# vandenheuvel/rust-lp

Measured on AMD Instinct MI355X. Metric: simplex iterations/sec, higher is better.
Workload: dtype f64; 1 GPU; dense10k: synthetic dense LP 10000x10000 f64 (+10000 slack columns), SteepestDescent, dense tableau with blocked f64-MFMA updates; m=10000, n=10000, seed=20250002, engine=tableau, update_block=64, parallelism=single GPU, solves=1

## Files before the change

include/relp_engine.h:

```cpp
#ifndef RELP_ENGINE_H
#define RELP_ENGINE_H

#include <stdint.h>

#ifdef __cplusplus
extern "C" {
#endif

typedef struct relp_engine relp_engine_t;

typedef enum {
    RELP_OK = 0,
    RELP_E_ARG = -1,
    RELP_E_HIP = -2,
    RELP_E_ZERO_PIVOT = -3,
    RELP_E_SINGULAR = -4,
    RELP_E_STATE = -5,
    RELP_E_UNSUPPORTED = -6,
    RELP_E_ALLOC = -7
} relp_status_t;

typedef enum {
    RELP_RUNNING = 0,
    RELP_OPTIMAL = 1,
// ... 37 lines not shown
    double  tol_zero;
    double  tol_tie;
    double  tol_feas;
    int32_t poll_interval;
    int32_t trace_capacity;
    int32_t shard_rank, shard_count;
    int32_t update_block;
    int32_t engine;
    int32_t ratio_rule;
    int32_t artificial_removal;
    int32_t pivot_rescue;
    int32_t auto_reinversion;
} relp_config_t;

typedef enum { RELP_RATIO_REFERENCE = 0, RELP_RATIO_LARGEST_PIVOT = 1 } relp_ratio_rule_t;
typedef enum { RELP_ARTIFICIAL_REFERENCE = 0, RELP_ARTIFICIAL_TEXTBOOK = 1 } relp_artificial_removal_t;

typedef enum {
    RELP_ENGINE_REVISED = 0,
    RELP_ENGINE_TABLEAU = 1,
    RELP_ENGINE_LU = 2,
    RELP_ENGINE_AUTO = 3
} relp_engine_kind_t;

void relp_default_config(relp_config_t *cfg);
void relp_robust_config(relp_config_t *cfg);
int32_t relp_engine_kind(const relp_engine_t *h);
relp_status_t relp_robust_stats(const relp_engine_t *h, int64_t *out4);
const char *relp_last_error(const relp_engine_t *h);
const char *relp_version(void);

relp_status_t relp_engine_create(const relp_matrix_data_t *md, const relp_config_t *cfg, relp_engine_t **out);
void          relp_engine_destroy(relp_engine_t *h);
relp_status_t relp_set_stream(relp_engine_t *h, void *hip_stream);

relp_status_t relp_select_primal_pivot_column(relp_engine_t *h, int32_t rule, int32_t *found,
                                              int32_t *column, double *relative_cost);
relp_status_t relp_relative_costs(relp_engine_t *h, double *out_n);
relp_status_t relp_generate_column(relp_engine_t *h, int32_t column, double *out_m);
relp_status_t relp_generate_element(relp_engine_t *h, int32_t row, int32_t column, double *out);
relp_status_t relp_select_primal_pivot_row(relp_engine_t *h, int32_t *found, int32_t *row);
relp_status_t relp_select_primal_pivot_row_of(relp_engine_t *h, const double *column_m, int32_t *found, int32_t *row);
relp_status_t relp_bring_into_basis(relp_engine_t *h, int32_t column, int32_t row, double relative_cost,
                                    int32_t *leaving_column);

relp_status_t relp_run(relp_engine_t *h, int64_t max_iters, int64_t *iterations_done, int32_t *outcome);
relp_status_t relp_solve_relaxation(relp_engine_t *h, int64_t max_iters, int32_t *outcome);
relp_status_t relp_from_basis(relp_engine_t *h, const int32_t *basis_columns_m);
relp_status_t relp_set_reinversion_interval(relp_engine_t *h, int64_t pivots);
int64_t       relp_reinversions(const relp_engine_t *h);
relp_status_t relp_flush(relp_engine_t *h);
relp_status_t relp_tab_flush_stats(relp_engine_t *h, int64_t *out2);
int32_t       relp_tab_load_batch(const relp_engine_t *h);
int32_t       relp_update_block(const relp_engine_t *h);
relp_status_t relp_lu_stats(const relp_engine_t *h, int64_t *out8);
relp_status_t relp_lu_lookahead_stats(const relp_engine_t *h, int64_t *out4);
relp_status_t relp_lu_kernel_layout(const relp_engine_t *h, int32_t *out4);
relp_status_t relp_lu_set_device_factorisation(relp_engine_t *h, int32_t on);
relp_status_t relp_lu_device_factorisation_stats(const relp_engine_t *h, int64_t *out6);
relp_status_t relp_lu_factor_residual(relp_engine_t *h, double *out);

relp_status_t relp_lu_phase_cycles(relp_engine_t *h, int64_t *out16);

relp_status_t relp_basis_inverse_row(relp_engine_t *h, int32_t row, double *out_m);
relp_status_t relp_should_refactor(relp_engine_t *h, int32_t *out);
relp_status_t relp_generate_column_of(relp_engine_t *h, const int32_t *row_idx, const double *values, int32_t nnz, double *out_m);
relp_status_t relp_cost_difference_of(relp_engine_t *h, const int32_t *row_idx, const double *values, int32_t nnz, double *out);
relp_status_t relp_lu_change_basis(relp_engine_t *h, int32_t pivot_row_index);
relp_status_t relp_lu_set_factors(relp_engine_t *h, const int64_t *l_col_ptr, const int32_t *l_row_idx, const double *l_values,
                                  const int64_t *u_col_ptr, const int32_t *u_row_idx, const double *u_values);
relp_status_t relp_lu_updates(relp_engine_t *h, int32_t *count);
relp_status_t relp_lu_get_update(relp_engine_t *h, int32_t k, int32_t *pivot, int32_t *idx, double *values, int32_t cap, int32_t *nnz);
relp_status_t relp_lu_get_upper(relp_engine_t *h, int64_t *col_ptr_m1, int32_t *row_idx, double *values, int64_t cap, int64_t *nnz);

int32_t relp_nr_rows(const relp_engine_t *h);
int32_t relp_nr_columns(const relp_engine_t *h);
int32_t relp_phase(const relp_engine_t *h);
int32_t relp_nr_artificial(const relp_engine_t *h);
relp_status_t relp_get_objective(relp_engine_t *h, double *out);
relp_status_t relp_get_b(relp_engine_t *h, double *out_m);
relp_status_t relp_get_minus_pi(relp_engine_t *h, double *out_m);
relp_status_t relp_get_basis_indices(relp_engine_t *h, int32_t *out_m);
relp_status_t relp_get_basis_inverse(relp_engine_t *h, double *out_mm);
relp_status_t relp_current_bfs(relp_engine_t *h, int32_t *cols, double *vals, int32_t cap, int32_t *count);
relp_status_t relp_get_iterations(relp_engine_t *h, int64_t *out);
relp_status_t relp_get_degenerate_pivots(relp_engine_t *h, int64_t *out);
relp_status_t relp_get_trace(relp_engine_t *h, int32_t *phase, int32_t *entering, int32_t *row,
                             int32_t *leaving, int64_t cap, int64_t *count);
relp_status_t relp_check_basis(relp_engine_t *h, double *max_identity_error, double *max_basic_cost,
                               double *min_b);

typedef enum {
    RELP_K_PRICE = 0, RELP_K_SELECT_COLUMN = 1, RELP_K_BUILD_COLUMN = 2, RELP_K_FTRAN = 3,
    RELP_K_RATIO = 4, RELP_K_UPDATE_VECTORS = 5, RELP_K_UPDATE_INVERSE = 6,
    RELP_K_APPLY_W = 7,
    RELP_K_UPDATE_W = 8,
    RELP_K_FLUSH = 9,
    RELP_K_FT_RUN = 10,
    RELP_K_COUNT = 11
} relp_kernel_id_t;
relp_status_t relp_profile_enable(relp_engine_t *h, int32_t enable, int64_t max_launches, int32_t sample_every);
relp_status_t relp_profile_read(relp_engine_t *h, int32_t kernel_id, int64_t *launches, double *total_ms);

relp_status_t relp_synth_fill_dense(double *device_a, int64_t ld, int32_t m, int32_t n, uint64_t seed,
                                    int64_t first_column, void *hip_stream);
relp_status_t relp_device_alloc(void **out, int64_t bytes);
// ... 33 lines not shown
```

rust-lp_amd/csrc/relp_abi.cpp:

```cpp
#include <cstring>
#include <new>

#include "relp_engine.hpp"

using relp::Engine;

struct relp_engine { Engine impl; };

#define H(h) ((h)->impl)

extern "C" {

void relp_default_config(relp_config_t* cfg) {
    std::memset(cfg, 0, sizeof(*cfg));
    cfg->device = -1;
    cfg->phase_one_rule = RELP_RULE_FIRST_PROFITABLE_WITH_MEMORY;
    cfg->phase_two_rule = RELP_RULE_STEEPEST_DESCENT;
    cfg->tol_cost = 1e-7; cfg->tol_pivot = 1e-5; cfg->tol_zero = 1e-11; cfg->tol_tie = 1e-9; cfg->tol_feas = 1e-7;
    cfg->poll_interval = 64;
    cfg->trace_capacity = 0;
    cfg->shard_rank = 0; cfg->shard_count = 1;
    cfg->update_block = -1;
    cfg->engine = RELP_ENGINE_REVISED;
}
// ... 5 lines not shown
    cfg->pivot_rescue = 1;
    cfg->auto_reinversion = 1;
    cfg->engine = RELP_ENGINE_AUTO;
}
int32_t relp_engine_kind(const relp_engine_t* h) { return h ? H(h).engine_kind() : -1; }
relp_status_t relp_robust_stats(const relp_engine_t* h, int64_t* out4) { return (h && out4) ? H(h).robust_stats(out4) : RELP_E_ARG; }

const char* relp_last_error(const relp_engine_t* h) { return h ? H(h).last_error() : "null handle"; }
const char* relp_version(void) { return "relp-mi355x 0.2 (gfx950; engines: explicit inverse, dense tableau, sparse LU + Forrest-Tomlin)"; }

relp_status_t relp_engine_create(const relp_matrix_data_t* md, const relp_config_t* cfg, relp_engine_t** out) {
    if (!md || !cfg || !out) return RELP_E_ARG;
    relp_engine_t* h = new (std::nothrow) relp_engine_t();
    if (!h) return RELP_E_ALLOC;
    relp_status_t st = H(h).create(*md, *cfg);
    *out = h;
    return st;
}

void relp_engine_destroy(relp_engine_t* h) { delete h; }
relp_status_t relp_set_stream(relp_engine_t* h, void* s) { return h ? H(h).set_stream((hipStream_t)s) : RELP_E_ARG; }

relp_status_t relp_select_primal_pivot_column(relp_engine_t* h, int32_t rule, int32_t* found, int32_t* column, double* cost) {
    return h ? H(h).select_primal_pivot_column(rule, found, column, cost) : RELP_E_ARG;
}
relp_status_t relp_relative_costs(relp_engine_t* h, double* out) { return (h && out) ? H(h).relative_costs(out) : RELP_E_ARG; }
relp_status_t relp_generate_column(relp_engine_t* h, int32_t column, double* out) { return h ? H(h).generate_column(column, out) : RELP_E_ARG; }
relp_status_t relp_generate_element(relp_engine_t* h, int32_t row, int32_t column, double* out) {
    return h ? H(h).generate_element(row, column, out) : RELP_E_ARG;
}
relp_status_t relp_select_primal_pivot_row(relp_engine_t* h, int32_t* found, int32_t* row) {
    return h ? H(h).select_primal_pivot_row(found, row) : RELP_E_ARG;
}
relp_status_t relp_select_primal_pivot_row_of(relp_engine_t* h, const double* column, int32_t* found, int32_t* row) {
    return (h && column) ? H(h).select_primal_pivot_row_of(column, found, row) : RELP_E_ARG;
}
relp_status_t relp_bring_into_basis(relp_engine_t* h, int32_t column, int32_t row, double cost, int32_t* leaving) {
    return h ? H(h).bring_into_basis(column, row, cost, leaving) : RELP_E_ARG;
}

relp_status_t relp_run(relp_engine_t* h, int64_t max_iters, int64_t* done, int32_t* outcome) {
    return h ? H(h).run(max_iters, done, outcome) : RELP_E_ARG;
}
relp_status_t relp_solve_relaxation(relp_engine_t* h, int64_t max_iters, int32_t* outcome) {
    return h ? H(h).solve_relaxation(max_iters, outcome) : RELP_E_ARG;
}
relp_status_t relp_from_basis(relp_engine_t* h, const int32_t* basis) { return (h && basis) ? H(h).from_basis(basis) : RELP_E_ARG; }

relp_status_t relp_flush(relp_engine_t* h) { return h ? H(h).flush() : RELP_E_ARG; }
relp_status_t relp_set_reinversion_interval(relp_engine_t* h, int64_t pivots) { return h ? H(h).set_reinversion_interval(pivots) : RELP_E_ARG; }
int64_t relp_reinversions(const relp_engine_t* h) { return h ? H(h).reinversions() : -1; }
int32_t relp_update_block(const relp_engine_t* h) { return h ? H(h).update_block() : -1; }
int32_t relp_tab_load_batch(const relp_engine_t* h) { return h ? H(h).tab_load_batch_size() : -1; }
relp_status_t relp_lu_stats(const relp_engine_t* h, int64_t* out8) { return (h && out8) ? H(h).lu_stats(out8) : RELP_E_ARG; }
relp_status_t relp_lu_lookahead_stats(const relp_engine_t* h, int64_t* out4) { return (h && out4) ? H(h).lu_lookahead_stats(out4) : RELP_E_ARG; }
relp_status_t relp_lu_kernel_layout(const relp_engine_t* h, int32_t* out4) { return (h && out4) ? H(h).lu_kernel_layout(out4) : RELP_E_ARG; }
relp_status_t relp_lu_set_device_factorisation(relp_engine_t* h, int32_t on) { return h ? H(h).lu_set_device_factorisation(on != 0) : RELP_E_ARG; }
relp_status_t relp_lu_factor_residual(relp_engine_t* h, double* out) { return (h && out) ? H(h).lu_factor_residual(out) : RELP_E_ARG; }
relp_status_t relp_lu_device_factorisation_stats(const relp_engine_t* h, int64_t* out6) { return (h && out6) ? H(h).luf_stats(out6) : RELP_E_ARG; }
relp_status_t relp_shard_inject_failure(relp_engine_t* h, int64_t after_pivots) { if (!h) return RELP_E_ARG; H(h).shard_inject_failure(after_pivots); return RELP_OK; }
relp_status_t relp_lu_phase_cycles(relp_engine_t* h, int64_t* out16) { return (h && out16) ? H(h).lu_phase_cycles(out16) : RELP_E_ARG; }
relp_status_t relp_basis_inverse_row(relp_engine_t* h, int32_t row, double* out_m) { return (h && out_m) ? H(h).basis_inverse_row(row, out_m) : RELP_E_ARG; }
relp_status_t relp_should_refactor(relp_engine_t* h, int32_t* out) { return (h && out) ? H(h).should_refactor(out) : RELP_E_ARG; }
relp_status_t relp_generate_column_of(relp_engine_t* h, const int32_t* idx, const double* val, int32_t nnz, double* out_m) {
    return h ? H(h).generate_column_of(idx, val, nnz, out_m) : RELP_E_ARG;
}
relp_status_t relp_cost_difference_of(relp_engine_t* h, const int32_t* idx, const double* val, int32_t nnz, double* out) {
    return h ? H(h).cost_difference_of(idx, val, nnz, out) : RELP_E_ARG;
}
relp_status_t relp_lu_change_basis(relp_engine_t* h, int32_t row) { return h ? H(h).lu_change_basis(row) : RELP_E_ARG; }
relp_status_t relp_lu_set_factors(relp_engine_t* h, const int64_t* l_ptr, const int32_t* l_idx, const double* l_val,
                                  const int64_t* u_ptr, const int32_t* u_idx, const double* u_val) {
    return h ? H(h).lu_set_factors(l_ptr, l_idx, l_val, u_ptr, u_idx, u_val) : RELP_E_ARG;
}
relp_status_t relp_lu_updates(relp_engine_t* h, int32_t* count) { return (h && count) ? H(h).lu_updates(count) : RELP_E_ARG; }
relp_status_t relp_lu_get_update(relp_engine_t* h, int32_t k, int32_t* pivot, int32_t* idx, double* val, int32_t cap, int32_t* nnz) {
    return h ? H(h).lu_get_update(k, pivot, idx, val, cap, nnz) : RELP_E_ARG;
}
relp_status_t relp_lu_get_upper(relp_engine_t* h, int64_t* col_ptr, int32_t* row_idx, double* values, int64_t cap, int64_t* nnz) {
    return h ? H(h).lu_get_upper(col_ptr, row_idx, values, cap, nnz) : RELP_E_ARG;
}
relp_status_t relp_shard_flush_begin(relp_engine_t* h, double** snap, int64_t* len) {
    return h ? H(h).shard_flush_begin(snap, len) : RELP_E_ARG;
}
relp_status_t relp_shard_flush_end(relp_engine_t* h) { return h ? H(h).shard_flush_end() : RELP_E_ARG; }
relp_status_t relp_shard_set_collectives(relp_engine_t* h, relp_allgather_fn ag, relp_allreduce_sum_fn ar, void* ctx) {
    return h ? H(h).shard_set_collectives(ag, ar, ctx) : RELP_E_ARG;
}
relp_status_t relp_shard_run(relp_engine_t* h, int64_t max_iters, int64_t* done, int32_t* outcome) {
    return h ? H(h).shard_run(max_iters, done, outcome) : RELP_E_ARG;
}
relp_status_t relp_rccl_attach(relp_engine_t* h, const uint8_t* id) { return (h && id) ? H(h).rccl_attach(id) : RELP_E_ARG; }

int32_t relp_nr_rows(const relp_engine_t* h) { return h ? H(h).nr_rows() : -1; }
int32_t relp_nr_columns(const relp_engine_t* h) { return h ? H(h).nr_columns() : -1; }
int32_t relp_phase(const relp_engine_t* h) { return h ? H(h).phase() : -1; }
int32_t relp_nr_artificial(const relp_engine_t* h) { return h ? H(h).nr_artificial() : -1; }
relp_status_t relp_get_objective(relp_engine_t* h, double* out) { return (h && out) ? H(h).get_objective(out) : RELP_E_ARG; }
relp_status_t relp_get_b(relp_engine_t* h, double* out) { return (h && out) ? H(h).get_vector(0, out) : RELP_E_ARG; }
relp_status_t relp_get_minus_pi(relp_engine_t* h, double* out) { return (h && out) ? H(h).get_vector(1, out) : RELP_E_ARG; }
relp_status_t relp_get_basis_indices(relp_engine_t* h, int32_t* out) { return (h && out) ? H(h).get_basis_indices(out) : RELP_E_ARG; }
relp_status_t relp_get_basis_inverse(relp_engine_t* h, double* out) { return (h && out) ? H(h).get_basis_inverse(out) : RELP_E_ARG; }
relp_status_t relp_current_bfs(relp_engine_t* h, int32_t* cols, double* vals, int32_t cap, int32_t* count) {
    return h ? H(h).current_bfs(cols, vals, cap, count) : RELP_E_ARG;
}
relp_status_t relp_get_iterations(relp_engine_t* h, int64_t* out) { return (h && out) ? H(h).get_iterations(out) : RELP_E_ARG; }
// ... 62 lines not shown
```

rust-lp_amd/csrc/relp_device_common.h:

```cpp
#pragma once
#include <algorithm>
#include "relp_kernels.h"

#include <math.h>

namespace relp {

static constexpr int kThreads = 256;
static constexpr int kVecPerBlock = 8;
static constexpr int kSingleBlock = 1024;

__device__ __forceinline__ double wave_sum(double v) {
#pragma unroll
    for (int off = 32; off > 0; off >>= 1) v += __shfl_down(v, off, 64);
    return v;
}

__device__ __forceinline__ void block_multi_dot(const double* __restrict__ M, int64_t ld, int len,
                                                int v0, int v_hi, const double* __restrict__ x,
                                                double* s_partial ,
                                                double& result) {
    const int t = threadIdx.x;
    double acc[kVecPerBlock];
    const double* base[kVecPerBlock];
// ... 44 lines not shown
    __shared__ double s_k[BS / 64];
    __shared__ int s_j[BS / 64];
#pragma unroll
    for (int off = 32; off > 0; off >>= 1) {
        const double ok = __shfl_down(key, off, 64);
        const int oj = __shfl_down(kj, off, 64);
        if (ok < key || (ok == key && oj < kj)) { key = ok; kj = oj; }
    }
    const int lane = threadIdx.x & 63, wave = threadIdx.x >> 6;
    if (lane == 0) { s_k[wave] = key; s_j[wave] = kj; }
    __syncthreads();
    key = s_k[0]; kj = s_j[0];
#pragma unroll
    for (int w = 1; w < BS / 64; ++w)
        if (s_k[w] < key || (s_k[w] == key && s_j[w] < kj)) { key = s_k[w]; kj = s_j[w]; }
}

__device__ __forceinline__ void block_partial_min(double key, int kj, SelectPartials sp, int slot) {
    block_min_key<kThreads>(key, kj);
    if (threadIdx.x == 0) { sp.k1[slot] = key; sp.j[slot] = kj; }
}

__device__ __forceinline__ void price_virtual_body(const ColumnTable& ct, const double* __restrict__ minus_pi,
                                                   double* __restrict__ d, int cost_mode, const SelectPartials& sp,
                                                   const PivotRecord* rec, int block) {
    const int t = block * kThreads + threadIdx.x;
    int j = -1;
    double val = 0.0;
    if (t < ct.nr_artificial) {
        j = t;
        val = (cost_mode == 1 ? 1.0 : 0.0) + minus_pi[ct.column_to_row[t]];
    } else {
        const int v = t - ct.nr_artificial;
        if (v < ct.nr_virtual) {
            const int r0 = ct.vrow0[v];
            double s = r0 >= 0 ? (double)ct.vsign[v] * minus_pi[r0] : 0.0;
            const int r1 = ct.vrow1[v];
            if (r1 >= 0) s += minus_pi[r1];
            j = ct.nr_artificial + ct.nr_normal + v;
            val = s;
        }
    }
    if (j >= 0) d[j] = val;
    if (!sp.k1) return;
    double key = INFINITY;
    int kj = 0x7fffffff;
    if (j >= 0 && !sp.in_basis[j] && val < -sp.tol_cost) { key = select_key(sp.rule, sp.n, rec, j, val); kj = j; }
    block_partial_min(key, kj, sp, sp.offset + block);
}

template <int BS>
__device__ __forceinline__ void tab_select_entering(const TableauView& tv, const SelectPartials& sp, int count, double& k1,
                                                    int& bj) {
    constexpr int kListMax = 32, kGroups = BS / kThreads;
    __shared__ int s_list[kListMax];
    __shared__ int s_cnt;
    __shared__ int s_low[BS / 64];
    for (int t = threadIdx.x + BS; t < count; t += BS) {
        const double key = sp.k1[t];
        const int j = sp.j[t];
        if (key < k1 || (key == k1 && j < bj)) { k1 = key; bj = j; }
    }
    if (threadIdx.x == 0) s_cnt = 0;
    block_min_key<BS>(k1, bj);
    if (!(bj != 0x7fffffff && sp.rule == 2 && sp.tol_tie > 0.0)) return;
    const double bound = k1 + sp.tol_tie * fmax(1.0, fabs(k1));
    for (int t = threadIdx.x; t < count; t += BS) {
        if (!(sp.k1[t] <= bound)) continue;
        const int pos = atomicAdd(&s_cnt, 1);
        if (pos < kListMax) s_list[pos] = t;
    }
    __syncthreads();
    const int listed = s_cnt;
    const int grp = threadIdx.x / kThreads, u = threadIdx.x % kThreads;
    int lowest = 0x7fffffff;
    auto scan_slot = [&](int t) {
        const int c = tv.c_lo + t * kThreads + u;
        const int j = c - tv.col_off;
        if (c < tv.c_hi && j >= 0 && j < tv.n) {
            const double v = tv.d[c];
            if (!sp.in_basis[j] && v < -sp.tol_cost && v <= bound && j < lowest) lowest = j;
        }
    };
    if (listed <= kListMax) {
        for (int i = grp; i < listed; i += kGroups) scan_slot(s_list[i]);
    } else {
        for (int t = grp; t < count; t += kGroups)
            if (sp.k1[t] <= bound) scan_slot(t);
    }
#pragma unroll
    for (int off = 32; off > 0; off >>= 1) lowest = min(lowest, __shfl_down(lowest, off, 64));
    if ((threadIdx.x & 63) == 0) s_low[threadIdx.x >> 6] = lowest;
    __syncthreads();
    bj = s_low[0];
#pragma unroll
    for (int w = 1; w < BS / 64; ++w) bj = min(bj, s_low[w]);
}

__device__ __forceinline__ int candidate_winner(const double* key, const double* idx, int64_t stride, int count, int rule,
                                                double tol_tie) {
    int win = -1; double k1 = INFINITY; double kj = 0.0;
    for (int g = 0; g < count; ++g) {
        const double a = key[g * stride], j = idx[g * stride];
        if (a < k1 || (a == k1 && win >= 0 && j < kj)) { k1 = a; kj = j; win = g; }
    }
    if (win >= 0 && rule == 2 && tol_tie > 0.0) {
        const double bound = k1 + tol_tie * fmax(1.0, fabs(k1));
        for (int g = 0; g < count; ++g)
            if (key[g * stride] <= bound && idx[g * stride] < kj) { kj = idx[g * stride]; win = g; }
    }
    return win;
}

static constexpr int kMaxRanks = 64;
__device__ __forceinline__ int candidate_winner_staged(const double* __restrict__ msgs, int count, int64_t msg_len, int rule,
                                                       double tol_tie, int* q, double* d_q) {
    __shared__ double s_key[kMaxRanks], s_idx[kMaxRanks], s_dq[kMaxRanks];
    __shared__ int s_win;
    for (int g = threadIdx.x; g < count && g < kMaxRanks; g += blockDim.x) {
        s_key[g] = msgs[g * msg_len + 0]; s_idx[g] = msgs[g * msg_len + 1]; s_dq[g] = msgs[g * msg_len + 2];
    }
    __syncthreads();
    if (threadIdx.x == 0) s_win = candidate_winner(s_key, s_idx, 1, count, rule, tol_tie);
    __syncthreads();
    const int win = s_win;
    if (win >= 0) { *q = (int)s_idx[win]; *d_q = s_dq[win]; }
    return win;
}

__device__ __forceinline__ void record_candidate(PivotRecord* rec, int rule, int win, int q, double d_q) {
    if (win < 0) {
        rec->outcome = DEV_NO_CANDIDATE;
        if (rule == 1) rec->last_selected = -1;
    } else {
        rec->q = q;
        rec->d_q = d_q;
        if (rule == 1) rec->last_selected = q;
    }
}

__device__ __forceinline__ double pivot_b(double a, double b_i, double br, bool is_r) {
    return is_r ? br : (a != 0.0 ? fma(-a, br, b_i) : b_i);
}

__device__ __forceinline__ void pivot_bookkeeping(int phase, long long iterations, double minus_objective, double d_q, double br,
                                                  int q, int r, int leaving, uint8_t* in_basis, int32_t* trace, int64_t trace_cap,
                                                  PivotRecord* rec) {
    rec->minus_objective = fma(-d_q, br, minus_objective);
    if (leaving < kWrappedArtificialBase) in_basis[leaving] = 0;
    in_basis[q] = 1;
    if (trace && iterations < trace_cap) {
        trace[0 * trace_cap + iterations] = phase;
        trace[1 * trace_cap + iterations] = q;
        trace[2 * trace_cap + iterations] = r;
        trace[3 * trace_cap + iterations] = leaving;
    }
    if (br == 0.0) rec->degenerate += 1;
    rec->iterations = iterations + 1;
}

static constexpr int kMaxEta = 128;

typedef unsigned long long tie_key_t;
static constexpr tie_key_t kNoTieKey = ~0ull;
__device__ __forceinline__ tie_key_t tie_key(double a, int leave, int ratio_rule) {
    const unsigned size = ratio_rule ? 0x7fffffffu - __float_as_uint((float)a) : 0u;
    return ((tie_key_t)size << 32) | (unsigned)leave;
}
__device__ __forceinline__ int tie_key_leaving(tie_key_t k) { return (int)(unsigned)(k & 0xffffffffull); }

template <int BS>
__device__ __forceinline__ void tie_reduce(tie_key_t& key, int& row, tie_key_t* s_k, int* s_r, bool wide) {
    const int lane = threadIdx.x & 63, wave = threadIdx.x >> 6;
    if (wide) {
#pragma unroll
        for (int off = 32; off > 0; off >>= 1) {
            const tie_key_t ok = __shfl_down(key, off, 64);
            const int orow = __shfl_down(row, off, 64);
            if (ok < key) { key = ok; row = orow; }
        }
    } else {
        int lv = (int)(unsigned)key;
        if (key == kNoTieKey) lv = 0x7fffffff;
#pragma unroll
        for (int off = 32; off > 0; off >>= 1) {
            const int ol = __shfl_down(lv, off, 64);
            const int orow = __shfl_down(row, off, 64);
            if (ol < lv) { lv = ol; row = orow; }
        }
        key = (unsigned)lv;
    }
    if (lane == 0) { s_k[wave] = key; s_r[wave] = row; }
    __syncthreads();
    key = s_k[0]; row = s_r[0];
#pragma unroll
    for (int w = 1; w < BS / 64; ++w)
        if (s_k[w] < key) { key = s_k[w]; row = s_r[w]; }
}

template <int BS>
__device__ __forceinline__ void ratio_commit_row(int r, int leaving, const double* alpha, const double* b, const DeferredUpdate& du,
                                                 int p, PivotRecord* rec, int guard_m = 0, double guard_rel = 0.0) {
    if (guard_m > 0) {
        __shared__ double s_gm[BS / 64];
        double mx = 0.0;
        for (int i = threadIdx.x; i < guard_m; i += BS) mx = fmax(mx, fabs(alpha[i]));
#pragma unroll
        for (int off = 32; off > 0; off >>= 1) mx = fmax(mx, __shfl_down(mx, off, 64));
        __syncthreads();
        if ((threadIdx.x & 63) == 0) s_gm[threadIdx.x >> 6] = mx;
        __syncthreads();
        double amax = s_gm[0];
#pragma unroll
        for (int w = 1; w < BS / 64; ++w) amax = fmax(amax, s_gm[w]);
// ... 189 lines not shown
```

rust-lp_amd/csrc/relp_engine.cpp:

```cpp
#include "relp_engine_internal.hpp"

#include <algorithm>
#include <chrono>
#include <cmath>
#include <cstdio>
#include <cstdlib>
#include <cstring>
#include <limits>

namespace relp {

bool Engine::hip_ok(hipError_t e, const char* what) {
    if (e == hipSuccess) return true;
    err_ = std::string(what) + ": " + hipGetErrorString(e);
    return false;
}

Engine::~Engine() { rccl_release(); luf_release(); }

ColumnTable Engine::table() const {
    ColumnTable ct;
    ct.nr_artificial = lay_.nr_artificial;
    ct.nr_normal = lay_.nr_normal;
    ct.nr_virtual = lay_.nr_virtual;
    ct.nr_constraints = lay_.mc;
    ct.column_to_row = d_column_to_row_;
    ct.bound_row = d_bound_row_;
    ct.vrow0 = d_vrow0_;
    ct.vrow1 = d_vrow1_;
    ct.vsign = d_vsign_;
    ct.cost = d_cost_;
    return ct;
}

Tolerances Engine::tolerances() const { return Tolerances{cfg_.tol_cost, cfg_.tol_pivot, cfg_.tol_zero, cfg_.tol_tie, cfg_.ratio_rule, (pivot_guard_on_ && guard_rel_ > 0.0) ? 1 : 0, guard_rel_}; }

TableauView Engine::tview() const {
    TableauView tv;
    tv.T0 = dT0_ - (int64_t)lay_.sc_lo * ld_t_; tv.ld_t = ld_t_;
    tv.R0 = dR0_ - (int64_t)lay_.sc_lo; tv.ld_r = ld_r_;
    tv.d = d_d_; tv.m = lay_.m; tv.n_store = n_store_;
    tv.col_off = phase_ == 1 ? 0 : tab_na_;
    tv.n = nr_columns();
    tv.c_lo = lay_.sc_lo; tv.c_hi = lay_.sc_hi;
    return tv;
}

FlushList Engine::flush_list() const {
    FlushList fl;
    fl.cols = d_fcols_; fl.count = d_fcount_; fl.mask = d_fmask_; fl.R0c = d_R0c_; fl.ld = ld_r_; fl.stats = d_fstats_;
    return fl;
}

SelectPartials Engine::tab_partials(int rule) const {
    SelectPartials sp;
    sp.k1 = d_part_k1_; sp.j = d_part_j_; sp.in_basis = d_in_basis_; sp.tol_cost = cfg_.tol_cost; sp.rule = rule;
    sp.n = nr_columns(); sp.offset = 0; sp.nb_struct = 0; sp.tol_tie = cfg_.tol_tie; sp.p_lo = 0; sp.cols_per_slot = 8;
    return sp;
}

DeferredUpdate Engine::deferred() const {
    DeferredUpdate du;
    du.W = d_W_; du.ld = ld_b_; du.kmax = block_; du.S = d_S_; du.pos_of_row = d_pos_of_row_; du.wr = d_wr_; du.R = d_R_;
    du.batch = load_batch_; du.w_split = w_split_;
    return du;
}

relp_status_t Engine::fetch(void* dst, const void* src, size_t bytes) {
    HIP_TRY(hipMemcpyAsync(dst, src, bytes, hipMemcpyDeviceToHost, stream_));
    HIP_TRY(hipStreamSynchronize(stream_));
    return RELP_OK;
}

relp_status_t Engine::download_rec() { return fetch(h_rec_, d_rec_, sizeof(PivotRecord)); }

relp_status_t Engine::upload_rec() {
    HIP_TRY(hipMemcpyAsync(d_rec_, h_rec_, sizeof(PivotRecord), hipMemcpyHostToDevice, stream_));
    HIP_TRY(hipStreamSynchronize(stream_));
    return RELP_OK;
}

relp_status_t Engine::set_stream(hipStream_t s) {
    if (stream_) HIP_TRY(hipStreamSynchronize(stream_));
    if (owns_stream_ && stream_) HIP_TRY(hipStreamDestroy(stream_));
    stream_ = s;
    owns_stream_ = false;
    return RELP_OK;
}

Switches Switches::read() {
    Switches s;
    auto given = [](const char* name) { return std::getenv(name) != nullptr; };
    auto num = [](const char* name, int unset) { const char* e = std::getenv(name); return e ? std::atoi(e) : unset; };
    s.debug = given("RELP_DEBUG");
    s.pivot_guard_set = given("RELP_PIVOT_GUARD");
    if (s.pivot_guard_set) s.pivot_guard = std::atof(std::getenv("RELP_PIVOT_GUARD"));
    s.tab_flush_all = num("RELP_TAB_FLUSH_ALL", 0) != 0;
    s.tab_load_batch = num("RELP_TAB_LOAD_BATCH", 0);
    s.tab_w_split = num("RELP_TAB_W_SPLIT", 0);
    s.fused_update = num("RELP_FUSED_UPDATE", 1) != 0;
    s.lu_lookahead_set = given("RELP_LU_LOOKAHEAD");
    s.lu_lookahead = num("RELP_LU_LOOKAHEAD", 8);
    s.fuse_lanes = num("RELP_FUSE_LANES", 256);
    s.lu_device_factor = num("RELP_LU_DEVICE_FACTOR", 0);
    s.lu_pipeline_short = num("RELP_LU_PIPELINE_SHORT", 0) != 0;
    s.ft_big = num("RELP_FT_BIG", -1);
    s.ft_hyper_set = given("RELP_FT_HYPER");
    s.ft_hyper = num("RELP_FT_HYPER", 0x9);
    s.ft_grid_price = given("RELP_FT_GRID_PRICE") ? (num("RELP_FT_GRID_PRICE", 0) != 0 ? 1 : 0) : -1;
    if (given("RELP_LUF_BUMP_CAP")) s.luf_bump_cap = std::max(16, num("RELP_LUF_BUMP_CAP", 0));
    s.luf_dense = std::max(0, std::min(64, num("RELP_LUF_DENSE", 64)));
    s.dump_basis_set = given("RELP_DUMP_BASIS");
    if (s.dump_basis_set) s.dump_basis = std::getenv("RELP_DUMP_BASIS");
    return s;
}

relp_status_t Engine::create(const relp_matrix_data_t& md, const relp_config_t& cfg) {
    (void)hipGetLastError();
    cfg_ = cfg;
    sw_ = Switches::read();
    if (sw_.pivot_guard_set && cfg_.pivot_rescue && cfg_.shard_count <= 1) guard_rel_ = sw_.pivot_guard;
    if (cfg_.shard_count < 1) cfg_.shard_count = 1;
    if (cfg_.poll_interval < 1) cfg_.poll_interval = 64;
    if (const relp_status_t lst = lay_.build(md, cfg_, &err_)) return lst;
    if (cfg_.device >= 0) HIP_TRY(hipSetDevice(cfg_.device));
    phase_ = 1;
    n_alloc_ = lay_.nr_columns();

    HIP_TRY(hipStreamCreateWithFlags(&stream_, hipStreamNonBlocking));
    owns_stream_ = true;
    const int32_t n_local = lay_.col_hi - lay_.col_lo;
    lu_ = lay_.engine == RELP_ENGINE_LU;
    tableau_ = lay_.engine == RELP_ENGINE_TABLEAU;
    if (lu_) {
        if (cfg_.shard_count > 1) return fail(RELP_E_UNSUPPORTED, "the LU engine is not sharded");
        relp_status_t lst = lu_load_matrix(md);
        if (lst) return lst;
    } else if (md.format == RELP_FORMAT_DENSE) {
        if (lay_.nr_normal > 0 && lay_.mc > 0 && !md.dense) return fail(RELP_E_ARG, "dense matrix missing");
        const int64_t src_ld = md.dense_ld > 0 ? md.dense_ld : lay_.mc;
        if (src_ld < lay_.mc) return fail(RELP_E_ARG, "dense_ld < nr_constraints");
        if (md.matrix_memory == RELP_MEM_DEVICE && (src_ld % 2) == 0) {
            dA_.adopt(const_cast<double*>(md.dense)); ld_a_ = src_ld;
        } else {
            ld_a_ = round_up(std::max<int64_t>(lay_.mc, 1), 2);
            HIP_TRY(dA_.alloc(ld_a_ * std::max(n_local, 1)));
            if (n_local > 0 && lay_.mc > 0)
                HIP_TRY(hipMemcpy2D(dA_, ld_a_ * sizeof(double), md.dense, src_ld * sizeof(double), lay_.mc * sizeof(double),
                                    n_local, md.matrix_memory == RELP_MEM_DEVICE ? hipMemcpyDeviceToDevice : hipMemcpyHostToDevice));
        }
    } else if (md.format == RELP_FORMAT_CSC) {
        if (md.matrix_memory != RELP_MEM_HOST) return fail(RELP_E_UNSUPPORTED, "CSC input must be in host memory");
        if (!md.col_ptr) return fail(RELP_E_ARG, "col_ptr missing");
        ld_a_ = round_up(std::max<int64_t>(lay_.mc, 1), 2);
        const int64_t e0 = n_local > 0 ? md.col_ptr[lay_.col_lo] : 0, e1 = n_local > 0 ? md.col_ptr[lay_.col_hi] : 0;
        for (int64_t p = e0; p < e1; ++p)
            if (md.row_idx[p] < 0 || md.row_idx[p] >= lay_.mc) return fail(RELP_E_ARG, "row index out of range");
        const int64_t cells = ld_a_ * std::max(n_local, 1);
        HIP_TRY(dA_.alloc(cells));
        HIP_TRY(hipMemset(dA_, 0, (size_t)cells * sizeof(double)));
        if (e1 > e0) {
            DeviceBuf<int64_t> t_ptr; DeviceBuf<int32_t> t_idx; DeviceBuf<double> t_val;
            if (t_ptr.alloc_raw(sizeof(int64_t) * (size_t)(n_local + 1)) != hipSuccess ||
                t_idx.alloc_raw(sizeof(int32_t) * (size_t)(e1 - e0)) != hipSuccess ||
                t_val.alloc_raw(sizeof(double) * (size_t)(e1 - e0)) != hipSuccess)
                return fail(RELP_E_ALLOC, "staging the CSC arrays");
            hipError_t err = hipMemcpy(t_ptr, md.col_ptr + lay_.col_lo, sizeof(int64_t) * (size_t)(n_local + 1), hipMemcpyHostToDevice);
            if (err == hipSuccess) err = hipMemcpy(t_idx, md.row_idx + e0, sizeof(int32_t) * (size_t)(e1 - e0), hipMemcpyHostToDevice);
            if (err == hipSuccess) err = hipMemcpy(t_val, md.values + e0, sizeof(double) * (size_t)(e1 - e0), hipMemcpyHostToDevice);
            if (err == hipSuccess) {
                launch_csc_to_dense(t_ptr, t_idx, t_val, n_local, dA_, ld_a_, nullptr);
                err = hipDeviceSynchronize();
            }
            if (err != hipSuccess) return fail(RELP_E_HIP, "dense copy of the CSC input");
        }
    } else {
        return fail(RELP_E_ARG, "unknown matrix format");
    }

    ld_b_ = round_up(lay_.m, 16);
    const int64_t rows_local = std::max(lay_.row_hi - lay_.row_lo, 1);
    HIP_TRY(dBinv_.alloc((tableau_ || lu_) ? 16 : rows_local * ld_b_));
    HIP_TRY(d_minus_pi_.alloc(ld_b_));
    HIP_TRY(d_b_.alloc(ld_b_));
    HIP_TRY(d_alpha_.alloc(ld_b_));
    HIP_TRY(d_aq_.alloc(ld_b_));
    HIP_TRY(d_rho_.alloc(ld_b_));
    HIP_TRY(d_w_.alloc(ld_b_));
    HIP_TRY(d_d_.alloc(n_alloc_));
    HIP_TRY(d_cost_.alloc(lay_.nr_normal));
    HIP_TRY(d_basis_.alloc(lay_.m));
    HIP_TRY(d_column_to_row_.alloc(lay_.nr_artificial));
    HIP_TRY(d_bound_row_.alloc(lay_.nr_normal));
    HIP_TRY(d_vrow0_.alloc(lay_.nr_virtual));
    HIP_TRY(d_vrow1_.alloc(lay_.nr_virtual));
    HIP_TRY(d_vsign_.alloc(lay_.nr_virtual));
    HIP_TRY(d_in_basis_.alloc(n_alloc_));
    HIP_TRY(d_rec_.alloc(1));
    {
        const int64_t slots = price_structural_blocks(lay_.col_lo, lay_.col_hi) + (lay_.nr_artificial + lay_.nr_virtual + 255) / 256 + 8 +
                              tab_scan_blocks(n_alloc_) + price_csc_blocks(0, lay_.nr_normal);
        HIP_TRY(d_part_k1_.alloc(slots));
        HIP_TRY(d_part_j_.alloc(slots));
    }
    block_ = cfg_.update_block < 0 ? (lay_.m >= 4096 ? 64 : 0) : std::min(cfg_.update_block, 128);
    if (lu_) {
        block_ = cfg_.update_block < 0 ? 128 : std::max(1, std::min(cfg_.update_block, 128));
        HIP_TRY(d_lu_scratch_.alloc(ld_b_));
        HIP_TRY(h_basis_.alloc(sizeof(int32_t) * (size_t)std::max(lay_.m, 1)));
        luf_enabled_ = sw_.lu_device_factor != 0;
        luf_download_ = sw_.lu_device_factor == 2;
        relp_status_t fst = ft_plan_and_alloc();
        if (fst) return fst;
    }
    if (tableau_) {
        if (block_ == 0) block_ = 64;
        if (cfg_.update_block < 0 && lay_.m >= 4096 && n_alloc_ >= 40000) block_ = 96;
        n_store_ = n_alloc_;
        tab_na_ = lay_.nr_artificial;
        const int64_t n_owned = std::max(lay_.sc_hi - lay_.sc_lo, 1);
        ld_t_ = round_up(lay_.m, 2);
        ld_r_ = round_up(n_owned, 2);
        HIP_TRY(dT0_.alloc(ld_t_ * n_owned));
        HIP_TRY(dR0_.alloc(ld_r_ * (block_ + 1)));
        {
            flush_all_ = sw_.tab_flush_all;
            HIP_TRY(d_fstats_.alloc(2));
            if (!flush_all_) {
                HIP_TRY(d_fcols_.alloc(n_owned));
                HIP_TRY(d_fcount_.alloc(1));
                HIP_TRY(d_fmask_.alloc((n_owned + 63) / 64));
                HIP_TRY(d_R0c_.alloc(ld_r_ * block_));
            }
        }
        {
            load_batch_ = tab_load_batch(sw_.tab_load_batch);
            w_split_ = sw_.tab_w_split >= 1 ? std::min(sw_.tab_w_split, 16) : kTabSplitDefault;
        }
        {
            fused_update_ = sw_.fused_update;
            if (cfg_.pivot_rescue && cfg_.shard_count == 1) fused_update_ = false;
            if (fused_update_) {
                HIP_TRY(d_b_alt_.alloc(ld_b_));
                HIP_TRY(d_basis_alt_.alloc(lay_.m));
                HIP_TRY(d_shadow_.alloc(std::max(block_, 1) + 1));
                HIP_TRY(d_shadow_meta_.alloc_raw(2 * sizeof(int32_t)));
                const int32_t none[2] = {-1, 0};
                HIP_TRY(hipMemcpy(d_shadow_meta_, none, sizeof none, hipMemcpyHostToDevice));
            }
        }
        HIP_TRY(d_cost_store_.alloc(n_store_));
        HIP_TRY(d_idcol_.alloc(lay_.m));
    }
    if (block_ > 0) HIP_TRY(d_v_.alloc(ld_b_));
    if (block_ > 0 && !ft_) {
        HIP_TRY(d_W_.alloc(ld_b_ * block_));
        if (!tableau_) HIP_TRY(d_R_.alloc(ld_b_ * block_));
        HIP_TRY(d_wr_.alloc(block_));
        HIP_TRY(d_S_.alloc(block_));
        HIP_TRY(d_pos_of_row_.alloc(lay_.m));
        HIP_TRY(hipMemset(d_pos_of_row_, 0xFF, sizeof(int32_t) * lay_.m));
    }
    HIP_TRY(d_rmin_.alloc(lay_.m / 8 + 2));
    HIP_TRY(h_rec_.alloc(sizeof(PivotRecord)));
    trace_cap_ = std::max(cfg_.trace_capacity, 0);
    if (trace_cap_ > 0) HIP_TRY(d_trace_.alloc(4 * trace_cap_));

    auto up = [&](void* dst, const void* src, size_t bytes) -> hipError_t {
        return bytes ? hipMemcpy(dst, src, bytes, hipMemcpyHostToDevice) : hipSuccess;
    };
    HIP_TRY(up(d_cost_, lay_.cost.data(), sizeof(double) * lay_.nr_normal));
    HIP_TRY(up(d_bound_row_, lay_.bound_row.data(), sizeof(int32_t) * lay_.nr_normal));
    HIP_TRY(up(d_vrow0_, lay_.vrow0.data(), sizeof(int32_t) * lay_.nr_virtual));
    HIP_TRY(up(d_vrow1_, lay_.vrow1.data(), sizeof(int32_t) * lay_.nr_virtual));
    HIP_TRY(up(d_vsign_, lay_.vsign.data(), sizeof(int32_t) * lay_.nr_virtual));
    HIP_TRY(up(d_column_to_row_, lay_.column_to_row.data(), sizeof(int32_t) * lay_.nr_artificial));
    HIP_TRY(up(d_basis_, lay_.basis.data(), sizeof(int32_t) * lay_.m));
    HIP_TRY(up(d_b_, lay_.rhs.data(), sizeof(double) * lay_.m));
    HIP_TRY(up(d_minus_pi_, lay_.minus_pi.data(), sizeof(double) * lay_.m));
    std::vector<uint8_t> flags(n_alloc_, 0);
    for (int32_t r = 0; r < lay_.m; ++r) flags[lay_.basis[r]] = 1;
    HIP_TRY(up(d_in_basis_, flags.data(), flags.size()));
    if (lay_.row_hi > lay_.row_lo && !tableau_ && !lu_) launch_set_identity(dBinv_, ld_b_, lay_.row_lo, lay_.row_hi, stream_);
    if (tableau_) {
        idcol_h_ = lay_.basis;
        HIP_TRY(up(d_idcol_, idcol_h_.data(), sizeof(int32_t) * lay_.m));
        launch_tab_build(tview(), A_base(), ld_a_, table(), stream_);
        cost_store_h_.assign(n_store_, 0.0);
        for (int32_t k = 0; k < lay_.nr_artificial; ++k) cost_store_h_[k] = 1.0;
        std::vector<double> w(ld_b_, 0.0);
// ... 33 lines not shown
        prof_ev_.resize((size_t)max_launches * 2);
        for (auto& e : prof_ev_) HIP_TRY(hipEventCreate(&e));
        prof_kid_.reserve((size_t)max_launches);
    }
    return RELP_OK;
}

void Engine::prof_begin(int kid, hipStream_t on) {
    prof_open_ = false;
    if (!prof_on_ || (prof_kid_.size() + 1) * 2 > prof_ev_.size()) return;
    if (kid != RELP_K_FLUSH && (prof_tick_ % prof_stride_) != 0) return;
    (void)hipEventRecord(prof_ev_[2 * prof_kid_.size()], on ? on : stream_);
    prof_kid_.push_back(kid);
    prof_open_ = true;
}

void Engine::prof_end(hipStream_t on) {
    if (!prof_open_) return;
    (void)hipEventRecord(prof_ev_[2 * (prof_kid_.size() - 1) + 1], on ? on : stream_);
    prof_open_ = false;
}

relp_status_t Engine::profile_read(int kernel_id, int64_t* launches, double* total_ms) {
    HIP_TRY(hipStreamSynchronize(stream_));
    int64_t n = 0; double ms = 0.0;
    for (size_t k = 0; k < prof_kid_.size(); ++k) {
        if (prof_kid_[k] != kernel_id) continue;
        float t = 0.f;
        if (hipEventElapsedTime(&t, prof_ev_[2 * k], prof_ev_[2 * k + 1]) == hipSuccess) { ms += t; ++n; }
    }
    if (launches) *launches = n;
    if (total_ms) *total_ms = ms;
    return RELP_OK;
}

void Engine::enqueue_price(int cost_mode, const double* vec, const PivotRecord* rec, int32_t p_lo, int32_t p_hi) {
    const ColumnTable ct = table();
    if (lu_) {
        launch_price_csc(csc(), ct, vec, d_d_, 0, lay_.nr_normal, cost_mode, SelectPartials{}, rec, stream_);
        launch_price_virtual(ct, vec, d_d_, cost_mode, rec, stream_);
        return;
    }
    launch_price_structural(A_base(), ld_a_, ct, vec, d_d_, p_lo, p_hi, cost_mode, rec, stream_);
    if (p_lo > 0 || p_hi < lay_.nr_normal) launch_price_mask_unowned(ct, d_d_, p_lo, p_hi, rec, stream_);
    launch_price_virtual(ct, vec, d_d_, cost_mode, rec, stream_);
}

void Engine::enqueue_iteration_tableau(int rule) {
    const TableauView tv = tview();
    const DeferredUpdate du = deferred();
    const SelectPartials sp = tab_partials(rule);
    if (fused_update_ && in_loop_) {
        prof_begin(RELP_K_FTRAN);
        launch_tab_select_column_rmin(tv, du, sp, tab_scan_blocks(lay_.sc_hi - lay_.sc_lo), d_alpha_, d_b_, tolerances(), d_rmin_,
                                      d_rec_, stream_, d_shadow_, d_shadow_meta_);
        prof_end();
        prof_begin(RELP_K_PRICE);
        launch_tab_ratio_update_all(tv, du, sp, lay_.m, d_alpha_, d_b_, d_b_alt_, d_basis_, d_basis_alt_, d_in_basis_, d_trace_,
                                    trace_cap_, tolerances(), d_rmin_, d_shadow_, d_shadow_meta_, d_rec_, stream_);
        prof_end();
        d_b_.swap(d_b_alt_);
        d_basis_.swap(d_basis_alt_);
        shadow_pending_ = true;
        if (++since_flush_ >= block_) enqueue_flush();
        return;
    }
    tab_settle();
    prof_begin(RELP_K_FTRAN);
    launch_tab_select_column_rmin(tv, du, sp, tab_scan_blocks(lay_.sc_hi - lay_.sc_lo), d_alpha_, d_b_, tolerances(), d_rmin_,
                                  d_rec_, stream_);
    prof_end();
    prof_begin(RELP_K_RATIO);
    launch_ratio_blocks(d_alpha_, d_b_, d_basis_, lay_.m, tolerances(), du, d_rmin_, d_rec_, stream_);
    prof_end();
    prof_begin(RELP_K_PRICE);
    launch_tab_update_all(tv, du, sp, lay_.m, d_alpha_, d_b_, d_basis_, d_in_basis_, d_trace_, trace_cap_, d_rec_, stream_);
    prof_end();
    if (++since_flush_ >= block_) enqueue_flush();
}

void Engine::enqueue_iteration(int rule) {
    struct Tick { int64_t& t; ~Tick() { ++t; } } tick{prof_tick_};
    if (tableau_) { enqueue_iteration_tableau(rule); return; }
    if (lu_) { enqueue_iteration_lu(rule); return; }
    const ColumnTable ct = table();
    const double* A = A_base();
    double* Binv = Binv_base();
    const int nb_struct = price_structural_blocks(lay_.col_lo, lay_.col_hi);
    SelectPartials sp = tab_partials(rule);
    sp.nb_struct = nb_struct; sp.p_lo = lay_.col_lo;
    const int nb_virt = price_virtual_blocks(ct);
    prof_begin(RELP_K_PRICE);
    if (lay_.col_lo > 0 || lay_.col_hi < lay_.nr_normal) {
        launch_price_structural_sel(A, ld_a_, ct, d_minus_pi_, d_d_, lay_.col_lo, lay_.col_hi, phase_, sp, d_rec_, stream_);
        launch_price_mask_unowned(ct, d_d_, lay_.col_lo, lay_.col_hi, d_rec_, stream_);
        SelectPartials spv = sp;
        spv.offset = nb_struct;
        launch_price_virtual_sel(ct, d_minus_pi_, d_d_, phase_, spv, d_rec_, stream_);
    } else {
        launch_price_all_sel(A, ld_a_, ct, d_minus_pi_, d_d_, lay_.col_lo, lay_.col_hi, phase_, sp, d_rec_, stream_);
    }
    prof_end();
    prof_begin(RELP_K_SELECT_COLUMN);
    launch_select_partials(sp, nb_struct + nb_virt, d_d_, A, ld_a_, ct, lay_.m, d_aq_, d_rec_, stream_);
    prof_end();
    if (block_ == 0) {
        prof_begin(RELP_K_FTRAN);
        launch_ftran_rmin(Binv, ld_b_, lay_.m, d_aq_, d_alpha_, d_b_, tolerances(), d_rmin_, d_rec_, stream_);
        prof_end();
        prof_begin(RELP_K_RATIO);
        launch_ratio_rows(d_alpha_, d_b_, d_basis_, lay_.m, tolerances(), DeferredUpdate{}, d_rmin_, ftran_rows_per_block(), d_rec_,
                          stream_);
        prof_end();
        prof_begin(RELP_K_UPDATE_VECTORS);
        launch_compute_rho(Binv, ld_b_, lay_.m, lay_.row_lo, lay_.row_hi, d_rho_, d_rec_, stream_);
        prof_end();
        prof_begin(RELP_K_UPDATE_INVERSE);
        launch_update_inverse_vectors(Binv, ld_b_, lay_.m, d_alpha_, d_rho_, d_b_, d_minus_pi_, d_basis_, d_in_basis_, d_trace_,
                                      trace_cap_, d_rec_, stream_);
        prof_end();
        return;
    }
// ... 41 lines not shown
        prof_begin(RELP_K_FLUSH);
        launch_tab_flush(tview(), dut, d_rec_, flush_list(), stream_);
        launch_flush_reset(dut, d_rec_, stream_);
        prof_end();
        since_flush_ = 0;
        if (++flushes_since_reprice_ >= kRepriceEveryFlushes) {
            tableau_reprice();
        }
        return;
    }
    const DeferredUpdate du = deferred();
    double* Binv = Binv_base();
    prof_begin(RELP_K_FLUSH);
    launch_flush_snapshot(du, Binv, ld_b_, lay_.row_lo, lay_.row_hi, d_rec_, stream_);
    launch_flush_apply(du, Binv, ld_b_, lay_.m, lay_.row_lo, lay_.row_hi, d_rec_, stream_);
    launch_flush_reset(du, d_rec_, stream_);
    prof_end();
    since_flush_ = 0;
}

void Engine::tableau_reprice() {
    const TableauView tv = tview();
    flushes_since_reprice_ = 0;
    launch_tab_basis_costs(tv, d_basis_, d_cost_store_, d_w_, stream_);
    launch_tab_price_init(tv, d_w_, d_cost_store_, stream_);
    launch_tab_scan(tv, tab_partials(current_rule()), d_rec_, stream_);
}

relp_status_t Engine::flush() {
    tab_settle();
    if (cfg_.shard_count > 1 && block_ > 0 && !tableau_) {
        if (!coll_allreduce_) return fail(RELP_E_STATE, "sharded flush needs relp_shard_flush_begin/end (or the collective hooks)");
        if (since_flush_ == 0) return RELP_OK;
        double* snap = nullptr; int64_t len = 0;
        relp_status_t st = shard_flush_begin(&snap, &len);
        if (st) return st;
        if (len > 0) {
            if (coll_allreduce_(coll_ctx_, snap, len, stream_)) return fail(RELP_E_HIP, "all-reduce of the flush snapshot failed");
            if ((st = shard_flush_end())) return st;
        }
        since_flush_ = 0;
        return RELP_OK;
    }
    enqueue_flush();
    return RELP_OK;
}

relp_status_t Engine::select_primal_pivot_column(int rule, int32_t* found, int32_t* column, double* cost) {
    relp_status_t st = edit_rec();
    if (st) return st;
    if (tableau_) {
        const SelectPartials sp = tab_partials(rule);
        launch_tab_scan(tview(), sp, d_rec_, stream_);
        launch_tab_select(tview(), sp, tab_scan_blocks(lay_.sc_hi - lay_.sc_lo), d_rec_, stream_);
    } else {
        enqueue_price(phase_, d_minus_pi_, d_rec_, lay_.col_lo, lay_.col_hi);
        launch_select_column(d_d_, d_in_basis_, nr_columns(), rule, cfg_.tol_cost, cfg_.tol_tie, d_rec_, stream_);
    }
    if ((st = download_rec())) return st;
    const bool ok = h_rec_->outcome == DEV_RUNNING;
    if (found) *found = ok ? 1 : 0;
    if (ok) { if (column) *column = h_rec_->q; if (cost) *cost = h_rec_->d_q; }
    h_rec_->outcome = DEV_RUNNING;
    return upload_rec();
}

relp_status_t Engine::relative_costs(double* out_n) {
    if (!tableau_) enqueue_price(phase_, d_minus_pi_, nullptr, lay_.col_lo, lay_.col_hi);
    const double* src = tableau_ ? d_d_ + (phase_ == 1 ? 0 : tab_na_) : d_d_;
    return fetch(out_n, src, sizeof(double) * nr_columns());
}

relp_status_t Engine::generate_column(int32_t column, double* out_m) {
    if (column < 0 || column >= nr_columns()) return fail(RELP_E_ARG, "column out of range");
    const relp_status_t st = edit_rec([&](PivotRecord& r) { r.q = column; });
    if (st) return st;
    if (tableau_) {
        launch_tab_column(tview(), deferred(), d_alpha_, d_rec_, stream_);
    } else if (lu_ && ft_) {
        launch_ft_ftran(dlu_, fts_, ft_problem(0), column, nullptr, d_alpha_, stream_);
    } else if (lu_) {
        launch_build_column_csc(csc(), table(), lay_.m, d_aq_, d_rec_, stream_);
        launch_lu_ftran(dlu_, d_aq_, d_v_, d_lu_scratch_, d_rec_, stream_);
        launch_apply_w(deferred(), lay_.m, d_v_, d_alpha_, d_rec_, stream_);
    } else {
        enqueue_flush();
        launch_build_column(A_base(), ld_a_, table(), lay_.m, d_aq_, d_rec_, stream_);
        launch_ftran(Binv_base(), ld_b_, lay_.m, lay_.row_lo, lay_.row_hi, d_aq_, d_alpha_, 0, d_rec_, stream_);
    }
    if (out_m) HIP_TRY(hipMemcpyAsync(out_m, d_alpha_, sizeof(double) * lay_.m, hipMemcpyDeviceToHost, stream_));
    HIP_TRY(hipStreamSynchronize(stream_));
    return RELP_OK;
}

relp_status_t Engine::generate_element(int32_t row, int32_t column, double* out) {
    if (row < 0 || row >= lay_.m) return fail(RELP_E_ARG, "row out of range");
    std::vector<double> col(lay_.m);
    relp_status_t st = generate_column(column, col.data());
    if (st) return st;
    if (out) *out = col[row];
    return RELP_OK;
}

relp_status_t Engine::read_pivot_row(int32_t* found, int32_t* row) {
    const relp_status_t st = download_rec();
    if (st) return st;
    const bool ok = h_rec_->outcome == DEV_RUNNING;
// ... 833 lines not shown
```

rust-lp_amd/csrc/relp_engine.hpp:

```cpp
#pragma once
#include <hip/hip_runtime.h>

#include <cstdint>
#include <chrono>
#include <condition_variable>
#include <functional>
#include <mutex>
#include <string>
#include <thread>
#include <vector>

#include "../../include/relp_engine.h"
#include "relp_buffers.hpp"
#include "relp_kernels.h"
#include "relp_layout.hpp"
#include "relp_lu.hpp"

namespace relp {

struct HostPool {
    struct Slot { std::thread th; std::mutex mu; std::condition_variable cv; std::function<void()> job; bool busy = false, stop = false; };
    Slot slot[2];
    void run(int i, std::function<void()> f) {
        Slot& s = slot[i];
        if (!s.th.joinable())
            s.th = std::thread([&s] {
                std::unique_lock<std::mutex> lk(s.mu);
                for (;;) {
                    s.cv.wait(lk, [&s] { return s.busy || s.stop; });
                    if (s.stop) return;
                    lk.unlock(); s.job(); lk.lock();
                    s.busy = false;
                    s.cv.notify_all();
                }
            });
        { std::lock_guard<std::mutex> lk(s.mu); s.job = std::move(f); s.busy = true; }
        s.cv.notify_all();
    }
    void wait() {
        for (Slot& s : slot) { std::unique_lock<std::mutex> lk(s.mu); s.cv.wait(lk, [&s] { return !s.busy; }); }
    }
    ~HostPool() {
        for (Slot& s : slot) {
            if (!s.th.joinable()) continue;
            { std::lock_guard<std::mutex> lk(s.mu); s.stop = true; }
            s.cv.notify_all();
            s.th.join();
        }
    }
};

struct Switches {
    bool debug = false;
    bool pivot_guard_set = false; double pivot_guard = 0.0;
    bool tab_flush_all = false;
    int tab_load_batch = 0, tab_w_split = 0;
    bool fused_update = true;
    bool lu_lookahead_set = false; int lu_lookahead = 8;
    int fuse_lanes = 256;
    int lu_device_factor = 0;
    bool lu_pipeline_short = false;
    int ft_big = -1;
    bool ft_hyper_set = false; int ft_hyper = 0x9;
    int ft_grid_price = -1;
    int luf_bump_cap = INT32_MAX;
    int luf_dense = 64;
    bool dump_basis_set = false; std::string dump_basis;
    static Switches read();
};

struct EngineQueue {
    hipStream_t stream_ = nullptr; bool owns_stream_ = false;
    std::vector<hipEvent_t> prof_ev_;
    ~EngineQueue() {
        for (auto e : prof_ev_) (void)hipEventDestroy(e);
        if (owns_stream_ && stream_) (void)hipStreamDestroy(stream_);
    }
};

class Engine : private EngineQueue {
  public:
    Engine() = default;
    ~Engine();

    relp_status_t create(const relp_matrix_data_t& md, const relp_config_t& cfg);
    relp_status_t set_stream(hipStream_t s);

    relp_status_t select_primal_pivot_column(int rule, int32_t* found, int32_t* column, double* cost);
    relp_status_t relative_costs(double* out_n);
    relp_status_t generate_column(int32_t column, double* out_m);
    relp_status_t generate_element(int32_t row, int32_t column, double* out);
    relp_status_t select_primal_pivot_row(int32_t* found, int32_t* row);
    relp_status_t select_primal_pivot_row_of(const double* column, int32_t* found, int32_t* row);
    relp_status_t bring_into_basis(int32_t column, int32_t row, double cost, int32_t* leaving);

    relp_status_t run(int64_t max_iters, int64_t* done, int32_t* outcome);
    int32_t engine_kind() const { return lay_.engine; }
    relp_status_t robust_stats(int64_t* out4) const;
    relp_status_t solve_relaxation(int64_t max_iters, int32_t* outcome);
    relp_status_t from_basis(const int32_t* basis_columns);
    relp_status_t set_reinversion_interval(int64_t pivots);
    int64_t reinversions() const { return reinversions_; }
    relp_status_t flush();
    int32_t update_block() const { return block_; }
    relp_status_t lu_stats(int64_t* out8) const;
    relp_status_t lu_lookahead_stats(int64_t* out4) const;
    relp_status_t lu_kernel_layout(int32_t* out4) const;
    relp_status_t luf_stats(int64_t* out6) const;
    relp_status_t lu_set_device_factorisation(bool on);
    relp_status_t lu_factor_residual(double* out);
    relp_status_t lu_basis_columns(std::vector<std::vector<std::pair<int32_t, double>>>& cols);
    relp_status_t lu_basis_flat(std::vector<int64_t>& ptr, std::vector<int32_t>& idx, std::vector<double>& val);
    relp_status_t lu_phase_cycles(int64_t* out16);
    relp_status_t lu_download_basis();
    relp_status_t lu_factor_downloaded_basis();
    relp_status_t lu_refactor_lookahead(int rule, int64_t budget, bool have_basis);
    relp_status_t ft_read_report(bool* have_basis);
    void lu_refactor_clock(std::chrono::steady_clock::time_point tb, std::chrono::steady_clock::time_point t0,
                           std::chrono::steady_clock::time_point t1, std::chrono::steady_clock::time_point t2);
    relp_status_t basis_inverse_row(int32_t row, double* out_m);
    relp_status_t should_refactor(int32_t* out);
    relp_status_t generate_column_of(const int32_t* idx, const double* val, int32_t nnz, double* out_m);
    relp_status_t cost_difference_of(const int32_t* idx, const double* val, int32_t nnz, double* out);
    relp_status_t lu_change_basis(int32_t row);
    relp_status_t lu_updates(int32_t* count);
    relp_status_t lu_get_update(int32_t k, int32_t* pivot, int32_t* idx, double* val, int32_t cap, int32_t* nnz);
    relp_status_t lu_get_upper(int64_t* col_ptr, int32_t* row_idx, double* values, int64_t cap, int64_t* nnz);
    relp_status_t lu_set_factors(const int64_t* l_ptr, const int32_t* l_idx, const double* l_val, const int64_t* u_ptr,
                                 const int32_t* u_idx, const double* u_val);
    relp_status_t shard_flush_begin(double** dev_snapshot, int64_t* len);
    relp_status_t shard_flush_end();

    int32_t nr_rows() const { return lay_.m; }
    int32_t nr_columns() const { return lay_.nr_columns(); }
    int32_t phase() const { return phase_; }
    int32_t nr_artificial() const { return lay_.nr_artificial; }
    relp_status_t get_objective(double* out);
    relp_status_t get_vector(int which, double* out);
    relp_status_t get_basis_indices(int32_t* out);
    relp_status_t get_basis_inverse(double* out);
    relp_status_t current_bfs(int32_t* cols, double* vals, int32_t cap, int32_t* count);
    relp_status_t get_iterations(int64_t* out);
    relp_status_t get_degenerate_pivots(int64_t* out);
    relp_status_t tab_flush_stats(int64_t* out2);
    int32_t tab_load_batch_size() const { return tableau_ ? load_batch_ : 0; }
    relp_status_t get_trace(int32_t* phase, int32_t* entering, int32_t* row, int32_t* leaving, int64_t cap,
                            int64_t* count);
    relp_status_t check_basis(double* max_identity_error, double* max_basic_cost, double* min_b);

    relp_status_t profile_enable(bool enable, int64_t max_launches, int32_t sample_every);
    relp_status_t profile_read(int kernel_id, int64_t* launches, double* total_ms);

    void shard_ranges(int32_t* col_lo, int32_t* col_hi, int32_t* row_lo, int32_t* row_hi, int32_t* stride) const;
    int64_t candidate_len() const { return lay_.candidate_len; }
    int64_t rho_len() const { return ld_b_; }
    relp_status_t shard_price(double* dev_candidate);
    relp_status_t shard_select_column(const double* dev_candidates, int32_t count);
    relp_status_t shard_ftran(double* dev_alpha_slice);
    relp_status_t shard_ratio(const double* dev_alpha_slices, int32_t count, double* dev_rho);
    relp_status_t shard_update(const double* dev_rho);
    relp_status_t shard_pivot();
    relp_status_t shard_set_collectives(relp_allgather_fn ag, relp_allreduce_sum_fn ar, void* ctx);
    relp_status_t shard_run(int64_t max_iters, int64_t* done, int32_t* outcome);
    void shard_inject_failure(int64_t after_pivots) { inject_failure_after_ = after_pivots; }
    relp_status_t rccl_attach(const uint8_t* id);
    relp_status_t poll(int32_t* outcome, int64_t* iterations);

    const char* last_error() const { return err_.c_str(); }

  private:
    Layout lay_;
    relp_config_t cfg_{};
    int32_t phase_ = 1;

    Switches sw_;
    DeviceBuf<double> dA_; int64_t ld_a_ = 0;
    DeviceBuf<double> dBinv_; int64_t ld_b_ = 0;
    DeviceBuf<double> d_minus_pi_, d_b_, d_alpha_, d_aq_, d_rho_, d_d_, d_w_, d_cost_;
    DeviceBuf<int32_t> d_basis_, d_column_to_row_, d_bound_row_, d_vrow0_, d_vrow1_, d_vsign_, d_trace_;
    DeviceBuf<uint8_t> d_in_basis_;
    DeviceBuf<PivotRecord> d_rec_;
    PinnedBuf<PivotRecord> h_rec_;
    int64_t trace_cap_ = 0;
    int32_t block_ = 0;
    int64_t since_flush_ = 0;
    DeviceBuf<double> d_v_;
    DeviceBuf<double> d_W_, d_wr_, d_R_;
    DeviceBuf<int32_t> d_S_, d_pos_of_row_;
    DeviceBuf<double> d_part_k1_;
    DeviceBuf<int32_t> d_part_j_;
    bool tableau_ = false;
    DeviceBuf<double> dT0_; int64_t ld_t_ = 0;
    DeviceBuf<double> dR0_; int64_t ld_r_ = 0;
    bool flush_all_ = false;
    DeviceBuf<int32_t> d_fcols_, d_fcount_;
    DeviceBuf<unsigned long long> d_fmask_, d_fstats_;
    DeviceBuf<double> d_R0c_;
    FlushList flush_list() const;
    int32_t load_batch_ = 0, w_split_ = 0;
    DeviceBuf<double> d_cost_store_;
    DeviceBuf<int32_t> d_idcol_;
    bool fused_update_ = false, shadow_pending_ = false;
    DeviceBuf<double> d_b_alt_, d_shadow_;
    DeviceBuf<int32_t> d_basis_alt_, d_shadow_meta_;
    DeviceBuf<double> d_rmin_;
    int32_t n_store_ = 0;
    int32_t tab_na_ = 0;
    bool tab_partials_valid_ = false;
    static constexpr int kRepriceEveryFlushes = 8;
    int32_t flushes_since_reprice_ = 0;
    std::vector<int32_t> idcol_h_;
    std::vector<double> cost_store_h_;
    bool in_loop_ = false;
    void tab_settle();
    struct LoopScope {
        Engine& e;
        explicit LoopScope(Engine& en) : e(en) { e.in_loop_ = true; }
        ~LoopScope() { e.in_loop_ = false; e.tab_settle(); }
    };
    struct SettledScope {
        Engine& e; bool was;
        explicit SettledScope(Engine& en) : e(en), was(en.in_loop_) { e.in_loop_ = false; e.tab_settle(); }
        ~SettledScope() { e.in_loop_ = was; }
    };
    TableauView tview() const;
    double* d_aq_big() { return dR0_ + (int64_t)block_ * ld_r_; }
    SelectPartials tab_partials(int rule) const;
    SelectPartials lu_partials(int rule) const;
    void enqueue_iteration_tableau(int rule);
    void tableau_reprice();
    bool lu_ = false;
    std::vector<int64_t> hc_ptr_; std::vector<int32_t> hc_idx_; std::vector<double> hc_val_;
    DeviceBuf<int64_t> d_cptr_; DeviceBuf<int32_t> d_cidx_; DeviceBuf<double> d_cval_;
    LUFactors hlu_;
    DeviceBuf<char> d_lu_buf_; int64_t lu_cap_ = 0;
    std::vector<std::vector<std::pair<int32_t, double>>> basis_cols_;
    std::vector<int64_t> basis_ptr_; std::vector<int32_t> basis_idx_; std::vector<double> basis_val_;
    HostPool host_pool_;
    PinnedBuf<char> h_lu_buf_; size_t h_lu_cap_ = 0;
    DeviceBuf<char> d_lu_buf_alt_; int64_t lu_cap_alt_ = 0;
    PinnedBuf<int32_t> h_basis_;
    PinnedBuf<FtMirror> h_mirror_;
    DeviceBuf<double> d_lu_scratch_;
    relp_status_t ensure_lu_scratch();
    DeviceLU dlu_{};
    relp_status_t lu_status_ = RELP_OK;
    int64_t lu_refactors_ = 0;
    int64_t lu_lookahead_installs_ = 0, lu_replayed_changes_ = 0;
    int32_t lu_pipeline_cap_ = 0;
    double refactor_us_[3] = {0.0, 0.0, 0.0};
    int64_t reinvert_interval_ = 0, since_reinvert_ = 0, reinversions_ = 0;
    DeviceCSC csc() const { return DeviceCSC{d_cptr_, d_cidx_, d_cval_}; }
// ... 122 lines not shown
```

rust-lp_amd/csrc/relp_engine_shard.cpp:

```cpp
#include "relp_engine_internal.hpp"

namespace relp {

void Engine::shard_ranges(int32_t* col_lo, int32_t* col_hi, int32_t* row_lo, int32_t* row_hi, int32_t* stride) const {
    if (col_lo) *col_lo = lay_.col_lo;
    if (col_hi) *col_hi = lay_.col_hi;
    if (row_lo) *row_lo = lay_.row_lo;
    if (row_hi) *row_hi = lay_.row_hi;
    if (stride) *stride = lay_.row_stride;
}

relp_status_t Engine::shard_pivot() {
    if (lu_) return fail(RELP_E_UNSUPPORTED, "the LU engine is not sharded");
    if (!tableau_) return fail(RELP_E_STATE, "relp_shard_pivot is the tableau engine's step");
    const int rule = current_rule();
    const TableauView tv = tview();
    const DeferredUpdate du = deferred();
    const SelectPartials sp = tab_partials(rule);
    prof_begin(RELP_K_PRICE);
    launch_tab_update_all(tv, du, sp, lay_.m, d_alpha_, d_b_, d_basis_, d_in_basis_, d_trace_, trace_cap_, d_rec_, stream_);
    prof_end();
    tab_partials_valid_ = true;
    if (++since_flush_ >= block_) enqueue_flush();
    ++prof_tick_;
    return RELP_OK;
}

relp_status_t Engine::shard_price(double* dev_candidate) {
    if (lu_) return fail(RELP_E_UNSUPPORTED, "the LU engine is not sharded");
    const int rule = current_rule();
    if (tableau_) {
        const TableauView tv = tview();
        const SelectPartials sp = tab_partials(rule);
        if (!tab_partials_valid_) { launch_tab_scan(tv, sp, d_rec_, stream_); tab_partials_valid_ = true; }
        prof_begin(RELP_K_FTRAN);
        launch_tab_select_column_msg(tv, deferred(), sp, tab_scan_blocks(lay_.sc_hi - lay_.sc_lo), dev_candidate, d_b_, tolerances(), d_rec_,
                                     stream_);
        prof_end();
        return RELP_OK;
    }
    prof_begin(RELP_K_PRICE);
    enqueue_price(phase_, d_minus_pi_, d_rec_, lay_.col_lo, lay_.col_hi);
    prof_end();
    prof_begin(RELP_K_SELECT_COLUMN);
    launch_select_column(d_d_, d_in_basis_, nr_columns(), rule, cfg_.tol_cost, cfg_.tol_tie, d_rec_, stream_);
    prof_end();
    prof_begin(RELP_K_BUILD_COLUMN);
    launch_build_column(A_base(), ld_a_, table(), lay_.m, d_aq_, d_rec_, stream_);
    launch_pack_candidate(d_aq_, lay_.m, dev_candidate, d_rec_, stream_);
    prof_end();
    return RELP_OK;
}

relp_status_t Engine::shard_select_column(const double* dev_candidates, int32_t count) {
    if (lu_) return fail(RELP_E_UNSUPPORTED, "the LU engine is not sharded");
    const int rule = current_rule();
    if (tableau_) {
        if (count > 64) return fail(RELP_E_UNSUPPORTED, "at most 64 shards");
        prof_begin(RELP_K_RATIO);
        launch_tab_select_candidate_ratio(dev_candidates, count, lay_.candidate_len, lay_.m, d_alpha_, d_b_, d_basis_, rule, tolerances(),
                                          deferred(), -1, d_rec_, stream_);
        prof_end();
        return RELP_OK;
    }
    launch_select_candidate(dev_candidates, count, lay_.candidate_len, lay_.m, d_aq_, rule, cfg_.tol_tie, d_rec_, stream_);
    return RELP_OK;
}

relp_status_t Engine::shard_ftran(double* dev_alpha_slice) {
    if (lu_) return fail(RELP_E_UNSUPPORTED, "the LU engine is not sharded");
    double* Binv = Binv_base();
    prof_begin(RELP_K_FTRAN);
    launch_ftran(Binv, ld_b_, lay_.m, lay_.row_lo, lay_.row_hi, d_aq_, dev_alpha_slice, lay_.row_lo, d_rec_, stream_);
    launch_pad_slice(dev_alpha_slice, lay_.row_hi - lay_.row_lo, lay_.row_stride, stream_);
    prof_end();
    return RELP_OK;
}

relp_status_t Engine::shard_ratio(const double* dev_alpha_slices, int32_t count, double* dev_rho) {
    if (lu_) return fail(RELP_E_UNSUPPORTED, "the LU engine is not sharded");
    double* Binv = Binv_base();
    if (block_ == 0) {
        prof_begin(RELP_K_RATIO);
        launch_gather_alpha(dev_alpha_slices, count, lay_.row_stride, lay_.m, d_alpha_, d_rec_, stream_);
        launch_ratio(d_alpha_, d_b_, d_basis_, lay_.m, tolerances(), d_rec_, stream_);
        launch_compute_rho(Binv, ld_b_, lay_.m, lay_.row_lo, lay_.row_hi, dev_rho, d_rec_, stream_);
        prof_end();
        return RELP_OK;
    }
// ... 26 lines not shown
    return RELP_OK;
}

relp_status_t Engine::shard_flush_end() {
    if (lu_) return fail(RELP_E_UNSUPPORTED, "the LU engine is not sharded");
    if (block_ == 0) return RELP_OK;
    const DeferredUpdate du = deferred();
    double* Binv = Binv_base();
    prof_begin(RELP_K_FLUSH);
    launch_flush_apply(du, Binv, ld_b_, lay_.m, lay_.row_lo, lay_.row_hi, d_rec_, stream_);
    launch_flush_reset(du, d_rec_, stream_);
    prof_end();
    since_flush_ = 0;
    return RELP_OK;
}

relp_status_t Engine::shard_update(const double* dev_rho) {
    if (lu_) return fail(RELP_E_UNSUPPORTED, "the LU engine is not sharded");
    double* Binv = Binv_base();
    prof_begin(RELP_K_UPDATE_VECTORS);
    launch_update_vectors(lay_.m, d_alpha_, dev_rho, d_b_, d_minus_pi_, d_basis_, d_in_basis_, d_trace_, trace_cap_, d_rec_,
                          stream_);
    prof_end();
    if (block_ == 0) {
        prof_begin(RELP_K_UPDATE_INVERSE);
        launch_update_inverse(Binv, ld_b_, lay_.m, lay_.row_lo, lay_.row_hi, d_alpha_, dev_rho, d_rec_, stream_);
        prof_end();
    } else {
        ++since_flush_;
    }
    return RELP_OK;
}

relp_status_t Engine::remove_artificial_basis_variables_sharded(std::vector<int32_t>& rows_to_remove) {
    std::vector<int32_t> basis, arts;
    relp_status_t st = basic_artificials(&basis, &arts);
    if (st) return st;
    if (arts.empty()) return RELP_OK;
    if (!coll_allgather_)
        return fail(RELP_E_STATE, "artificial variables are still basic after phase 1: the sharded engine pivots them out "
                                  "through the collective hooks (relp_shard_set_collectives / relp_rccl_attach)");
    const int32_t g = std::max(cfg_.shard_count, 1);
    const bool textbook = cfg_.artificial_removal == RELP_ARTIFICIAL_TEXTBOOK;
    for (int32_t a : arts) {
        int32_t pivot_row = lay_.column_to_row[a];
        if (textbook) pivot_row = (int32_t)(std::find(basis.begin(), basis.end(), a) - basis.begin());
        if ((st = edit_rec())) return st;
        const TableauView tv = tview();
        const DeferredUpdate du = deferred();
        const SelectPartials sp = tab_partials(RELP_RULE_FIRST_PROFITABLE);
        Tolerances zt = tolerances();
        if (textbook) zt.cost = INFINITY;
        launch_tab_zero_level_scan(tv, du, sp, pivot_row, lay_.nr_artificial, zt, d_rec_, stream_);
        launch_tab_select_column_msg(tv, du, sp, tab_scan_blocks(lay_.sc_hi - lay_.sc_lo), d_msg_cand_, d_b_, tolerances(), d_rec_, stream_);
        if (coll_allgather_(coll_ctx_, d_msg_cand_, d_msg_cands_, lay_.candidate_len * (int64_t)sizeof(double), stream_))
            return fail(RELP_E_HIP, "all-gather of the zero-level candidates failed");
        launch_tab_select_candidate_ratio(d_msg_cands_, g, lay_.candidate_len, lay_.m, d_alpha_, d_b_, d_basis_, RELP_RULE_FIRST_PROFITABLE,
                                          tolerances(), du, pivot_row, d_rec_, stream_);
        if ((st = download_rec())) return st;
        if (h_rec_->outcome == DEV_NO_CANDIDATE) { keep_artificial_row(a, rows_to_remove); continue; }
        if (h_rec_->alpha_r == 0.0) return fail(RELP_E_ZERO_PIVOT, "Pivot value can't be zero.");
        launch_tab_update_all(tv, du, sp, lay_.m, d_alpha_, d_b_, d_basis_, d_in_basis_, d_trace_, trace_cap_, d_rec_, stream_);
        tab_partials_valid_ = false;
        basis[pivot_row] = h_rec_->q;
        if (++since_flush_ >= block_) enqueue_flush();
    }
    return RELP_OK;
}

relp_status_t Engine::shard_set_collectives(relp_allgather_fn ag, relp_allreduce_sum_fn ar, void* ctx) {
    if (lu_) return fail(RELP_E_UNSUPPORTED, "the LU engine is not sharded");
    if (!ag || (!tableau_ && !ar)) return fail(RELP_E_ARG, "collective hooks missing");
    coll_allgather_ = ag; coll_allreduce_ = ar; coll_ctx_ = ctx;
    const int64_t g = std::max(cfg_.shard_count, 1);
    if (!d_msg_cand_) {
        HIP_TRY(d_msg_status_.alloc(2));
        HIP_TRY(d_msg_statuses_.alloc(2 * g));
        HIP_TRY(d_msg_cand_.alloc(lay_.candidate_len));
        HIP_TRY(d_msg_cands_.alloc(lay_.candidate_len * g));
        if (!tableau_) {
            HIP_TRY(d_msg_slice_.alloc(lay_.row_stride));
            HIP_TRY(d_msg_slices_.alloc((int64_t)lay_.row_stride * g));
            HIP_TRY(d_msg_rho_.alloc(rho_len()));
        }
    }
    return RELP_OK;
}

relp_status_t Engine::shard_iteration() {
    relp_status_t st;
    const int32_t g = std::max(cfg_.shard_count, 1);
    coll_step_ = 0;
    shadow_flush_ = since_flush_;
    if (inject_failure_after_ == 0) { inject_failure_after_ = -1; return fail(RELP_E_STATE, "injected failure (relp_shard_inject_failure)"); }
    if (inject_failure_after_ > 0) --inject_failure_after_;
    auto broken = [&](const char* what) { coll_broken_ = true; return fail(RELP_E_HIP, what); };
    if (tableau_ && fused_update_ && in_loop_) {
        if (g > 64) return fail(RELP_E_UNSUPPORTED, "at most 64 shards");
        const int rule = current_rule();
        const TableauView tv = tview();
        const DeferredUpdate du = deferred();
        const SelectPartials sp = tab_partials(rule);
        if (!tab_partials_valid_) { launch_tab_scan(tv, sp, d_rec_, stream_); tab_partials_valid_ = true; }
        prof_begin(RELP_K_FTRAN);
        launch_tab_select_column_msg(tv, du, sp, tab_scan_blocks(lay_.sc_hi - lay_.sc_lo), d_msg_cand_, d_b_, tolerances(), d_rec_, stream_,
                                     d_shadow_, d_shadow_meta_);
        prof_end();
        if (coll_allgather_(coll_ctx_, d_msg_cand_, d_msg_cands_, lay_.candidate_len * (int64_t)sizeof(double), stream_))
            return broken("all-gather of the PRICE candidates failed");
        ++coll_step_;
        prof_begin(RELP_K_PRICE);
        launch_tab_ratio_update_all(tv, du, sp, lay_.m, nullptr, d_b_, d_b_alt_, d_basis_, d_basis_alt_, d_in_basis_, d_trace_,
                                    trace_cap_, tolerances(), nullptr, d_shadow_, d_shadow_meta_, d_rec_, stream_, d_msg_cands_, g,
                                    lay_.candidate_len, rule);
        prof_end();
        d_b_.swap(d_b_alt_);
        d_basis_.swap(d_basis_alt_);
        shadow_pending_ = true;
        if (++since_flush_ >= block_) enqueue_flush();
        ++prof_tick_;
        return RELP_OK;
    }
    if ((st = shard_price(d_msg_cand_))) return st;
    if (coll_allgather_(coll_ctx_, d_msg_cand_, d_msg_cands_, lay_.candidate_len * (int64_t)sizeof(double), stream_))
        return broken("all-gather of the PRICE candidates failed");
    ++coll_step_;
    if ((st = shard_select_column(d_msg_cands_, g))) return st;
    if (tableau_) return shard_pivot();
    if ((st = shard_ftran(d_msg_slice_))) return st;
    if (coll_allgather_(coll_ctx_, d_msg_slice_, d_msg_slices_, lay_.row_stride * (int64_t)sizeof(double), stream_))
        return broken("all-gather of the FTRAN slices failed");
    ++coll_step_;
    if ((st = shard_ratio(d_msg_slices_, g, d_msg_rho_))) return st;
    if (coll_allreduce_(coll_ctx_, d_msg_rho_, rho_len(), stream_)) return broken("all-reduce of the pivot row failed");
    ++coll_step_;
    if ((st = shard_update(d_msg_rho_))) return st;
    if (block_ > 0 && since_flush_ >= block_) {
        double* snap = nullptr; int64_t len = 0;
        if ((st = shard_flush_begin(&snap, &len))) return st;
        if (len > 0) {
            if (coll_allreduce_(coll_ctx_, snap, len, stream_)) return broken("all-reduce of the flush snapshot failed");
            ++coll_step_;
            if ((st = shard_flush_end())) return st;
        }
        since_flush_ = 0;
    }
    return RELP_OK;
}

relp_status_t Engine::shard_iteration_comm_only(int from_step) {
    auto broken = [&](const char* what) { coll_broken_ = true; return fail(RELP_E_HIP, what); };
    if (from_step <= 0 && coll_allgather_(coll_ctx_, d_msg_cand_, d_msg_cands_, lay_.candidate_len * (int64_t)sizeof(double), stream_)) return broken("all-gather failed");
    if (tableau_) return RELP_OK;
    if (from_step <= 1 && coll_allgather_(coll_ctx_, d_msg_slice_, d_msg_slices_, lay_.row_stride * (int64_t)sizeof(double), stream_)) return broken("all-gather failed");
    if (from_step <= 2 && coll_allreduce_(coll_ctx_, d_msg_rho_, rho_len(), stream_)) return broken("all-reduce failed");
    ++shadow_flush_;
    if (block_ > 0 && shadow_flush_ >= block_) {
        if (from_step <= 3 && coll_allreduce_(coll_ctx_, d_R_, ld_b_ * block_, stream_)) return broken("all-reduce failed");
// ... 71 lines not shown
```

rust-lp_amd/csrc/relp_kernels.h:

```cpp
#pragma once
#include <hip/hip_runtime.h>
#include <stdint.h>

#include "relp_layout.hpp"

namespace relp {

enum DeviceOutcome : int32_t { DEV_RUNNING = 0, DEV_NO_CANDIDATE = 1, DEV_NO_ROW = 2 };

struct PivotRecord {
    int32_t outcome;
    int32_t q;
    double  d_q;
    int32_t r;
    int32_t leaving;
    double  alpha_r;
    double  b_r;
    double  minus_objective;
    long long iterations;
    int32_t last_selected;
    int32_t phase;
    int32_t owner_has_row;
    int32_t pad_;
    double  key1;
    int32_t n_eta;
    int32_t eta_target;
    int32_t n_eta_old;
    int32_t degenerate;
    int32_t p_now;
    int32_t pad2_;
};

struct DeferredUpdate {
    double*  W;
    int64_t  ld;
    int32_t  kmax;
    int32_t* S;
    int32_t* pos_of_row;
    double*  wr;
    double*  R;
    int32_t  batch;
    int32_t  w_split;
};

struct ColumnTable {
    int32_t nr_artificial;
    int32_t nr_normal;
    int32_t nr_virtual;
    int32_t nr_constraints;
    const int32_t* column_to_row;
    const int32_t* bound_row;
    const int32_t* vrow0;
    const int32_t* vrow1;
    const int32_t* vsign;
    const double*  cost;
};

struct Tolerances { double cost, pivot, zero, tie; int32_t ratio_rule, pivot_guard; double guard_rel; };

struct SelectPartials {
    double*        k1;
    int32_t*       j;
    const uint8_t* in_basis;
    double         tol_cost;
    int32_t        rule;
    int32_t        n;
    int32_t        offset;
    int32_t        nb_struct;
    double         tol_tie;
    int32_t        p_lo;
    int32_t        cols_per_slot;
};

struct LuRow { int32_t k, e0, e1, pad_; double diag; };
struct DeviceSchedule {
    const LuRow* rows;
    const int32_t* idx; const double* val;
    const int32_t* level_ptr;
    int32_t n_levels; int32_t nnz;
    const int32_t* seg; int32_t n_seg; int32_t pad_;
};
struct DeviceLU {
    int32_t m; int32_t pad_;
    const int32_t* rowperm;
    const int32_t* colperm;
    DeviceSchedule Lf, Uf, Ub, Lb;
};
static constexpr int kEllLg = 13;
static constexpr int kEllLgWide = 24;
static constexpr int kEllPadHeaders = 4;
struct EllPass { int32_t lane0, lanes, info, level; };
struct EllSchedule {
    const EllPass*  passes;
    const int32_t*  lvl_pass;
    double*         rdiag;
    double*         sval;
    const double*   oval;
    const int32_t*  rovf;
    const uint16_t* sidx;
    const uint16_t* oidx;
    const int32_t*  via_ptr;
    const int32_t*  via_pos;
    int32_t n_passes, n_levels, m, n_lanes, n_ovf;
    int32_t bytes;
    int32_t rhs_base;
    int32_t n_triv;
    const int32_t* triv;
    const int32_t* reach;
    const int32_t* rhs_src;
    int32_t n_rhs, pad_;
    const int32_t* rhs_pos;
    const uint32_t* triv_bits;
};

struct DeviceCSC { const int64_t* col_ptr; const int32_t* row_idx; const double* values; };

static constexpr int kFtThreads = 512;
static constexpr int kFtWaves = kFtThreads / 64;
static constexpr int kFtMaxSlots = 64;
static constexpr int kFtMaxRows = 1 << 20;
static constexpr int kFtLdsBudget = 156 * 1024;
static constexpr int kFtBitmapBytes = 40 * 1024;
static inline __host__ __device__ int ft_bitmap_shift(int m, int rhs_cap) {
    int s = 0;
// ... 106 lines not shown
void launch_compute_rho(const double* Binv, int64_t ld_b, int32_t m, int32_t row_lo, int32_t row_hi,
                        double* rho, PivotRecord* rec, hipStream_t s);
void launch_update_vectors(int32_t m, const double* alpha, const double* rho, double* b, double* minus_pi,
                           int32_t* basis_indices, uint8_t* in_basis, int32_t* trace, int64_t trace_cap,
                           PivotRecord* rec, hipStream_t s);
void launch_update_inverse(double* Binv, int64_t ld_b, int32_t m, int32_t row_lo, int32_t row_hi,
                           const double* alpha, const double* rho, const PivotRecord* rec, hipStream_t s);
void launch_update_inverse_vectors(double* Binv, int64_t ld_b, int32_t m, const double* alpha, const double* rho, double* b,
                                   double* minus_pi, int32_t* basis_indices, uint8_t* in_basis, int32_t* trace,
                                   int64_t trace_cap, PivotRecord* rec, hipStream_t s);

void launch_weighted_column_sums(const double* Binv, int64_t ld_b, int32_t m, const double* w,
                                 double* minus_pi, hipStream_t s);
void launch_set_identity(double* Binv_local, int64_t ld_b, int32_t row_lo, int32_t row_hi, hipStream_t s);
void launch_fill_dense(double* A, int64_t ld, int32_t m, int32_t n, uint64_t seed, int64_t first_column,
                       hipStream_t s);
void launch_csc_to_dense(const int64_t* col_ptr, const int32_t* row_idx, const double* values, int32_t n_cols, double* A,
                         int64_t ld, hipStream_t s);

void launch_apply_w(const DeferredUpdate& du, int32_t m, const double* v, double* alpha, const PivotRecord* rec,
                    hipStream_t s);
int32_t ftran_rows_per_block();
void launch_ftran_rmin(const double* Binv, int64_t ld_b, int32_t m, const double* aq, double* out, const double* b,
                       Tolerances tol, double* rmin, const PivotRecord* rec, hipStream_t s);
void launch_apply_w_rmin(const DeferredUpdate& du, int32_t m, const double* v, double* alpha, const double* b, Tolerances tol,
                         double* rmin, const PivotRecord* rec, hipStream_t s);
void launch_ratio_rows(const double* alpha, const double* b, const int32_t* basis_indices, int32_t m, Tolerances tol,
                       const DeferredUpdate& du, const double* rmin, int32_t rows_per_block, PivotRecord* rec, hipStream_t s);
void launch_eta_prepare(const DeferredUpdate& du, PivotRecord* rec, hipStream_t s);
void launch_update_w(const DeferredUpdate& du, int32_t m, const double* alpha, const PivotRecord* rec, hipStream_t s);
void launch_rho_deferred(const DeferredUpdate& du, const double* Binv, int64_t ld_b, int32_t m, int32_t row_lo,
                         int32_t row_hi, double* rho, PivotRecord* rec, hipStream_t s);
void launch_flush_snapshot(const DeferredUpdate& du, const double* Binv, int64_t ld_b, int32_t row_lo, int32_t row_hi,
                           const PivotRecord* rec, hipStream_t s);
void launch_flush_apply(const DeferredUpdate& du, double* Binv, int64_t ld_b, int32_t m, int32_t row_lo,
                        int32_t row_hi, const PivotRecord* rec, hipStream_t s);
void launch_flush_reset(const DeferredUpdate& du, PivotRecord* rec, hipStream_t s);

struct TableauView {
    double*  T0;      int64_t ld_t;
    double*  R0;      int64_t ld_r;
    double*  d;
    int32_t  m;
    int32_t  n_store;
    int32_t  col_off;
    int32_t  n;
    int32_t  c_lo, c_hi;
};
void launch_tab_build(const TableauView& tv, const double* A, int64_t ld_a, const ColumnTable& ct, hipStream_t s);
void launch_tab_price_init(const TableauView& tv, const double* w, const double* cost_store, hipStream_t s);
void launch_tab_basis_costs(const TableauView& tv, const int32_t* basis_indices, const double* cost_store, double* w,
                            hipStream_t s);
void launch_tab_scan(const TableauView& tv, SelectPartials sp, const PivotRecord* rec, hipStream_t s);
int32_t tab_scan_blocks(int32_t n_owned_columns);
bool launch_lu_ftran_cols(const DeviceLU& lu, const TableauView& tv, const double* A, int64_t ld_a, const ColumnTable& ct,
                          int32_t c_first, int32_t c_count, hipStream_t s);
void launch_tab_select(const TableauView& tv, SelectPartials sp, int32_t count, PivotRecord* rec, hipStream_t s);
void launch_tab_column(const TableauView& tv, const DeferredUpdate& du, double* alpha, const PivotRecord* rec,
                       hipStream_t s);
void launch_tab_row_update(const TableauView& tv, const DeferredUpdate& du, SelectPartials sp, PivotRecord* rec,
                           hipStream_t s);
void launch_tab_update_vectors(int32_t m, const double* alpha, double* b, int32_t* basis_indices, uint8_t* in_basis,
                               int32_t* trace, int64_t trace_cap, PivotRecord* rec, hipStream_t s);
void launch_tab_select_column_rmin(const TableauView& tv, const DeferredUpdate& du, SelectPartials sp, int32_t count,
                                   double* alpha, const double* b, Tolerances tol, double* rmin, PivotRecord* rec,
                                   hipStream_t s, const double* shadow = nullptr, int32_t* shadow_meta = nullptr);
void launch_ratio_blocks(const double* alpha, const double* b, const int32_t* basis_indices, int32_t m, Tolerances tol,
                         const DeferredUpdate& du, const double* rmin, PivotRecord* rec, hipStream_t s);
void launch_tab_select_column_msg(const TableauView& tv, const DeferredUpdate& du, SelectPartials sp, int32_t count,
                                  double* msg, const double* b, Tolerances tol, PivotRecord* rec, hipStream_t s,
                                  const double* shadow = nullptr, int32_t* shadow_meta = nullptr);
void launch_tab_select_candidate_ratio(const double* msgs, int32_t count, int64_t msg_len, int32_t m, double* alpha,
                                       const double* b, const int32_t* basis_indices, int32_t rule, Tolerances tol,
                                       const DeferredUpdate& du, int32_t forced_row, PivotRecord* rec, hipStream_t s);
void launch_tab_zero_level_scan(const TableauView& tv, const DeferredUpdate& du, SelectPartials sp, int32_t row,
                                int32_t nr_artificial, Tolerances tol, const PivotRecord* rec, hipStream_t s);
void launch_tab_update_all(const TableauView& tv, const DeferredUpdate& du, SelectPartials sp, int32_t m,
                           const double* alpha, double* b, int32_t* basis_indices, uint8_t* in_basis, int32_t* trace,
                           int64_t trace_cap, PivotRecord* rec, hipStream_t s);
struct FlushList {
    int32_t*            cols;
    int32_t*            count;
    unsigned long long* mask;
    double*             R0c;
    int64_t             ld;
    unsigned long long* stats;
};
static constexpr int32_t kTabLoadBatchDefault = 8;
static constexpr int32_t kTabSplitDefault = 2;
static constexpr int32_t kTabSplitCUs = 256;
int32_t tab_load_batch(int32_t wanted);
void launch_tab_flush(const TableauView& tv, const DeferredUpdate& du, const PivotRecord* rec, const FlushList& fl,
                      hipStream_t s);
void launch_tab_ratio_update_all(const TableauView& tv, const DeferredUpdate& du, SelectPartials sp, int32_t m,
                                 const double* alpha, const double* b_in, double* b_out, const int32_t* basis_in,
                                 int32_t* basis_out, uint8_t* in_basis, int32_t* trace, int64_t trace_cap, Tolerances tol,
                                 const double* rmin, double* shadow, int32_t* shadow_meta, PivotRecord* rec, hipStream_t s,
                                 const double* msgs = nullptr, int32_t count = 0, int64_t msg_len = 0, int32_t rule = 0);
void launch_tab_apply_shadow(const DeferredUpdate& du, double* shadow, int32_t* shadow_meta, hipStream_t s);
void launch_tab_gather_columns(const TableauView& tv, const int32_t* cols, double* out, hipStream_t s);
void launch_tab_row(const TableauView& tv, const DeferredUpdate& du, int32_t row, double* out, const PivotRecord* rec,
                    hipStream_t s);

void launch_price_csc(const DeviceCSC& csc, const ColumnTable& ct, const double* vec, double* d, int32_t p_lo,
                      int32_t p_hi, int32_t cost_mode, SelectPartials sp, const PivotRecord* rec, hipStream_t s);
void launch_price_csc_all(const DeviceCSC& csc, const ColumnTable& ct, const double* vec, double* d, int32_t nr_normal,
                          int32_t cost_mode, SelectPartials sp, int32_t nb_virtual, const PivotRecord* rec, hipStream_t s);
int32_t price_csc_blocks(int32_t p_lo, int32_t p_hi);
void launch_select_partials_csc(SelectPartials sp, int32_t count, const double* d, const DeviceCSC& csc,
                                const ColumnTable& ct, int32_t m, double* aq, PivotRecord* rec, hipStream_t s);
void launch_build_column_csc(const DeviceCSC& csc, const ColumnTable& ct, int32_t m, double* aq, const PivotRecord* rec,
                             hipStream_t s);
void launch_lu_ftran(const DeviceLU& lu, const double* aq, double* v, double* scratch, const PivotRecord* rec,
                     hipStream_t s);
void launch_lu_btran(const DeviceLU& lu, const DeferredUpdate& du, const double* rhs, int32_t row, double* rho,
                     double* scratch, const PivotRecord* rec, hipStream_t s);
void launch_lu_btran_rows(const DeviceLU& lu, const DeferredUpdate& none, double* out, int64_t ld, double* scratch,
                          hipStream_t s);

size_t ft_lds_base_bytes(int32_t m, int32_t tcap, int32_t eta_cap, int32_t tier, int32_t rhs_cap);
int64_t ft_schedule_stage_bytes(int32_t m, int64_t nnz, int32_t n_levels, int32_t n_seg);
void launch_ft_run(const DeviceLU& lu, const FtState& st, const FtProblem& pb, int64_t max_pivots, hipStream_t s);
void launch_ft_ftran(const DeviceLU& lu, const FtState& st, const FtProblem& pb, int32_t column, const double* rhs, double* alpha,
                     hipStream_t s);
void launch_ft_btran(const DeviceLU& lu, const FtState& st, const FtProblem& pb, int32_t row, const double* rhs, double* rho,
                     hipStream_t s);
void launch_ft_update(const DeviceLU& lu, const FtState& st, const FtProblem& pb, hipStream_t s);
void launch_ft_replay(const DeviceLU& lu, const FtState& st, const FtProblem& pb, int32_t count, hipStream_t s);

void launch_pack_candidate(const double* aq, int32_t m, double* msg, PivotRecord* rec, hipStream_t s);
void launch_select_candidate(const double* msgs, int32_t count, int64_t msg_len, int32_t m, double* aq,
                             int32_t rule, double tol_tie, PivotRecord* rec, hipStream_t s);
void launch_gather_alpha(const double* slices, int32_t count, int32_t stride, int32_t m, double* alpha,
                         const PivotRecord* rec, hipStream_t s);
void launch_pad_slice(double* slice, int32_t valid, int32_t stride, hipStream_t s);

}
```

rust-lp_amd/csrc/relp_kernels_tableau.hip:

```cpp
#include "relp_device_common.h"
#include <type_traits>

namespace relp {

typedef double double4_t __attribute__((ext_vector_type(4)));

template <int B, class Use>
__device__ __forceinline__ void for_pending(const double* base, int64_t stride, int64_t x, int n, Use&& use) {
    int j0 = 0;
    for (; j0 + B <= n; j0 += B) {
        double v[B];
#pragma unroll
        for (int t = 0; t < B; ++t) v[t] = base[(int64_t)(j0 + t) * stride + x];
#pragma unroll
        for (int t = 0; t < B; ++t) use(j0 + t, v[t]);
    }
    if (B > 1 && j0 < n) {
        double v[B];
#pragma unroll
        for (int t = 0; t < B; ++t) v[t] = j0 + t < n ? base[(int64_t)(j0 + t) * stride + x] : 0.0;
#pragma unroll
        for (int t = 0; t < B; ++t)
            if (j0 + t < n) use(j0 + t, v[t]);
    }
}

template <int B>
__device__ __forceinline__ void tab_update_w_row(const DeferredUpdate& du, int i, double u, const double* s_wr, int j0, int j1) {
    if (u == 0.0 || j1 <= j0) return;
    double* col = du.W + (int64_t)j0 * du.ld;
    for_pending<B>(col, du.ld, i, j1 - j0, [&](int j, double old) {
        const double w = s_wr[j0 + j];
        if (w != 0.0) col[(int64_t)j * du.ld + i] = fma(u, w, old);
    });
}

__global__ void k_tab_build(TableauView tv, const double* __restrict__ A, int64_t ld_a, ColumnTable ct) {
    const int64_t total = (int64_t)tv.m * (tv.c_hi - tv.c_lo);
    for (int64_t idx = (int64_t)blockIdx.x * blockDim.x + threadIdx.x; idx < total; idx += (int64_t)gridDim.x * blockDim.x) {
        const int c = tv.c_lo + (int)(idx / tv.m), i = (int)(idx % tv.m);
        double v = 0.0;
        if (c < ct.nr_artificial) {
            v = (i == ct.column_to_row[c]) ? 1.0 : 0.0;
        } else {
            const int p = c - ct.nr_artificial;
            if (p < ct.nr_normal) {
                if (i < ct.nr_constraints) v = A[(int64_t)p * ld_a + i];
                else v = (i == ct.bound_row[p]) ? 1.0 : 0.0;
            } else {
                const int vv = p - ct.nr_normal;
                if (i == ct.vrow0[vv]) v = (double)ct.vsign[vv];
                else if (i == ct.vrow1[vv]) v = 1.0;
            }
        }
        tv.T0[(int64_t)c * tv.ld_t + i] = v;
    }
}

__global__ __launch_bounds__(kThreads) void k_tab_price_init(TableauView tv, const double* __restrict__ w,
                                                             const double* __restrict__ cost_store) {
    __shared__ double s_partial[4 * kVecPerBlock];
    const int v0 = tv.c_lo + blockIdx.x * kVecPerBlock;
    double dot = 0.0;
    block_multi_dot(tv.T0, tv.ld_t, tv.m, v0, tv.c_hi, w, s_partial, dot);
    const int c = v0 + threadIdx.x;
    if (threadIdx.x < kVecPerBlock && c < tv.c_hi) tv.d[c] = cost_store[c] - dot;
}

__global__ void k_tab_basis_costs(const int32_t* __restrict__ basis_indices, const double* __restrict__ cost_store,
                                  int col_off, int n_store, int m, double* __restrict__ w) {
    const int i = blockIdx.x * blockDim.x + threadIdx.x;
    if (i >= m) return;
    const int j = basis_indices[i];
    const int c = j + col_off;
    w[i] = (j < kWrappedArtificialBase && c >= 0 && c < n_store) ? cost_store[c] : 0.0;
}

__global__ __launch_bounds__(kThreads) void k_tab_scan(TableauView tv, SelectPartials sp, const PivotRecord* rec) {
    if (rec->outcome != DEV_RUNNING) return;
    const int c = tv.c_lo + blockIdx.x * kThreads + threadIdx.x;
    const int j = c - tv.col_off;
    double key = INFINITY;
    int kj = 0x7fffffff;
    if (c < tv.c_hi && j >= 0 && j < tv.n) {
        const double v = tv.d[c];
        if (!sp.in_basis[j] && v < -sp.tol_cost) { key = select_key(sp.rule, sp.n, rec, j, v); kj = j; }
    }
    block_partial_min(key, kj, sp, blockIdx.x);
}

__global__ __launch_bounds__(kSingleBlock) void k_tab_select(TableauView tv, SelectPartials sp, int count,
                                                             PivotRecord* rec) {
    if (rec->outcome != DEV_RUNNING) return;
    double k1 = INFINITY;
    int bj = 0x7fffffff;
    if ((int)threadIdx.x < count) { k1 = sp.k1[threadIdx.x]; bj = sp.j[threadIdx.x]; }
    tab_select_entering<kSingleBlock>(tv, sp, count, k1, bj);
    if (threadIdx.x == 0) {
        if (bj == 0x7fffffff) {
            rec->outcome = DEV_NO_CANDIDATE;
            if (sp.rule == 1) rec->last_selected = -1;
        } else {
            rec->q = bj;
            rec->d_q = tv.d[bj + tv.col_off];
            rec->key1 = k1;
            if (sp.rule == 1) rec->last_selected = bj;
        }
    }
}

template <int B>
__global__ __launch_bounds__(kThreads) void k_tab_column(TableauView tv, DeferredUpdate du, double* __restrict__ alpha,
                                                         const PivotRecord* rec) {
    if (rec->outcome != DEV_RUNNING) return;
    __shared__ double s_vs[kMaxEta];
    const int p = rec->n_eta;
    const int cq = rec->q + tv.col_off;
    if ((int)threadIdx.x < p) s_vs[threadIdx.x] = tv.R0[(int64_t)threadIdx.x * tv.ld_r + cq];
    __syncthreads();
    const int i = blockIdx.x * kThreads + threadIdx.x;
    if (i >= tv.m) return;
    double a = tv.T0[(int64_t)cq * tv.ld_t + i];
    for_pending<B>(du.W, du.ld, i, p, [&](int j, double w) { a = fma(w, s_vs[j], a); });
    alpha[i] = a;
}

template <int B>
__device__ __forceinline__ void tab_row_update_core(const TableauView& tv, const DeferredUpdate& du, const SelectPartials& sp,
                                                    const PivotRecord& R, int block, const double* s_wr, int p_old, int jt, int r,
                                                    int q, int leaving, double d_q, double alpha_r) {
    const PivotRecord* rec = &R;
    const int c = tv.c_lo + block * kThreads + threadIdx.x;
    const double d_old = c < tv.c_hi ? tv.d[c] : 0.0;
    __syncthreads();
    double key = INFINITY;
    int kj = 0x7fffffff;
    if (c < tv.c_hi) {
        double base;
        if (jt < p_old) base = tv.R0[(int64_t)jt * tv.ld_r + c];
        else {
            base = tv.T0[(int64_t)c * tv.ld_t + r];
            tv.R0[(int64_t)jt * tv.ld_r + c] = base;
        }
        double row = base;
        for_pending<B>(tv.R0, tv.ld_r, c, p_old, [&](int j, double r0) { row = fma(s_wr[j], r0, row); });
        const double theta = d_q / alpha_r;
        const int j = c - tv.col_off;
        double dn = fma(-theta, row, d_old);
        if (j == q) dn = 0.0;
        tv.d[c] = dn;
        if (j >= 0 && j < tv.n) {
            const bool basic = (j == q) || (sp.in_basis[j] && j != leaving);
            if (!basic && dn < -sp.tol_cost) { key = select_key(sp.rule, sp.n, rec, j, dn); kj = j; }
        }
    }
    block_partial_min(key, kj, sp, block);
}

template <int B>
__device__ __forceinline__ void tab_row_update_body(const TableauView& tv, const DeferredUpdate& du,
                                                    const SelectPartials& sp, const PivotRecord& R, int block) {
    __shared__ double s_wr[kMaxEta];
    if ((int)threadIdx.x < du.kmax) s_wr[threadIdx.x] = du.wr[threadIdx.x];
    tab_row_update_core<B>(tv, du, sp, R, block, s_wr, R.n_eta_old, R.eta_target, R.r, R.q, R.leaving, R.d_q, R.alpha_r);
}

template <int B>
__global__ __launch_bounds__(kThreads) void k_tab_row_update(TableauView tv, DeferredUpdate du, SelectPartials sp,
                                                             PivotRecord* rec) {
    const PivotRecord R = *rec;
    if (R.outcome != DEV_RUNNING) return;
    tab_row_update_body<B>(tv, du, sp, R, blockIdx.x);
}

template <int B>
__device__ __forceinline__ void tab_update_w_vectors_body(const DeferredUpdate& du, int m, const double* __restrict__ alpha,
                                                          double* __restrict__ b, int32_t* __restrict__ basis_indices,
                                                          uint8_t* __restrict__ in_basis, int32_t* __restrict__ trace,
                                                          int64_t trace_cap, const PivotRecord& R, PivotRecord* rec,
                                                          int block) {
    __shared__ double s_wr2[kMaxEta];
    const int p_old = R.n_eta_old, jt = R.eta_target, r = R.r;
    if ((int)threadIdx.x < du.kmax) s_wr2[threadIdx.x] = du.wr[threadIdx.x];
    const int i = block * kThreads + threadIdx.x;
    const double a_i = i < m ? alpha[i] : 0.0;
    const double b_i = i < m ? b[i] : 0.0;
    __syncthreads();
    const double ar = R.alpha_r;
    const double br = R.b_r / ar;
    if (i < m) {
        const double a = a_i;
        const double u = (i == r) ? (1.0 / ar - 1.0) : (-a / ar);
        tab_update_w_row<B>(du, i, u, s_wr2, 0, p_old);
        double* tgt = du.W + (int64_t)jt * du.ld + i;
        if (jt < p_old) *tgt += u; else *tgt = u;
        b[i] = pivot_b(a, b_i, br, i == r);
    }
    if (i == 0) {
        basis_indices[r] = R.q;
        pivot_bookkeeping(R.phase, R.iterations, R.minus_objective, R.d_q, br, R.q, r, R.leaving, in_basis, trace, trace_cap, rec);
    }
}

template <int B>
__global__ __launch_bounds__(kThreads) void k_tab_update_all(TableauView tv, DeferredUpdate du, SelectPartials sp,
                                                             int nb_row, int m, const double* __restrict__ alpha,
                                                             double* __restrict__ b, int32_t* __restrict__ basis_indices,
                                                             uint8_t* __restrict__ in_basis, int32_t* __restrict__ trace,
                                                             int64_t trace_cap, PivotRecord* rec) {
    const PivotRecord R = *rec;
    if (R.outcome != DEV_RUNNING) return;
    if ((int)blockIdx.x < nb_row) tab_row_update_body<B>(tv, du, sp, R, blockIdx.x);
    else tab_update_w_vectors_body<B>(du, m, alpha, b, basis_indices, in_basis, trace, trace_cap, R, rec, blockIdx.x - nb_row);
}

template <int B>
__global__ __launch_bounds__(kThreads) void k_tab_ratio_update_all(TableauView tv, DeferredUpdate du, SelectPartials sp, int nb_row,
                                                                   int m, const double* alpha,
                                                                   const double* __restrict__ b_in, double* __restrict__ b_out,
                                                                   const int32_t* __restrict__ basis_in,
                                                                   int32_t* __restrict__ basis_out, uint8_t* in_basis,
                                                                   int32_t* __restrict__ trace, int64_t trace_cap, Tolerances tol,
                                                                   const double* rmin, int nblk,
                                                                   double* __restrict__ shadow, int32_t* __restrict__ shadow_meta,
                                                                   PivotRecord* rec, const double* __restrict__ msgs, int count,
                                                                   int64_t msg_len, int rule, int split) {
    const double first = (!msgs && (int)threadIdx.x < nblk) ? rmin[threadIdx.x] : INFINITY;
    PivotRecord R = *rec;
    const bool w_half = (int)blockIdx.x >= nb_row;
    const int part = w_half ? ((int)blockIdx.x - nb_row) / nblk : 0;
    const int wblock = (int)blockIdx.x - nb_row - part * nblk;
    const int i = wblock * kThreads + threadIdx.x;
    const bool lead = w_half && part == 0;
    const bool mine = lead && i < m;
    if (R.outcome != DEV_RUNNING) {
        if (mine) { b_out[i] = b_in[i]; basis_out[i] = basis_in[i]; }
        return;
    }
    if (msgs) {
        int q_win = 0;
        double d_win = 0.0;
        const int win = candidate_winner_staged(msgs, count, msg_len, rule, tol.tie, &q_win, &d_win);
        if (win < 0) {
            if (mine) { b_out[i] = b_in[i]; basis_out[i] = basis_in[i]; }
            if (lead && wblock == 0 && threadIdx.x == 0) record_candidate(rec, rule, -1, 0, 0.0);
            return;
        }
        R.q = q_win;
        R.d_q = d_win;
        if (rule == 1) R.last_selected = R.q;
        alpha = msgs + win * msg_len + 3;
        rmin = alpha + m;
    }
    int r, leaving;
    ratio_blocks_pick<kThreads>(alpha, b_in, basis_in, m, tol, rmin, nblk, &r, &leaving, first, !msgs);
    if (r < 0) {
        if (mine) { b_out[i] = b_in[i]; basis_out[i] = basis_in[i]; }
        if (lead && wblock == 0 && threadIdx.x == 0) rec->outcome = DEV_NO_ROW;
        return;
    }
    __shared__ double s_wr[kMaxEta];
    __shared__ double s_ab[2];
    __shared__ int s_jt;
    const int p_old = R.p_now;
    if ((int)threadIdx.x < p_old) s_wr[threadIdx.x] = du.W[(int64_t)threadIdx.x * du.ld + r];
    if (threadIdx.x == 0) {
        s_ab[0] = alpha[r]; s_ab[1] = b_in[r];
        const int slot = du.pos_of_row[r];
        s_jt = slot < 0 ? p_old : slot;
    }
    __syncthreads();
    const double alpha_r = s_ab[0], b_r = s_ab[1];
    const int jt = s_jt, q = R.q;
    if (!w_half) {
        tab_row_update_core<B>(tv, du, sp, R, blockIdx.x, s_wr, p_old, jt, r, q, leaving, R.d_q, alpha_r);
        return;
    }
    const double br = b_r / alpha_r;
    const int share = (p_old + split - 1) / split;
    const int j_lo = min(part * share, p_old), j_hi = min(j_lo + share, p_old);
    if (!lead) {
        if (i < m && i != r) {
            const double u = -alpha[i] / alpha_r;
            tab_update_w_row<B>(du, i, u, s_wr, j_lo, j_hi);
            if (jt >= j_lo && jt < j_hi) du.W[(int64_t)jt * du.ld + i] += u;
        }
        return;
    }
    if (i < m) {
        const double a = alpha[i], b_i = b_in[i];
        const double u = (i == r) ? (1.0 / alpha_r - 1.0) : (-a / alpha_r);
        if (i != r) {
            tab_update_w_row<B>(du, i, u, s_wr, j_lo, j_hi);
            double* tgt = du.W + (int64_t)jt * du.ld + i;
            if (jt >= p_old) *tgt = u;
            else if (jt < j_hi) *tgt += u;
        } else {
            for (int j = 0; j < p_old; ++j) {
                const double w = s_wr[j];
                shadow[j] = (u != 0.0 && w != 0.0) ? fma(u, w, w) : w;
            }
            if (jt < p_old) shadow[jt] += u; else shadow[jt] = u;
            shadow_meta[0] = r;
            shadow_meta[1] = jt < p_old ? p_old : p_old + 1;
        }
        b_out[i] = pivot_b(a, b_i, br, i == r);
        basis_out[i] = (i == r) ? q : basis_in[i];
    }
    if (i == 0) {
        if (msgs) record_candidate(rec, rule, 0, q, R.d_q);
        rec->r = r; rec->leaving = leaving; rec->alpha_r = alpha_r; rec->b_r = b_r;
        rec->n_eta_old = p_old; rec->eta_target = jt;
        if (jt >= p_old) { du.S[p_old] = r; du.pos_of_row[r] = p_old; rec->n_eta = p_old + 1; }
        pivot_bookkeeping(R.phase, R.iterations, R.minus_objective, R.d_q, br, q, r, leaving, in_basis, trace, trace_cap, rec);
    }
}

__global__ void k_tab_apply_shadow(DeferredUpdate du, double* __restrict__ shadow, int32_t* __restrict__ shadow_meta) {
    const int row = shadow_meta[0], len = shadow_meta[1];
    if (row < 0) return;
    for (int j = threadIdx.x; j < len; j += blockDim.x) du.W[(int64_t)j * du.ld + row] = shadow[j];
    __syncthreads();
    if (threadIdx.x == 0) shadow_meta[0] = -1;
}

template <int B>
__global__ __launch_bounds__(kThreads) void k_tab_select_column(TableauView tv, DeferredUpdate du, SelectPartials sp,
                                                                int count, double* alpha, double* msg,
                                                                const double* b, Tolerances tol,
                                                                double* rmin, PivotRecord* rec,
                                                                const double* shadow, int32_t* shadow_meta) {
    const int outcome = rec->outcome, p = rec->n_eta;
    if (shadow_meta) {
        const int srow = shadow_meta[0], slen = shadow_meta[1];
        if (srow >= 0 && srow / kThreads == (int)blockIdx.x) {
            if ((int)threadIdx.x < slen) du.W[(int64_t)threadIdx.x * du.ld + srow] = shadow[threadIdx.x];
            __syncthreads();
            if (threadIdx.x == 0) shadow_meta[0] = -1;
        }
        if (blockIdx.x == 0 && threadIdx.x == 0) rec->p_now = p;
    }
    double k1 = INFINITY;
    int bj = 0x7fffffff;
    if ((int)threadIdx.x < count) { k1 = sp.k1[threadIdx.x]; bj = sp.j[threadIdx.x]; }
    const int i = blockIdx.x * kThreads + threadIdx.x;
    const double b_i = (rmin && i < tv.m) ? b[i] : 0.0;
    if (outcome != DEV_RUNNING) return;
    __shared__ double s_vs[kMaxEta];
    __shared__ double s_min[kThreads / 64];
    tab_select_entering<kThreads>(tv, sp, count, k1, bj);
    if (bj == 0x7fffffff) {
        if (msg) {
            if (i < tv.m) alpha[i] = 0.0;
            if (i == 0) { msg[0] = INFINITY; msg[1] = 0.0; msg[2] = 0.0; }
        } else if (blockIdx.x == 0 && threadIdx.x == 0) {
            rec->outcome = DEV_NO_CANDIDATE;
            if (sp.rule == 1) rec->last_selected = -1;
        }
        return;
    }
    const int cq = bj + tv.col_off;
    if (blockIdx.x == 0 && threadIdx.x == 0) {
        if (msg) { msg[0] = k1; msg[1] = (double)bj; msg[2] = tv.d[cq]; }
        else {
            rec->q = bj;
            rec->d_q = tv.d[cq];
            rec->key1 = k1;
            if (sp.rule == 1) rec->last_selected = bj;
        }
    }
    if ((int)threadIdx.x < p) s_vs[threadIdx.x] = tv.R0[(int64_t)threadIdx.x * tv.ld_r + cq];
    const double t0 = i < tv.m ? tv.T0[(int64_t)cq * tv.ld_t + i] : 0.0;
    __syncthreads();
    double ratio = INFINITY;
    if (i < tv.m) {
        double a = t0;
        for_pending<B>(du.W, du.ld, i, p, [&](int j, double w) { a = fma(w, s_vs[j], a); });
        alpha[i] = a;
        const double bz = b_i <= tol.zero ? 0.0 : b_i;
        if (a > tol.pivot) ratio = bz / a;
    }
    if (!rmin) return;
#pragma unroll
    for (int off = 32; off > 0; off >>= 1) ratio = fmin(ratio, __shfl_down(ratio, off, 64));
    if ((threadIdx.x & 63) == 0) s_min[threadIdx.x >> 6] = ratio;
    __syncthreads();
    if (threadIdx.x == 0) rmin[blockIdx.x] = fmin(fmin(s_min[0], s_min[1]), fmin(s_min[2], s_min[3]));
}

__global__ __launch_bounds__(kSingleBlock) void k_ratio_blocks(const double* __restrict__ alpha, const double* __restrict__ b,
                                                               const int32_t* __restrict__ basis_indices, int m,
                                                               Tolerances tol, DeferredUpdate du,
                                                               const double* __restrict__ rmin, int nblk, PivotRecord* rec) {
    const int outcome = rec->outcome, p = rec->n_eta;
    const double first = (int)threadIdx.x < nblk ? rmin[threadIdx.x] : INFINITY;
    if (outcome != DEV_RUNNING) return;
    ratio_blocks_body<kSingleBlock>(alpha, b, basis_indices, m, tol, du, rmin, nblk, p, rec, first, true);
}

__global__ __launch_bounds__(kSingleBlock) void k_tab_select_candidate_ratio(const double* __restrict__ msgs, int count,
                                                                             int64_t msg_len, int m, double* __restrict__ alpha,
                                                                             const double* __restrict__ b,
                                                                             const int32_t* __restrict__ basis_indices,
                                                                             int rule, Tolerances tol, DeferredUpdate du,
                                                                             int forced_row, PivotRecord* rec) {
    const int outcome = rec->outcome, p = rec->n_eta;
    if (outcome != DEV_RUNNING) return;
    int q = 0;
    double d_q = 0.0;
    const int win = candidate_winner_staged(msgs, count, msg_len, rule, tol.tie, &q, &d_q);
    if (threadIdx.x == 0) record_candidate(rec, rule, win, q, d_q);
    if (win < 0) return;
    const double* __restrict__ col = msgs + win * msg_len + 3;
    const int nblk = (m + kThreads - 1) / kThreads;
    if (forced_row >= 0) {
        for (int i = threadIdx.x; i < m; i += kSingleBlock) alpha[i] = col[i];
        ratio_commit_row<kSingleBlock>(forced_row, basis_indices[forced_row], col, b, du, p, rec);
        return;
    }
    const double first = (int)threadIdx.x < nblk ? col[m + threadIdx.x] : INFINITY;
    constexpr int kCopy = 16;
    double cp[kCopy];
#pragma unroll
    for (int u = 0; u < kCopy; ++u) {
        const int i = threadIdx.x + u * kSingleBlock;
        cp[u] = i < m ? col[i] : 0.0;
    }
    ratio_blocks_body<kSingleBlock>(col, b, basis_indices, m, tol, du, col + m, nblk, p, rec, first, true);
#pragma unroll
    for (int u = 0; u < kCopy; ++u) {
        const int i = threadIdx.x + u * kSingleBlock;
        if (i < m) alpha[i] = cp[u];
    }
    for (int i = threadIdx.x + kCopy * kSingleBlock; i < m; i += kSingleBlock) alpha[i] = col[i];
}

__global__ void k_tab_update_vectors(int m, const double* __restrict__ alpha, double* __restrict__ b,
                                     int32_t* __restrict__ basis_indices, uint8_t* __restrict__ in_basis,
                                     int32_t* __restrict__ trace, int64_t trace_cap, PivotRecord* rec) {
    if (rec->outcome != DEV_RUNNING) return;
    const int i = blockIdx.x * blockDim.x + threadIdx.x;
    const int r = rec->r;
    const double br = rec->b_r / rec->alpha_r;
    if (i < m) b[i] = pivot_b(alpha[i], b[i], br, i == r);
    if (i == 0) {
        basis_indices[r] = rec->q;
        pivot_bookkeeping(rec->phase, rec->iterations, rec->minus_objective, rec->d_q, br, rec->q, r, rec->leaving, in_basis, trace,
                          trace_cap, rec);
    }
}
// ... 201 lines not shown
    before = s_before[0] + s_before[1] + s_before[2] + s_before[3];
    const unsigned long long mask = fl.mask[blockIdx.x];
    if ((mask >> lane) & 1ull) {
        const int c = tv.c_lo + blockIdx.x * 64 + lane;
        const int x = before + __popcll(mask & ((1ull << lane) - 1ull));
        if (wave == 0) fl.cols[x] = c;
        for (int j0 = wave; j0 < p; j0 += 4 * 8) {
            double v[8];
#pragma unroll
            for (int u = 0; u < 8; ++u) v[u] = j0 + 4 * u < p ? tv.R0[(int64_t)(j0 + 4 * u) * tv.ld_r + c] : 0.0;
#pragma unroll
            for (int u = 0; u < 8; ++u)
                if (j0 + 4 * u < p) fl.R0c[(int64_t)(j0 + 4 * u) * fl.ld + x] = v[u];
        }
    }
    if ((int)blockIdx.x == nb - 1 && threadIdx.x == 0) {
        const int count = before + __popcll(mask);
        *fl.count = count;
        fl.stats[0] += 1;
        fl.stats[1] += count;
    }
}

__global__ void k_tab_gather_columns(TableauView tv, const int32_t* __restrict__ cols, double* __restrict__ out) {
    const int64_t total = (int64_t)tv.m * tv.m;
    for (int64_t idx = (int64_t)blockIdx.x * blockDim.x + threadIdx.x; idx < total; idx += (int64_t)gridDim.x * blockDim.x) {
        const int k = (int)(idx / tv.m), i = (int)(idx % tv.m);
        out[(int64_t)i * tv.m + k] = tv.T0[(int64_t)cols[k] * tv.ld_t + i];
    }
}

template <int B>
__global__ __launch_bounds__(kThreads) void k_tab_row(TableauView tv, DeferredUpdate du, int row, double* __restrict__ out,
                                                      const PivotRecord* rec) {
    __shared__ double s_w[kMaxEta];
    const int p = rec->n_eta;
    if ((int)threadIdx.x < p) s_w[threadIdx.x] = du.W[(int64_t)threadIdx.x * du.ld + row];
    __syncthreads();
    const int c = tv.c_lo + blockIdx.x * kThreads + threadIdx.x;
    if (c >= tv.c_hi) return;
    double v = tv.T0[(int64_t)c * tv.ld_t + row];
    for_pending<B>(tv.R0, tv.ld_r, c, p, [&](int j, double r0) { v = fma(s_w[j], r0, v); });
    out[c - tv.c_lo] = v;
}

template <int B>
__global__ __launch_bounds__(kThreads) void k_tab_zero_level_scan(TableauView tv, DeferredUpdate du, SelectPartials sp, int row,
                                                                  int nr_artificial, Tolerances tol, const PivotRecord* rec) {
    const int outcome = rec->outcome, p = rec->n_eta;
    if (outcome != DEV_RUNNING) return;
    __shared__ double s_w[kMaxEta];
    if ((int)threadIdx.x < p) s_w[threadIdx.x] = du.W[(int64_t)threadIdx.x * du.ld + row];
    __syncthreads();
    const int c = tv.c_lo + blockIdx.x * kThreads + threadIdx.x;
    const int j = c - tv.col_off;
    double key = INFINITY;
    int kj = 0x7fffffff;
    if (c < tv.c_hi && j >= nr_artificial && j < tv.n && !sp.in_basis[j] && fabs(tv.d[c]) <= tol.cost) {
        double v = tv.T0[(int64_t)c * tv.ld_t + row];
        for_pending<B>(tv.R0, tv.ld_r, c, p, [&](int k, double r0) { v = fma(s_w[k], r0, v); });
        if (fabs(v) > tol.pivot) { key = (double)j; kj = j; }
    }
    block_partial_min(key, kj, sp, blockIdx.x);
}

int32_t tab_scan_blocks(int32_t n_owned_columns) { return cdiv(n_owned_columns, kThreads); }

int32_t tab_load_batch(int32_t wanted) {
    return (wanted == 1 || wanted == 8 || wanted == 16 || wanted == 32) ? wanted : kTabLoadBatchDefault;
}

template <class Launch>
static void with_load_batch(int32_t batch, Launch&& launch) {
    switch (tab_load_batch(batch)) {
    case 1:  launch(std::integral_constant<int, 1>{}); break;
    case 16: launch(std::integral_constant<int, 16>{}); break;
    case 32: launch(std::integral_constant<int, 32>{}); break;
    default: launch(std::integral_constant<int, 8>{}); break;
    }
    static_assert(kTabLoadBatchDefault == 8, "the default of tab_load_batch is the switch's default case");
}

void launch_tab_build(const TableauView& tv, const double* A, int64_t ld_a, const ColumnTable& ct, hipStream_t s) {
    const int64_t total = (int64_t)tv.m * (tv.c_hi - tv.c_lo);
    if (total <= 0) return;
    hipLaunchKernelGGL(k_tab_build, dim3(element_blocks(total)), dim3(256), 0, s, tv, A, ld_a, ct);
}

void launch_tab_price_init(const TableauView& tv, const double* w, const double* cost_store, hipStream_t s) {
    if (tv.c_hi <= tv.c_lo) return;
    hipLaunchKernelGGL(k_tab_price_init, dim3(cdiv(tv.c_hi - tv.c_lo, kVecPerBlock)), dim3(kThreads), 0, s, tv, w,
                       cost_store);
}

void launch_tab_basis_costs(const TableauView& tv, const int32_t* basis_indices, const double* cost_store, double* w,
                            hipStream_t s) {
    hipLaunchKernelGGL(k_tab_basis_costs, dim3(cdiv(tv.m, 256)), dim3(256), 0, s, basis_indices, cost_store, tv.col_off,
                       tv.n_store, tv.m, w);
}

void launch_tab_scan(const TableauView& tv, SelectPartials sp, const PivotRecord* rec, hipStream_t s) {
    if (tv.c_hi <= tv.c_lo) return;
    hipLaunchKernelGGL(k_tab_scan, dim3(tab_scan_blocks(tv.c_hi - tv.c_lo)), dim3(kThreads), 0, s, tv, sp, rec);
}

void launch_tab_select(const TableauView& tv, SelectPartials sp, int32_t count, PivotRecord* rec, hipStream_t s) {
    hipLaunchKernelGGL(k_tab_select, dim3(1), dim3(kSingleBlock), 0, s, tv, sp, count, rec);
}

void launch_tab_column(const TableauView& tv, const DeferredUpdate& du, double* alpha, const PivotRecord* rec,
                       hipStream_t s) {
    with_load_batch(du.batch, [&](auto B) {
        hipLaunchKernelGGL((k_tab_column<decltype(B)::value>), dim3(cdiv(tv.m, kThreads)), dim3(kThreads), 0, s, tv, du, alpha, rec);
    });
}

void launch_tab_row_update(const TableauView& tv, const DeferredUpdate& du, SelectPartials sp, PivotRecord* rec,
                           hipStream_t s) {
    if (tv.c_hi <= tv.c_lo) return;
    with_load_batch(du.batch, [&](auto B) {
        hipLaunchKernelGGL((k_tab_row_update<decltype(B)::value>), dim3(tab_scan_blocks(tv.c_hi - tv.c_lo)), dim3(kThreads), 0, s, tv, du, sp,
                           rec);
    });
}

void launch_tab_update_vectors(int32_t m, const double* alpha, double* b, int32_t* basis_indices, uint8_t* in_basis,
                               int32_t* trace, int64_t trace_cap, PivotRecord* rec, hipStream_t s) {
    hipLaunchKernelGGL(k_tab_update_vectors, dim3(cdiv(m, 256)), dim3(256), 0, s, m, alpha, b, basis_indices, in_basis,
                       trace, trace_cap, rec);
}

void launch_tab_select_column_rmin(const TableauView& tv, const DeferredUpdate& du, SelectPartials sp, int32_t count,
                                   double* alpha, const double* b, Tolerances tol, double* rmin, PivotRecord* rec,
                                   hipStream_t s, const double* shadow, int32_t* shadow_meta) {
    with_load_batch(du.batch, [&](auto B) {
        hipLaunchKernelGGL((k_tab_select_column<decltype(B)::value>), dim3(cdiv(tv.m, kThreads)), dim3(kThreads), 0, s, tv, du, sp, count, alpha,
                           (double*)nullptr, b, tol, rmin, rec, shadow, shadow_meta);
    });
}

void launch_tab_ratio_update_all(const TableauView& tv, const DeferredUpdate& du, SelectPartials sp, int32_t m,
                                 const double* alpha, const double* b_in, double* b_out, const int32_t* basis_in,
                                 int32_t* basis_out, uint8_t* in_basis, int32_t* trace, int64_t trace_cap, Tolerances tol,
                                 const double* rmin, double* shadow, int32_t* shadow_meta, PivotRecord* rec, hipStream_t s,
                                 const double* msgs, int32_t count, int64_t msg_len, int32_t rule) {
    const int nb_row = tv.c_hi > tv.c_lo ? tab_scan_blocks(tv.c_hi - tv.c_lo) : 0;
    const int nb_w = cdiv(m, kThreads);
    int split = tab_load_batch(du.batch) == 1 ? 1 : std::max(1, std::min({(int)du.w_split, (int)du.kmax, (kTabSplitCUs - nb_row) / nb_w}));
    with_load_batch(du.batch, [&](auto B) {
        hipLaunchKernelGGL((k_tab_ratio_update_all<decltype(B)::value>), dim3(nb_row + split * nb_w), dim3(kThreads), 0, s, tv, du, sp, nb_row, m,
                           alpha, b_in, b_out, basis_in, basis_out, in_basis, trace, trace_cap, tol, rmin, nb_w, shadow,
                           shadow_meta, rec, msgs, (int)count, msg_len, (int)rule, split);
    });
}

void launch_tab_apply_shadow(const DeferredUpdate& du, double* shadow, int32_t* shadow_meta, hipStream_t s) {
    hipLaunchKernelGGL(k_tab_apply_shadow, dim3(1), dim3(128), 0, s, du, shadow, shadow_meta);
}

void launch_ratio_blocks(const double* alpha, const double* b, const int32_t* basis_indices, int32_t m, Tolerances tol,
                         const DeferredUpdate& du, const double* rmin, PivotRecord* rec, hipStream_t s) {
    hipLaunchKernelGGL(k_ratio_blocks, dim3(1), dim3(kSingleBlock), 0, s, alpha, b, basis_indices, m, tol, du, rmin,
                       cdiv(m, kThreads), rec);
}

void launch_tab_select_column_msg(const TableauView& tv, const DeferredUpdate& du, SelectPartials sp, int32_t count,
                                  double* msg, const double* b, Tolerances tol, PivotRecord* rec, hipStream_t s,
                                  const double* shadow, int32_t* shadow_meta) {
    with_load_batch(du.batch, [&](auto B) {
        hipLaunchKernelGGL((k_tab_select_column<decltype(B)::value>), dim3(cdiv(tv.m, kThreads)), dim3(kThreads), 0, s, tv, du, sp, count, msg + 3,
                           msg, b, tol, msg + 3 + tv.m, rec, shadow, shadow_meta);
    });
}

void launch_tab_select_candidate_ratio(const double* msgs, int32_t count, int64_t msg_len, int32_t m, double* alpha,
                                       const double* b, const int32_t* basis_indices, int32_t rule, Tolerances tol,
                                       const DeferredUpdate& du, int32_t forced_row, PivotRecord* rec, hipStream_t s) {
    hipLaunchKernelGGL(k_tab_select_candidate_ratio, dim3(1), dim3(kSingleBlock), 0, s, msgs, count, msg_len, m, alpha, b,
                       basis_indices, rule, tol, du, forced_row, rec);
}

void launch_tab_zero_level_scan(const TableauView& tv, const DeferredUpdate& du, SelectPartials sp, int32_t row,
                                int32_t nr_artificial, Tolerances tol, const PivotRecord* rec, hipStream_t s) {
    if (tv.c_hi <= tv.c_lo) return;
    with_load_batch(du.batch, [&](auto B) {
        hipLaunchKernelGGL((k_tab_zero_level_scan<decltype(B)::value>), dim3(tab_scan_blocks(tv.c_hi - tv.c_lo)), dim3(kThreads), 0, s, tv, du, sp,
                           row, nr_artificial, tol, rec);
    });
}

void launch_tab_update_all(const TableauView& tv, const DeferredUpdate& du, SelectPartials sp, int32_t m,
                           const double* alpha, double* b, int32_t* basis_indices, uint8_t* in_basis, int32_t* trace,
                           int64_t trace_cap, PivotRecord* rec, hipStream_t s) {
    const int nb_row = tv.c_hi > tv.c_lo ? tab_scan_blocks(tv.c_hi - tv.c_lo) : 0;
    const int nb_w = cdiv(m, kThreads);
    with_load_batch(du.batch, [&](auto B) {
        hipLaunchKernelGGL((k_tab_update_all<decltype(B)::value>), dim3(nb_row + nb_w), dim3(kThreads), 0, s, tv, du, sp, nb_row, m, alpha, b,
                           basis_indices, in_basis, trace, trace_cap, rec);
    });
}

void launch_tab_flush(const TableauView& tv, const DeferredUpdate& du, const PivotRecord* rec, const FlushList& fl,
                      hipStream_t s) {
    if (tv.c_hi <= tv.c_lo) return;
    const int ncols = tv.c_hi - tv.c_lo;
    const int32_t* p_dev = &rec->n_eta;
    if ((int64_t)ncols * tv.m >= (1 << 16)) {
        constexpr int WC = 2, WR = 4, KC = 16;
        dim3 grid(cdiv(tv.m, WR * 32), cdiv(ncols, WC * 64));
        if (fl.cols) {
            const int nb = cdiv(ncols, 64);
            hipLaunchKernelGGL(k_tab_flush_mark, dim3(nb), dim3(kThreads), 0, s, tv, fl, p_dev);
            hipLaunchKernelGGL(k_tab_flush_compact, dim3(nb), dim3(kThreads), 0, s, tv, fl, p_dev, nb);
            hipLaunchKernelGGL((k_tab_flush_lds<WC, WR, KC, true>), grid, dim3(WC * WR * 64), 0, s, tv, du, p_dev, fl);
        } else {
            hipLaunchKernelGGL((k_tab_flush_lds<WC, WR, KC, false>), grid, dim3(WC * WR * 64), 0, s, tv, du, p_dev, fl);
        }
        return;
    }
    constexpr int MT = 4, NT = 2;
    dim3 grid(cdiv(ncols, 2 * 16 * MT), cdiv(tv.m, 2 * 16 * NT));
    hipLaunchKernelGGL((k_tab_flush<MT, NT>), grid, dim3(kThreads), 0, s, tv, du, p_dev, fl.stats);
}

void launch_tab_gather_columns(const TableauView& tv, const int32_t* cols, double* out, hipStream_t s) {
    const int64_t total = (int64_t)tv.m * tv.m;
    hipLaunchKernelGGL(k_tab_gather_columns, dim3(element_blocks(total)), dim3(256), 0, s, tv, cols, out);
}

void launch_tab_row(const TableauView& tv, const DeferredUpdate& du, int32_t row, double* out, const PivotRecord* rec,
                    hipStream_t s) {
    if (tv.c_hi <= tv.c_lo) return;
    with_load_batch(du.batch, [&](auto B) {
        hipLaunchKernelGGL((k_tab_row<decltype(B)::value>), dim3(tab_scan_blocks(tv.c_hi - tv.c_lo)), dim3(kThreads), 0, s, tv, du, row, out, rec);
    });
}


}
```

rust-lp_amd/engine.py:

```python
from __future__ import annotations

import ctypes as C
import os
from typing import List, Optional, Tuple

import numpy as np

from .matrix_data import MatrixData

_HERE = os.path.dirname(os.path.abspath(__file__))
LIB_PATH = os.path.join(_HERE, "librelp_engine.so")

FIRST_PROFITABLE, FIRST_PROFITABLE_WITH_MEMORY, STEEPEST_DESCENT = 0, 1, 2
RUNNING, OPTIMAL, UNBOUNDED, INFEASIBLE, PHASE_ONE_DONE, NO_ROW_PHASE_ONE = range(6)
OUTCOME_NAMES = {RUNNING: "running", OPTIMAL: "optimal", UNBOUNDED: "unbounded", INFEASIBLE: "infeasible",
                 PHASE_ONE_DONE: "phase_one_done", NO_ROW_PHASE_ONE: "no_row_phase_one"}
(K_PRICE, K_SELECT_COLUMN, K_BUILD_COLUMN, K_FTRAN, K_RATIO, K_UPDATE_VECTORS, K_UPDATE_INVERSE, K_APPLY_W,
 K_UPDATE_W, K_FLUSH, K_FT_RUN) = range(11)
KERNEL_NAMES = ["price", "select_column", "build_column", "ftran", "ratio", "update_vectors", "update_inverse",
                "apply_w", "update_w", "flush", "ft_run"]
ENGINE_REVISED, ENGINE_TABLEAU, ENGINE_LU, ENGINE_AUTO = 0, 1, 2, 3
RATIO_REFERENCE, RATIO_LARGEST_PIVOT = 0, 1
ARTIFICIAL_REFERENCE, ARTIFICIAL_TEXTBOOK = 0, 1
E_ARG, E_HIP, E_ZERO_PIVOT, E_SINGULAR, E_STATE, E_UNSUPPORTED, E_ALLOC = -1, -2, -3, -4, -5, -6, -7
FORMAT_CSC, FORMAT_DENSE = 0, 1
MEM_HOST, MEM_DEVICE = 0, 1


class RelpError(RuntimeError):
    pass


class _MatrixData(C.Structure):
    _fields_ = [("nr_normal", C.c_int32), ("nr_eq", C.c_int32), ("nr_range", C.c_int32), ("nr_le", C.c_int32),
                ("nr_ge", C.c_int32), ("format", C.c_int32), ("matrix_memory", C.c_int32),
                ("col_ptr", C.c_void_p), ("row_idx", C.c_void_p), ("values", C.c_void_p),
                ("dense", C.c_void_p), ("dense_ld", C.c_int64),
                ("b", C.c_void_p), ("ranges", C.c_void_p), ("cost", C.c_void_p), ("upper_bound", C.c_void_p)]


class Config(C.Structure):
    _fields_ = [("device", C.c_int32), ("phase_one_rule", C.c_int32), ("phase_two_rule", C.c_int32),
                ("tol_cost", C.c_double), ("tol_pivot", C.c_double), ("tol_zero", C.c_double),
                ("tol_tie", C.c_double), ("tol_feas", C.c_double),
                ("poll_interval", C.c_int32), ("trace_capacity", C.c_int32),
                ("shard_rank", C.c_int32), ("shard_count", C.c_int32),
                ("update_block", C.c_int32), ("engine", C.c_int32),
                ("ratio_rule", C.c_int32), ("artificial_removal", C.c_int32),
                ("pivot_rescue", C.c_int32), ("auto_reinversion", C.c_int32)]


_SIGNATURES = {
    "relp_default_config": (None, [C.POINTER(Config)]),
    "relp_robust_config": (None, [C.POINTER(Config)]),
    "relp_engine_kind": (C.c_int32, [C.c_void_p]),
    "relp_robust_stats": (C.c_int, [C.c_void_p, C.POINTER(C.c_int64)]),
    "relp_last_error": (C.c_char_p, [C.c_void_p]),
    "relp_version": (C.c_char_p, []),
    "relp_engine_create": (C.c_int, [C.POINTER(_MatrixData), C.POINTER(Config), C.POINTER(C.c_void_p)]),
    "relp_engine_destroy": (None, [C.c_void_p]),
    "relp_set_stream": (C.c_int, [C.c_void_p, C.c_void_p]),
    "relp_select_primal_pivot_column": (C.c_int, [C.c_void_p, C.c_int32, C.POINTER(C.c_int32), C.POINTER(C.c_int32),
                                                  C.POINTER(C.c_double)]),
    "relp_relative_costs": (C.c_int, [C.c_void_p, C.c_void_p]),
    "relp_generate_column": (C.c_int, [C.c_void_p, C.c_int32, C.c_void_p]),
    "relp_generate_element": (C.c_int, [C.c_void_p, C.c_int32, C.c_int32, C.POINTER(C.c_double)]),
    "relp_select_primal_pivot_row": (C.c_int, [C.c_void_p, C.POINTER(C.c_int32), C.POINTER(C.c_int32)]),
    "relp_select_primal_pivot_row_of": (C.c_int, [C.c_void_p, C.POINTER(C.c_double), C.POINTER(C.c_int32), C.POINTER(C.c_int32)]),
    "relp_bring_into_basis": (C.c_int, [C.c_void_p, C.c_int32, C.c_int32, C.c_double, C.POINTER(C.c_int32)]),
    "relp_run": (C.c_int, [C.c_void_p, C.c_int64, C.POINTER(C.c_int64), C.POINTER(C.c_int32)]),
    "relp_solve_relaxation": (C.c_int, [C.c_void_p, C.c_int64, C.POINTER(C.c_int32)]),
    "relp_from_basis": (C.c_int, [C.c_void_p, C.c_void_p]),
    "relp_flush": (C.c_int, [C.c_void_p]),
    "relp_update_block": (C.c_int32, [C.c_void_p]),
    "relp_tab_load_batch": (C.c_int32, [C.c_void_p]),
    "relp_tab_flush_stats": (C.c_int, [C.c_void_p, C.POINTER(C.c_int64)]),
    "relp_lu_stats": (C.c_int, [C.c_void_p, C.POINTER(C.c_int64)]),
    "relp_lu_lookahead_stats": (C.c_int, [C.c_void_p, C.POINTER(C.c_int64)]),
    "relp_lu_kernel_layout": (C.c_int, [C.c_void_p, C.POINTER(C.c_int32)]),
    "relp_lu_set_device_factorisation": (C.c_int, [C.c_void_p, C.c_int32]),
    "relp_lu_device_factorisation_stats": (C.c_int, [C.c_void_p, C.POINTER(C.c_int64)]),
    "relp_lu_factor_residual": (C.c_int, [C.c_void_p, C.POINTER(C.c_double)]),
    "relp_lu_phase_cycles": (C.c_int, [C.c_void_p, C.POINTER(C.c_int64)]),
    "relp_basis_inverse_row": (C.c_int, [C.c_void_p, C.c_int32, C.c_void_p]),
    "relp_should_refactor": (C.c_int, [C.c_void_p, C.POINTER(C.c_int32)]),
    "relp_generate_column_of": (C.c_int, [C.c_void_p, C.c_void_p, C.c_void_p, C.c_int32, C.c_void_p]),
    "relp_cost_difference_of": (C.c_int, [C.c_void_p, C.c_void_p, C.c_void_p, C.c_int32, C.POINTER(C.c_double)]),
    "relp_lu_change_basis": (C.c_int, [C.c_void_p, C.c_int32]),
    "relp_lu_set_factors": (C.c_int, [C.c_void_p] + [C.c_void_p] * 6),
    "relp_lu_updates": (C.c_int, [C.c_void_p, C.POINTER(C.c_int32)]),
    "relp_lu_get_update": (C.c_int, [C.c_void_p, C.c_int32, C.POINTER(C.c_int32), C.c_void_p, C.c_void_p, C.c_int32, C.POINTER(C.c_int32)]),
    "relp_lu_get_upper": (C.c_int, [C.c_void_p, C.c_void_p, C.c_void_p, C.c_void_p, C.c_int64, C.POINTER(C.c_int64)]),
    "relp_shard_flush_begin": (C.c_int, [C.c_void_p, C.POINTER(C.c_void_p), C.POINTER(C.c_int64)]),
    "relp_shard_flush_end": (C.c_int, [C.c_void_p]),
    "relp_nr_rows": (C.c_int32, [C.c_void_p]),
    "relp_nr_columns": (C.c_int32, [C.c_void_p]),
    "relp_phase": (C.c_int32, [C.c_void_p]),
    "relp_nr_artificial": (C.c_int32, [C.c_void_p]),
    "relp_get_objective": (C.c_int, [C.c_void_p, C.POINTER(C.c_double)]),
    "relp_get_b": (C.c_int, [C.c_void_p, C.c_void_p]),
    "relp_get_minus_pi": (C.c_int, [C.c_void_p, C.c_void_p]),
    "relp_get_basis_indices": (C.c_int, [C.c_void_p, C.c_void_p]),
    "relp_get_basis_inverse": (C.c_int, [C.c_void_p, C.c_void_p]),
    "relp_current_bfs": (C.c_int, [C.c_void_p, C.c_void_p, C.c_void_p, C.c_int32, C.POINTER(C.c_int32)]),
    "relp_get_iterations": (C.c_int, [C.c_void_p, C.POINTER(C.c_int64)]),
    "relp_get_degenerate_pivots": (C.c_int, [C.c_void_p, C.POINTER(C.c_int64)]),
    "relp_get_trace": (C.c_int, [C.c_void_p, C.c_void_p, C.c_void_p, C.c_void_p, C.c_void_p, C.c_int64,
                                 C.POINTER(C.c_int64)]),
    "relp_check_basis": (C.c_int, [C.c_void_p, C.POINTER(C.c_double), C.POINTER(C.c_double), C.POINTER(C.c_double)]),
    "relp_profile_enable": (C.c_int, [C.c_void_p, C.c_int32, C.c_int64, C.c_int32]),
    "relp_profile_read": (C.c_int, [C.c_void_p, C.c_int32, C.POINTER(C.c_int64), C.POINTER(C.c_double)]),
    "relp_synth_fill_dense": (C.c_int, [C.c_void_p, C.c_int64, C.c_int32, C.c_int32, C.c_uint64, C.c_int64, C.c_void_p]),
    "relp_device_alloc": (C.c_int, [C.POINTER(C.c_void_p), C.c_int64]),
    "relp_device_free": (C.c_int, [C.c_void_p]),
    "relp_shard_ranges": (C.c_int, [C.c_void_p] + [C.POINTER(C.c_int32)] * 5),
    "relp_shard_column_range": (None, [C.c_int32, C.c_int32, C.c_int32, C.POINTER(C.c_int32), C.POINTER(C.c_int32)]),
    "relp_shard_candidate_len": (C.c_int64, [C.c_void_p]),
    "relp_shard_rho_len": (C.c_int64, [C.c_void_p]),
    "relp_shard_price": (C.c_int, [C.c_void_p, C.c_void_p]),
    "relp_shard_select_column": (C.c_int, [C.c_void_p, C.c_void_p, C.c_int32]),
    "relp_shard_ftran": (C.c_int, [C.c_void_p, C.c_void_p]),
    "relp_shard_ratio": (C.c_int, [C.c_void_p, C.c_void_p, C.c_int32, C.c_void_p]),
    "relp_shard_update": (C.c_int, [C.c_void_p, C.c_void_p]),
    "relp_poll": (C.c_int, [C.c_void_p, C.POINTER(C.c_int32), C.POINTER(C.c_int64)]),
    "relp_shard_pivot": (C.c_int, [C.c_void_p]),
    "relp_set_reinversion_interval": (C.c_int, [C.c_void_p, C.c_int64]),
    "relp_reinversions": (C.c_int64, [C.c_void_p]),
    "relp_shard_set_collectives": (C.c_int, [C.c_void_p, C.c_void_p, C.c_void_p, C.c_void_p]),
# ... 161 lines not shown

    def generate_column(self, j: int) -> np.ndarray:
        out = np.zeros(self.nr_rows())
        self._ck(self._lib.relp_generate_column(self._h, j, out.ctypes.data))
        return out

    def generate_element(self, i: int, j: int) -> float:
        v = C.c_double()
        self._ck(self._lib.relp_generate_element(self._h, i, j, C.byref(v)))
        return v.value

    def set_reinversion_interval(self, pivots: int) -> None:
        self._ck(self._lib.relp_set_reinversion_interval(self._h, int(pivots)))

    def reinversions(self) -> int:
        return int(self._lib.relp_reinversions(self._h))

    def select_primal_pivot_row(self, column=None) -> Optional[int]:
        found, row = C.c_int32(), C.c_int32()
        if column is None:
            self._ck(self._lib.relp_select_primal_pivot_row(self._h, C.byref(found), C.byref(row)))
        else:
            col = np.ascontiguousarray(column, dtype=np.float64)
            if col.shape != (self.nr_rows(),):
                raise ValueError("column must have nr_rows() entries")
            self._ck(self._lib.relp_select_primal_pivot_row_of(self._h, col.ctypes.data_as(C.POINTER(C.c_double)),
                                                              C.byref(found), C.byref(row)))
        return row.value if found.value else None

    def bring_into_basis(self, column: int, row: int, cost: float) -> int:
        leaving = C.c_int32()
        self._ck(self._lib.relp_bring_into_basis(self._h, column, row, cost, C.byref(leaving)))
        return leaving.value

    def run(self, max_iters: int) -> Tuple[int, int]:
        done, oc = C.c_int64(), C.c_int32()
        self._ck(self._lib.relp_run(self._h, max_iters, C.byref(done), C.byref(oc)))
        return done.value, oc.value

    def solve_relaxation(self, max_iters: int = 1 << 40) -> int:
        oc = C.c_int32()
        self._ck(self._lib.relp_solve_relaxation(self._h, max_iters, C.byref(oc)))
        return oc.value

    def flush(self) -> None:
        self._ck(self._lib.relp_flush(self._h))

    def update_block(self) -> int:
        return self._lib.relp_update_block(self._h)

    def load_batch(self) -> int:
        return self._lib.relp_tab_load_batch(self._h)

    def flush_stats(self) -> Tuple[int, int]:
        out = (C.c_int64 * 2)()
        self._ck(self._lib.relp_tab_flush_stats(self._h, out))
        return int(out[0]), int(out[1])

    def engine_kind(self) -> int:
        return int(self._lib.relp_engine_kind(self._h))

    def robust_stats(self) -> dict:
        out = (C.c_int64 * 4)()
        self._ck(self._lib.relp_robust_stats(self._h, out))
        return dict(zip(("small_pivots", "columns_barred", "confirmations", "reinversion_interval"), (int(v) for v in out)))

    def lu_stats(self) -> dict:
        out = (C.c_int64 * 8)()
        self._ck(self._lib.relp_lu_stats(self._h, out))
        keys = ("refactorisations", "m", "nnz_l", "nnz_u", "levels_l", "levels_u", "levels_ut", "levels_lt")
        stats = dict(zip(keys, (int(v) for v in out)))
        la = (C.c_int64 * 4)()
        self._ck(self._lib.relp_lu_lookahead_stats(self._h, la))
        stats.update(lookahead_installs=int(la[0]), replayed_changes=int(la[1]), lookahead=int(la[2]), fuse_lanes=int(la[3]))
        return stats

    def lu_kernel_layout(self) -> dict:
        out = (C.c_int32 * 4)()
        self._ck(self._lib.relp_lu_kernel_layout(self._h, out))
        return {"persistent_kernel": bool(out[0]), "layout": int(out[1]), "tail_slots": int(out[2]), "grid_price": bool(out[3])}

    def lu_set_device_factorisation(self, on: bool) -> None:
        self._ck(self._lib.relp_lu_set_device_factorisation(self._h, 1 if on else 0))

    def lu_factor_residual(self) -> float:
        out = C.c_double()
        self._ck(self._lib.relp_lu_factor_residual(self._h, C.byref(out)))
        return out.value

    def lu_device_factorisation_stats(self) -> dict:
        out = (C.c_int64 * 6)()
        self._ck(self._lib.relp_lu_device_factorisation_stats(self._h, out))
        keys = ("enabled", "device_factorisations", "host_fallbacks", "kernel_us", "last_bump", "last_peeled")
        return dict(zip(keys, (int(v) for v in out)))

    def basis_inverse_row(self, row: int) -> np.ndarray:
        out = np.zeros(self.nr_rows())
        self._ck(self._lib.relp_basis_inverse_row(self._h, row, out.ctypes.data))
        return out

    def should_refactor(self) -> bool:
        v = C.c_int32()
        self._ck(self._lib.relp_should_refactor(self._h, C.byref(v)))
        return bool(v.value)

    @staticmethod
# ... 219 lines not shown
```

Baseline: 45450 iterations/s.

## Add adaptive tableau geometry: split pending-eta work across thread groups with relay

Introduces a geometry rule that picks rows per block for the column-select kernel and columns per slot for the row scan/update kernels, based on m, owned columns and w_split. When fewer rows or columns are assigned per block, the pending eta updates are split into shares across thread groups, and a partial accumulator is relayed between groups through shared memory with barriers. The aim is to launch more blocks and fill more CUs on the per-iteration kernels. The cost is extra barriers, shared-memory handoffs and more template instantiations.

```diff
diff --git a/include/relp_engine.h b/include/relp_engine.h
--- a/include/relp_engine.h
+++ b/include/relp_engine.h
@@ -113,6 +113,9 @@
 relp_status_t relp_flush(relp_engine_t *h);
 relp_status_t relp_tab_flush_stats(relp_engine_t *h, int64_t *out2);
 int32_t       relp_tab_load_batch(const relp_engine_t *h);
+relp_status_t relp_tab_geometry(const relp_engine_t *h, int32_t out[2]);
+void          relp_tab_geometry_rule(int32_t m, int32_t n_owned, int32_t w_split, int32_t want_rows, int32_t want_cols,
+                                     int32_t out[2]);
 int32_t       relp_update_block(const relp_engine_t *h);
 relp_status_t relp_lu_stats(const relp_engine_t *h, int64_t *out8);
 relp_status_t relp_lu_lookahead_stats(const relp_engine_t *h, int64_t *out4);
diff --git a/rust-lp_amd/csrc/relp_abi.cpp b/rust-lp_amd/csrc/relp_abi.cpp
--- a/rust-lp_amd/csrc/relp_abi.cpp
+++ b/rust-lp_amd/csrc/relp_abi.cpp
@@ -81,6 +81,8 @@
 int64_t relp_reinversions(const relp_engine_t* h) { return h ? H(h).reinversions() : -1; }
 int32_t relp_update_block(const relp_engine_t* h) { return h ? H(h).update_block() : -1; }
 int32_t relp_tab_load_batch(const relp_engine_t* h) { return h ? H(h).tab_load_batch_size() : -1; }
+relp_status_t relp_tab_geometry(const relp_engine_t* h, int32_t* out2) { if (!h || !out2) return RELP_E_ARG; H(h).tab_geometry_read(out2); return RELP_OK; }
+void relp_tab_geometry_rule(int32_t m, int32_t n_owned, int32_t w_split, int32_t want_rows, int32_t want_cols, int32_t* out2) { if (out2) relp::tab_geometry(m, n_owned, w_split, want_rows, want_cols, out2); }
 relp_status_t relp_lu_stats(const relp_engine_t* h, int64_t* out8) { return (h && out8) ? H(h).lu_stats(out8) : RELP_E_ARG; }
 relp_status_t relp_lu_lookahead_stats(const relp_engine_t* h, int64_t* out4) { return (h && out4) ? H(h).lu_lookahead_stats(out4) : RELP_E_ARG; }
 relp_status_t relp_lu_kernel_layout(const relp_engine_t* h, int32_t* out4) { return (h && out4) ? H(h).lu_kernel_layout(out4) : RELP_E_ARG; }
diff --git a/rust-lp_amd/csrc/relp_device_common.h b/rust-lp_amd/csrc/relp_device_common.h
--- a/rust-lp_amd/csrc/relp_device_common.h
+++ b/rust-lp_amd/csrc/relp_device_common.h
@@ -120,7 +120,7 @@
 template <int BS>
 __device__ __forceinline__ void tab_select_entering(const TableauView& tv, const SelectPartials& sp, int count, double& k1,
                                                     int& bj) {
-    constexpr int kListMax = 32, kGroups = BS / kThreads;
+    constexpr int kListMax = 32;
     __shared__ int s_list[kListMax];
     __shared__ int s_cnt;
     __shared__ int s_low[BS / 64];
@@ -140,10 +140,11 @@
     }
     __syncthreads();
     const int listed = s_cnt;
-    const int grp = threadIdx.x / kThreads, u = threadIdx.x % kThreads;
+    const int shift = sp.slot_cols == 128 ? 7 : 8, groups = BS >> shift;
+    const int grp = threadIdx.x >> shift, u = threadIdx.x & ((1 << shift) - 1);
     int lowest = 0x7fffffff;
     auto scan_slot = [&](int t) {
-        const int c = tv.c_lo + t * kThreads + u;
+        const int c = tv.c_lo + (t << shift) + u;
         const int j = c - tv.col_off;
         if (c < tv.c_hi && j >= 0 && j < tv.n) {
             const double v = tv.d[c];
@@ -151,9 +152,9 @@
         }
     };
     if (listed <= kListMax) {
-        for (int i = grp; i < listed; i += kGroups) scan_slot(s_list[i]);
-    } else {
-        for (int t = grp; t < count; t += kGroups)
+        for (int i = grp; i < listed; i += groups) scan_slot(s_list[i]);
+    } else {
+        for (int t = grp; t < count; t += groups)
             if (sp.k1[t] <= bound) scan_slot(t);
     }
 #pragma unroll
@@ -228,6 +229,7 @@
 }
 
 static constexpr int kMaxEta = 128;
+static_assert(tab_shares_tile(kMaxEta), "tab_share: ascending, disjoint shares that cover [0, p), and one share when p <= B");
 
 typedef unsigned long long tie_key_t;
 static constexpr tie_key_t kNoTieKey = ~0ull;
diff --git a/rust-lp_amd/csrc/relp_engine.cpp b/rust-lp_amd/csrc/relp_engine.cpp
--- a/rust-lp_amd/csrc/relp_engine.cpp
+++ b/rust-lp_amd/csrc/relp_engine.cpp
@@ -56,13 +56,14 @@
     SelectPartials sp;
     sp.k1 = d_part_k1_; sp.j = d_part_j_; sp.in_basis = d_in_basis_; sp.tol_cost = cfg_.tol_cost; sp.rule = rule;
     sp.n = nr_columns(); sp.offset = 0; sp.nb_struct = 0; sp.tol_tie = cfg_.tol_tie; sp.p_lo = 0; sp.cols_per_slot = 8;
+    sp.slot_cols = slot_cols_;
     return sp;
 }
 
 DeferredUpdate Engine::deferred() const {
     DeferredUpdate du;
     du.W = d_W_; du.ld = ld_b_; du.kmax = block_; du.S = d_S_; du.pos_of_row = d_pos_of_row_; du.wr = d_wr_; du.R = d_R_;
-    du.batch = load_batch_; du.w_split = w_split_;
+    du.batch = load_batch_; du.w_split = w_split_; du.col_rows = col_rows_;
     return du;
 }
 
@@ -98,6 +99,8 @@
     s.tab_flush_all = num("RELP_TAB_FLUSH_ALL", 0) != 0;
     s.tab_load_batch = num("RELP_TAB_LOAD_BATCH", 0);
     s.tab_w_split = num("RELP_TAB_W_SPLIT", 0);
+    s.tab_col_rows = num("RELP_TAB_COL_ROWS", 0);
+    s.tab_slot_cols = num("RELP_TAB_SLOT_COLS", 0);
     s.fused_update = num("RELP_FUSED_UPDATE", 1) != 0;
     s.lu_lookahead_set = given("RELP_LU_LOOKAHEAD");
     s.lu_lookahead = num("RELP_LU_LOOKAHEAD", 8);
@@ -199,7 +202,7 @@
     HIP_TRY(d_rec_.alloc(1));
     {
         const int64_t slots = price_structural_blocks(lay_.col_lo, lay_.col_hi) + (lay_.nr_artificial + lay_.nr_virtual + 255) / 256 + 8 +
-                              tab_scan_blocks(n_alloc_) + price_csc_blocks(0, lay_.nr_normal);
+                              tab_scan_blocks(n_alloc_, 128) + price_csc_blocks(0, lay_.nr_normal);
         HIP_TRY(d_part_k1_.alloc(slots));
         HIP_TRY(d_part_j_.alloc(slots));
     }
@@ -236,6 +239,11 @@
         {
             load_batch_ = tab_load_batch(sw_.tab_load_batch);
             w_split_ = sw_.tab_w_split >= 1 ? std::min(sw_.tab_w_split, 16) : kTabSplitDefault;
+        }
+        {
+            int32_t g[2];
+            tab_geometry(lay_.m, (int32_t)n_owned, w_split_, cfg_.shard_count > 1 ? 256 : sw_.tab_col_rows, sw_.tab_slot_cols, g);
+            col_rows_ = g[0]; slot_cols_ = g[1];
         }
         {
             fused_update_ = sw_.fused_update;
@@ -375,7 +383,7 @@
     const SelectPartials sp = tab_partials(rule);
     if (fused_update_ && in_loop_) {
         prof_begin(RELP_K_FTRAN);
-        launch_tab_select_column_rmin(tv, du, sp, tab_scan_blocks(lay_.sc_hi - lay_.sc_lo), d_alpha_, d_b_, tolerances(), d_rmin_,
+        launch_tab_select_column_rmin(tv, du, sp, tab_slots(), d_alpha_, d_b_, tolerances(), d_rmin_,
                                       d_rec_, stream_, d_shadow_, d_shadow_meta_);
         prof_end();
         prof_begin(RELP_K_PRICE);
@@ -390,7 +398,7 @@
     }
     tab_settle();
     prof_begin(RELP_K_FTRAN);
-    launch_tab_select_column_rmin(tv, du, sp, tab_scan_blocks(lay_.sc_hi - lay_.sc_lo), d_alpha_, d_b_, tolerances(), d_rmin_,
+    launch_tab_select_column_rmin(tv, du, sp, tab_slots(), d_alpha_, d_b_, tolerances(), d_rmin_,
                                   d_rec_, stream_);
     prof_end();
     prof_begin(RELP_K_RATIO);
@@ -538,7 +546,7 @@
     if (tableau_) {
         const SelectPartials sp = tab_partials(rule);
         launch_tab_scan(tview(), sp, d_rec_, stream_);
-        launch_tab_select(tview(), sp, tab_scan_blocks(lay_.sc_hi - lay_.sc_lo), d_rec_, stream_);
+        launch_tab_select(tview(), sp, tab_slots(), d_rec_, stream_);
     } else {
         enqueue_price(phase_, d_minus_pi_, d_rec_, lay_.col_lo, lay_.col_hi);
         launch_select_column(d_d_, d_in_basis_, nr_columns(), rule, cfg_.tol_cost, cfg_.tol_tie, d_rec_, stream_);
diff --git a/rust-lp_amd/csrc/relp_engine.hpp b/rust-lp_amd/csrc/relp_engine.hpp
--- a/rust-lp_amd/csrc/relp_engine.hpp
+++ b/rust-lp_amd/csrc/relp_engine.hpp
@@ -55,6 +55,7 @@
     bool pivot_guard_set = false; double pivot_guard = 0.0;
     bool tab_flush_all = false;
     int tab_load_batch = 0, tab_w_split = 0;
+    int tab_col_rows = 0, tab_slot_cols = 0;
     bool fused_update = true;
     bool lu_lookahead_set = false; int lu_lookahead = 8;
     int fuse_lanes = 256;
@@ -144,6 +145,7 @@
     relp_status_t get_degenerate_pivots(int64_t* out);
     relp_status_t tab_flush_stats(int64_t* out2);
     int32_t tab_load_batch_size() const { return tableau_ ? load_batch_ : 0; }
+    void tab_geometry_read(int32_t out[2]) const { out[0] = tableau_ ? col_rows_ : 0; out[1] = tableau_ ? slot_cols_ : 0; }
     relp_status_t get_trace(int32_t* phase, int32_t* entering, int32_t* row, int32_t* leaving, int64_t cap,
                             int64_t* count);
     relp_status_t check_basis(double* max_identity_error, double* max_basic_cost, double* min_b);
@@ -198,6 +200,8 @@
     DeviceBuf<double> d_R0c_;
     FlushList flush_list() const;
     int32_t load_batch_ = 0, w_split_ = 0;
+    int32_t col_rows_ = 256, slot_cols_ = 256;
+    int32_t tab_slots() const { return tab_scan_blocks(lay_.sc_hi - lay_.sc_lo, slot_cols_); }
     DeviceBuf<double> d_cost_store_;
     DeviceBuf<int32_t> d_idcol_;
     bool fused_update_ = false, shadow_pending_ = false;
diff --git a/rust-lp_amd/csrc/relp_engine_shard.cpp b/rust-lp_amd/csrc/relp_engine_shard.cpp
--- a/rust-lp_amd/csrc/relp_engine_shard.cpp
+++ b/rust-lp_amd/csrc/relp_engine_shard.cpp
@@ -34,7 +34,7 @@
         const SelectPartials sp = tab_partials(rule);
         if (!tab_partials_valid_) { launch_tab_scan(tv, sp, d_rec_, stream_); tab_partials_valid_ = true; }
         prof_begin(RELP_K_FTRAN);
-        launch_tab_select_column_msg(tv, deferred(), sp, tab_scan_blocks(lay_.sc_hi - lay_.sc_lo), dev_candidate, d_b_, tolerances(), d_rec_,
+        launch_tab_select_column_msg(tv, deferred(), sp, tab_slots(), dev_candidate, d_b_, tolerances(), d_rec_,
                                      stream_);
         prof_end();
         return RELP_OK;
@@ -167,7 +167,7 @@
         Tolerances zt = tolerances();
         if (textbook) zt.cost = INFINITY;
         launch_tab_zero_level_scan(tv, du, sp, pivot_row, lay_.nr_artificial, zt, d_rec_, stream_);
-        launch_tab_select_column_msg(tv, du, sp, tab_scan_blocks(lay_.sc_hi - lay_.sc_lo), d_msg_cand_, d_b_, tolerances(), d_rec_, stream_);
+        launch_tab_select_column_msg(tv, du, sp, tab_slots(), d_msg_cand_, d_b_, tolerances(), d_rec_, stream_);
         if (coll_allgather_(coll_ctx_, d_msg_cand_, d_msg_cands_, lay_.candidate_len * (int64_t)sizeof(double), stream_))
             return fail(RELP_E_HIP, "all-gather of the zero-level candidates failed");
         launch_tab_select_candidate_ratio(d_msg_cands_, g, lay_.candidate_len, lay_.m, d_alpha_, d_b_, d_basis_, RELP_RULE_FIRST_PROFITABLE,
@@ -218,7 +218,7 @@
         const SelectPartials sp = tab_partials(rule);
         if (!tab_partials_valid_) { launch_tab_scan(tv, sp, d_rec_, stream_); tab_partials_valid_ = true; }
         prof_begin(RELP_K_FTRAN);
-        launch_tab_select_column_msg(tv, du, sp, tab_scan_blocks(lay_.sc_hi - lay_.sc_lo), d_msg_cand_, d_b_, tolerances(), d_rec_, stream_,
+        launch_tab_select_column_msg(tv, du, sp, tab_slots(), d_msg_cand_, d_b_, tolerances(), d_rec_, stream_,
                                      d_shadow_, d_shadow_meta_);
         prof_end();
         if (coll_allgather_(coll_ctx_, d_msg_cand_, d_msg_cands_, lay_.candidate_len * (int64_t)sizeof(double), stream_))
diff --git a/rust-lp_amd/csrc/relp_kernels.h b/rust-lp_amd/csrc/relp_kernels.h
--- a/rust-lp_amd/csrc/relp_kernels.h
+++ b/rust-lp_amd/csrc/relp_kernels.h
@@ -41,6 +41,7 @@
     double*  R;
     int32_t  batch;
     int32_t  w_split;
+    int32_t  col_rows;
 };
 
 struct ColumnTable {
@@ -70,6 +71,7 @@
     double         tol_tie;
     int32_t        p_lo;
     int32_t        cols_per_slot;
+    int32_t        slot_cols;
 };
 
 struct LuRow { int32_t k, e0, e1, pad_; double diag; };
@@ -282,7 +284,7 @@
 void launch_tab_basis_costs(const TableauView& tv, const int32_t* basis_indices, const double* cost_store, double* w,
                             hipStream_t s);
 void launch_tab_scan(const TableauView& tv, SelectPartials sp, const PivotRecord* rec, hipStream_t s);
-int32_t tab_scan_blocks(int32_t n_owned_columns);
+int32_t tab_scan_blocks(int32_t n_owned_columns, int32_t slot_cols);
 bool launch_lu_ftran_cols(const DeviceLU& lu, const TableauView& tv, const double* A, int64_t ld_a, const ColumnTable& ct,
                           int32_t c_first, int32_t c_count, hipStream_t s);
 void launch_tab_select(const TableauView& tv, SelectPartials sp, int32_t count, PivotRecord* rec, hipStream_t s);
@@ -320,6 +322,35 @@
 static constexpr int32_t kTabSplitDefault = 2;
 static constexpr int32_t kTabSplitCUs = 256;
 int32_t tab_load_batch(int32_t wanted);
+void tab_geometry(int32_t m, int32_t n_owned, int32_t w_split, int32_t want_rows, int32_t want_cols, int32_t out[2]);
+struct TabShare { int lo, hi; };
+constexpr TabShare tab_share(int p, int parts, int part, int B) {
+    const int per = ((p + B - 1) / B + parts - 1) / parts * B;
+    const int lo = part * per < p ? part * per : p;
+    return TabShare{lo, lo + per < p ? lo + per : p};
+}
+constexpr int tab_share_count(int p, int parts, int B) {
+    const int per = ((p + B - 1) / B + parts - 1) / parts * B;
+    return per > 0 ? (p + per - 1) / per : 1;
+}
+constexpr bool tab_shares_tile(int p_max) {
+    const int batches[] = {1, 8, 16, 32}, groups[] = {1, 2, 4};
+    for (int B : batches)
+        for (int parts : groups)
+            for (int p = 0; p <= p_max; ++p) {
+                int at = 0;
+                const int count = tab_share_count(p, parts, B);
+                for (int part = 0; part < parts; ++part) {
+                    const TabShare s = tab_share(p, parts, part, B);
+                    if (s.lo != at || s.hi < s.lo || s.hi > p) return false;
+                    if ((s.hi > s.lo) != (part < count) && !(p == 0 && part == 0)) return false;
+                    at = s.hi;
+                }
+                if (at != p) return false;
+                if (p <= B && (tab_share(p, parts, 0, B).hi != p || count != 1)) return false;
+            }
+    return true;
+}
 void launch_tab_flush(const TableauView& tv, const DeferredUpdate& du, const PivotRecord* rec, const FlushList& fl,
                       hipStream_t s);
 void launch_tab_ratio_update_all(const TableauView& tv, const DeferredUpdate& du, SelectPartials sp, int32_t m,
diff --git a/rust-lp_amd/csrc/relp_kernels_tableau.hip b/rust-lp_amd/csrc/relp_kernels_tableau.hip
--- a/rust-lp_amd/csrc/relp_kernels_tableau.hip
+++ b/rust-lp_amd/csrc/relp_kernels_tableau.hip
@@ -22,6 +22,65 @@
 #pragma unroll
         for (int t = 0; t < B; ++t)
             if (j0 + t < n) use(j0 + t, v[t]);
+    }
+}
+
+template <int B, int PARTS, class Use>
+__device__ __forceinline__ bool for_pending_relay(const double* base, int64_t stride, int64_t x, int p, bool valid, double& acc,
+                                                  double* s_hand, Use&& use) {
+    if constexpr (PARTS == 1) {
+        if (valid) for_pending<B>(base, stride, x, p, use);
+        return true;
+    } else {
+        constexpr int G = kThreads / PARTS;
+        constexpr int kHold = 64 / (B * PARTS) > 1 ? 64 / (B * PARTS) : 1;
+        static_assert(G % 64 == 0, "a group is whole wavefronts: its share is uniform in a wavefront");
+        const int g = __builtin_amdgcn_readfirstlane((int)threadIdx.x / G), u = (int)threadIdx.x % G;
+        const int last = tab_share_count(p, PARTS, B) - 1;
+        if (last == 0) {
+            if (g == 0 && valid) for_pending<B>(base, stride, x, p, use);
+            return g == 0;
+        }
+        const TabShare sh = tab_share(p, PARTS, g, B);
+        double v[kHold * B];
+        if (valid) {
+#pragma unroll
+            for (int h = 0; h < kHold; ++h) {
+                const int j0 = sh.lo + h * B;
+                if (j0 + B <= sh.hi) {
+#pragma unroll
+                    for (int t = 0; t < B; ++t) v[h * B + t] = base[(int64_t)(j0 + t) * stride + x];
+                } else if (j0 < sh.hi) {
+#pragma unroll
+                    for (int t = 0; t < B; ++t) v[h * B + t] = base[(int64_t)min(j0 + t, sh.hi - 1) * stride + x];
+                }
+            }
+        }
+        for (int turn = 0; turn <= last; ++turn) {
+            if (g == turn && valid) {
+                int lo = sh.lo, hi = sh.hi;
+                asm volatile("" : "+s"(lo), "+s"(hi));
+                if (turn > 0) acc = s_hand[u];
+#pragma unroll
+                for (int h = 0; h < kHold; ++h) {
+                    const int j0 = lo + h * B;
+                    if (j0 + B <= hi) {
+#pragma unroll
+                        for (int t = 0; t < B; ++t) use(j0 + t, v[h * B + t]);
+                    } else {
+#pragma unroll
+                        for (int t = 0; t < B; ++t)
+                            if (j0 + t < hi) use(j0 + t, v[h * B + t]);
+                    }
+                }
+                const int held = lo + kHold * B;
+                if (held < hi)
+                    for_pending<B>(base + (int64_t)held * stride, stride, x, hi - held, [&](int j, double e) { use(held + j, e); });
+                if (turn < last) s_hand[u] = acc;
+            }
+            if (turn < last) __syncthreads();
+        }
+        return g == last;
     }
 }
 
@@ -78,7 +137,7 @@
 
 __global__ __launch_bounds__(kThreads) void k_tab_scan(TableauView tv, SelectPartials sp, const PivotRecord* rec) {
     if (rec->outcome != DEV_RUNNING) return;
-    const int c = tv.c_lo + blockIdx.x * kThreads + threadIdx.x;
+    const int c = (int)threadIdx.x < sp.slot_cols ? tv.c_lo + blockIdx.x * sp.slot_cols + (int)threadIdx.x : tv.c_hi;
     const int j = c - tv.col_off;
     double key = INFINITY;
     int kj = 0x7fffffff;
@@ -125,25 +184,29 @@
     alpha[i] = a;
 }
 
-template <int B>
+template <int B, int PARTS>
 __device__ __forceinline__ void tab_row_update_core(const TableauView& tv, const DeferredUpdate& du, const SelectPartials& sp,
                                                     const PivotRecord& R, int block, const double* s_wr, int p_old, int jt, int r,
                                                     int q, int leaving, double d_q, double alpha_r) {
     const PivotRecord* rec = &R;
-    const int c = tv.c_lo + block * kThreads + threadIdx.x;
+    constexpr int C = kThreads / PARTS;
+    __shared__ double s_hand[PARTS > 1 ? C : 1];
+    const int c = tv.c_lo + block * C + (int)threadIdx.x % C;
     const double d_old = c < tv.c_hi ? tv.d[c] : 0.0;
     __syncthreads();
     double key = INFINITY;
     int kj = 0x7fffffff;
-    if (c < tv.c_hi) {
-        double base;
-        if (jt < p_old) base = tv.R0[(int64_t)jt * tv.ld_r + c];
+    double row = 0.0;
+    if ((int)threadIdx.x < C && c < tv.c_hi) {
+        if (jt < p_old) row = tv.R0[(int64_t)jt * tv.ld_r + c];
         else {
-            base = tv.T0[(int64_t)c * tv.ld_t + r];
-            tv.R0[(int64_t)jt * tv.ld_r + c] = base;
-        }
-        double row = base;
-        for_pending<B>(tv.R0, tv.ld_r, c, p_old, [&](int j, double r0) { row = fma(s_wr[j], r0, row); });
+            row = tv.T0[(int64_t)c * tv.ld_t + r];
+            tv.R0[(int64_t)jt * tv.ld_r + c] = row;
+        }
+    }
+    const bool ends = for_pending_relay<B, PARTS>(tv.R0, tv.ld_r, c, p_old, c < tv.c_hi, row, s_hand,
+                                                  [&](int j, double r0) { row = fma(s_wr[j], r0, row); });
+    if (ends && c < tv.c_hi) {
         const double theta = d_q / alpha_r;
         const int j = c - tv.col_off;
         double dn = fma(-theta, row, d_old);
@@ -157,20 +220,20 @@
     block_partial_min(key, kj, sp, block);
 }
 
-template <int B>
+template <int B, int PARTS>
 __device__ __forceinline__ void tab_row_update_body(const TableauView& tv, const DeferredUpdate& du,
                                                     const SelectPartials& sp, const PivotRecord& R, int block) {
     __shared__ double s_wr[kMaxEta];
     if ((int)threadIdx.x < du.kmax) s_wr[threadIdx.x] = du.wr[threadIdx.x];
-    tab_row_update_core<B>(tv, du, sp, R, block, s_wr, R.n_eta_old, R.eta_target, R.r, R.q, R.leaving, R.d_q, R.alpha_r);
-}
-
-template <int B>
+    tab_row_update_core<B, PARTS>(tv, du, sp, R, block, s_wr, R.n_eta_old, R.eta_target, R.r, R.q, R.leaving, R.d_q, R.alpha_r);
+}
+
+template <int B, int PARTS>
 __global__ __launch_bounds__(kThreads) void k_tab_row_update(TableauView tv, DeferredUpdate du, SelectPartials sp,
                                                              PivotRecord* rec) {
     const PivotRecord R = *rec;
     if (R.outcome != DEV_RUNNING) return;
-    tab_row_update_body<B>(tv, du, sp, R, blockIdx.x);
+    tab_row_update_body<B, PARTS>(tv, du, sp, R, blockIdx.x);
 }
 
 template <int B>
@@ -202,7 +265,7 @@
     }
 }
 
-template <int B>
+template <int B, int PARTS>
 __global__ __launch_bounds__(kThreads) void k_tab_update_all(TableauView tv, DeferredUpdate du, SelectPartials sp,
                                                              int nb_row, int m, const double* __restrict__ alpha,
                                                              double* __restrict__ b, int32_t* __restrict__ basis_indices,
@@ -210,22 +273,22 @@
                                                              int64_t trace_cap, PivotRecord* rec) {
     const PivotRecord R = *rec;
     if (R.outcome != DEV_RUNNING) return;
-    if ((int)blockIdx.x < nb_row) tab_row_update_body<B>(tv, du, sp, R, blockIdx.x);
+    if ((int)blockIdx.x < nb_row) tab_row_update_body<B, PARTS>(tv, du, sp, R, blockIdx.x);
     else tab_update_w_vectors_body<B>(du, m, alpha, b, basis_indices, in_basis, trace, trace_cap, R, rec, blockIdx.x - nb_row);
 }
 
-template <int B>
+template <int B, int PARTS>
 __global__ __launch_bounds__(kThreads) void k_tab_ratio_update_all(TableauView tv, DeferredUpdate du, SelectPartials sp, int nb_row,
                                                                    int m, const double* alpha,
                                                                    const double* __restrict__ b_in, double* __restrict__ b_out,
                                                                    const int32_t* __restrict__ basis_in,
                                                                    int32_t* __restrict__ basis_out, uint8_t* in_basis,
                                                                    int32_t* __restrict__ trace, int64_t trace_cap, Tolerances tol,
-                                                                   const double* rmin, int nblk,
+                                                                   const double* rmin, int nblk, int nrmin, int rpb,
                                                                    double* __restrict__ shadow, int32_t* __restrict__ shadow_meta,
                                                                    PivotRecord* rec, const double* __restrict__ msgs, int count,
                                                                    int64_t msg_len, int rule, int split) {
-    const double first = (!msgs && (int)threadIdx.x < nblk) ? rmin[threadIdx.x] : INFINITY;
+    const double first = (!msgs && (int)threadIdx.x < nrmin) ? rmin[threadIdx.x] : INFINITY;
     PivotRecord R = *rec;
     const bool w_half = (int)blockIdx.x >= nb_row;
     const int part = w_half ? ((int)blockIdx.x - nb_row) / nblk : 0;
@@ -253,7 +316,7 @@
         rmin = alpha + m;
     }
     int r, leaving;
-    ratio_blocks_pick<kThreads>(alpha, b_in, basis_in, m, tol, rmin, nblk, &r, &leaving, first, !msgs);
+    ratio_blocks_pick<kThreads>(alpha, b_in, basis_in, m, tol, rmin, nrmin, &r, &leaving, first, !msgs, rpb);
     if (r < 0) {
         if (mine) { b_out[i] = b_in[i]; basis_out[i] = basis_in[i]; }
         if (lead && wblock == 0 && threadIdx.x == 0) rec->outcome = DEV_NO_ROW;
@@ -273,7 +336,7 @@
     const double alpha_r = s_ab[0], b_r = s_ab[1];
     const int jt = s_jt, q = R.q;
     if (!w_half) {
-        tab_row_update_core<B>(tv, du, sp, R, blockIdx.x, s_wr, p_old, jt, r, q, leaving, R.d_q, alpha_r);
+        tab_row_update_core<B, PARTS>(tv, du, sp, R, blockIdx.x, s_wr, p_old, jt, r, q, leaving, R.d_q, alpha_r);
         return;
     }
     const double br = b_r / alpha_r;
@@ -324,16 +387,17 @@
     if (threadIdx.x == 0) shadow_meta[0] = -1;
 }
 
-template <int B>
+template <int B, int PARTS>
 __global__ __launch_bounds__(kThreads) void k_tab_select_column(TableauView tv, DeferredUpdate du, SelectPartials sp,
                                                                 int count, double* alpha, double* msg,
                                                                 const double* b, Tolerances tol,
                                                                 double* rmin, PivotRecord* rec,
                                                                 const double* shadow, int32_t* shadow_meta) {
+    constexpr int R = kThreads / PARTS;
     const int outcome = rec->outcome, p = rec->n_eta;
     if (shadow_meta) {
         const int srow = shadow_meta[0], slen = shadow_meta[1];
-        if (srow >= 0 && srow / kThreads == (int)blockIdx.x) {
+        if (srow >= 0 && srow / R == (int)blockIdx.x) {
             if ((int)threadIdx.x < slen) du.W[(int64_t)threadIdx.x * du.ld + srow] = shadow[threadIdx.x];
             __syncthreads();
             if (threadIdx.x == 0) shadow_meta[0] = -1;
@@ -343,16 +407,18 @@
     double k1 = INFINITY;
     int bj = 0x7fffffff;
     if ((int)threadIdx.x < count) { k1 = sp.k1[threadIdx.x]; bj = sp.j[threadIdx.x]; }
-    const int i = blockIdx.x * kThreads + threadIdx.x;
+    const int i = blockIdx.x * R + (int)threadIdx.x % R;
+    const bool head = (int)threadIdx.x < R;
     const double b_i = (rmin && i < tv.m) ? b[i] : 0.0;
     if (outcome != DEV_RUNNING) return;
     __shared__ double s_vs[kMaxEta];
     __shared__ double s_min[kThreads / 64];
+    __shared__ double s_hand[PARTS > 1 ? R : 1];
     tab_select_entering<kThreads>(tv, sp, count, k1, bj);
     if (bj == 0x7fffffff) {
         if (msg) {
-            if (i < tv.m) alpha[i] = 0.0;
-            if (i == 0) { msg[0] = INFINITY; msg[1] = 0.0; msg[2] = 0.0; }
+            if (head && i < tv.m) alpha[i] = 0.0;
+            if (threadIdx.x == 0 && i == 0) { msg[0] = INFINITY; msg[1] = 0.0; msg[2] = 0.0; }
         } else if (blockIdx.x == 0 && threadIdx.x == 0) {
             rec->outcome = DEV_NO_CANDIDATE;
             if (sp.rule == 1) rec->last_selected = -1;
@@ -370,12 +436,12 @@
         }
     }
     if ((int)threadIdx.x < p) s_vs[threadIdx.x] = tv.R0[(int64_t)threadIdx.x * tv.ld_r + cq];
-    const double t0 = i < tv.m ? tv.T0[(int64_t)cq * tv.ld_t + i] : 0.0;
+    const double t0 = (head && i < tv.m) ? tv.T0[(int64_t)cq * tv.ld_t + i] : 0.0;
     __syncthreads();
     double ratio = INFINITY;
-    if (i < tv.m) {
-        double a = t0;
-        for_pending<B>(du.W, du.ld, i, p, [&](int j, double w) { a = fma(w, s_vs[j], a); });
+    double a = t0;
+    const bool ends = for_pending_relay<B, PARTS>(du.W, du.ld, i, p, i < tv.m, a, s_hand, [&](int j, double w) { a = fma(w, s_vs[j], a); });
+    if (ends && i < tv.m) {
         alpha[i] = a;
         const double bz = b_i <= tol.zero ? 0.0 : b_i;
         if (a > tol.pivot) ratio = bz / a;
@@ -391,11 +457,12 @@
 __global__ __launch_bounds__(kSingleBlock) void k_ratio_blocks(const double* __restrict__ alpha, const double* __restrict__ b,
                                                                const int32_t* __restrict__ basis_indices, int m,
                                                                Tolerances tol, DeferredUpdate du,
-                                                               const double* __restrict__ rmin, int nblk, PivotRecord* rec) {
+                                                               const double* __restrict__ rmin, int nblk, int rpb,
+                                                               PivotRecord* rec) {
     const int outcome = rec->outcome, p = rec->n_eta;
     const double first = (int)threadIdx.x < nblk ? rmin[threadIdx.x] : INFINITY;
     if (outcome != DEV_RUNNING) return;
-    ratio_blocks_body<kSingleBlock>(alpha, b, basis_indices, m, tol, du, rmin, nblk, p, rec, first, true);
+    ratio_blocks_body<kSingleBlock>(alpha, b, basis_indices, m, tol, du, rmin, nblk, p, rec, first, true, rpb);
 }
 
 __global__ __launch_bounds__(kSingleBlock) void k_tab_select_candidate_ratio(const double* __restrict__ msgs, int count,
@@ -703,7 +770,7 @@
     __shared__ double s_w[kMaxEta];
     if ((int)threadIdx.x < p) s_w[threadIdx.x] = du.W[(int64_t)threadIdx.x * du.ld + row];
     __syncthreads();
-    const int c = tv.c_lo + blockIdx.x * kThreads + threadIdx.x;
+    const int c = (int)threadIdx.x < sp.slot_cols ? tv.c_lo + blockIdx.x * sp.slot_cols + (int)threadIdx.x : tv.c_hi;
     const int j = c - tv.col_off;
     double key = INFINITY;
     int kj = 0x7fffffff;
@@ -715,7 +782,16 @@
     block_partial_min(key, kj, sp, blockIdx.x);
 }
 
-int32_t tab_scan_blocks(int32_t n_owned_columns) { return cdiv(n_owned_columns, kThreads); }
+int32_t tab_scan_blocks(int32_t n_owned_columns, int32_t slot_cols) { return cdiv(n_owned_columns, slot_cols == 128 ? 128 : kThreads); }
+
+void tab_geometry(int32_t m, int32_t n_owned, int32_t w_split, int32_t want_rows, int32_t want_cols, int32_t out[2]) {
+    int rows = 64;
+    while (rows < kThreads && cdiv(m, rows) > 256) rows *= 2;
+    if (want_rows == 64 || want_rows == 128 || want_rows == 256) rows = want_rows;
+    int cols = cdiv(n_owned, 128) + std::max(w_split, 1) * cdiv(m, kThreads) <= kTabSplitCUs ? 128 : 256;
+    if (want_cols == 128 || want_cols == 256) cols = want_cols;
+    out[0] = rows; out[1] = cols;
+}
 
 int32_t tab_load_batch(int32_t wanted) {
     return (wanted == 1 || wanted == 8 || wanted == 16 || wanted == 32) ? wanted : kTabLoadBatchDefault;
@@ -732,6 +808,17 @@
     static_assert(kTabLoadBatchDefault == 8, "the default of tab_load_batch is the switch's default case");
 }
 
+template <bool kRows, class Launch>
+static void with_geometry(int32_t batch, int32_t width, Launch&& launch) {
+    with_load_batch(batch, [&](auto B) {
+        if (width == 128) { launch(B, std::integral_constant<int, 2>{}); return; }
+        if constexpr (kRows)
+            if (width == 64) { launch(B, std::integral_constant<int, 4>{}); return; }
+        launch(B, std::integral_constant<int, 1>{});
+    });
+}
+static int32_t col_rows(const DeferredUpdate& du) { return (du.col_rows == 64 || du.col_rows == 128) ? du.col_rows : kThreads; }
+
 void launch_tab_build(const TableauView& tv, const double* A, int64_t ld_a, const ColumnTable& ct, hipStream_t s) {
     const int64_t total = (int64_t)tv.m * (tv.c_hi - tv.c_lo);
     if (total <= 0) return;
@@ -752,7 +839,7 @@
 
 void launch_tab_scan(const TableauView& tv, SelectPartials sp, const PivotRecord* rec, hipStream_t s) {
     if (tv.c_hi <= tv.c_lo) return;
-    hipLaunchKernelGGL(k_tab_scan, dim3(tab_scan_blocks(tv.c_hi - tv.c_lo)), dim3(kThreads), 0, s, tv, sp, rec);
+    hipLaunchKernelGGL(k_tab_scan, dim3(tab_scan_blocks(tv.c_hi - tv.c_lo, sp.slot_cols)), dim3(kThreads), 0, s, tv, sp, rec);
 }
 
 void launch_tab_select(const TableauView& tv, SelectPartials sp, int32_t count, PivotRecord* rec, hipStream_t s) {
@@ -769,9 +856,9 @@
 void launch_tab_row_update(const TableauView& tv, const DeferredUpdate& du, SelectPartials sp, PivotRecord* rec,
                            hipStream_t s) {
     if (tv.c_hi <= tv.c_lo) return;
-    with_load_batch(du.batch, [&](auto B) {
-        hipLaunchKernelGGL((k_tab_row_update<decltype(B)::value>), dim3(tab_scan_blocks(tv.c_hi - tv.c_lo)), dim3(kThreads), 0, s, tv, du, sp,
-                           rec);
+    with_geometry<false>(du.batch, sp.slot_cols, [&](auto B, auto P) {
+        hipLaunchKernelGGL((k_tab_row_update<decltype(B)::value, decltype(P)::value>), dim3(tab_scan_blocks(tv.c_hi - tv.c_lo, sp.slot_cols)),
+                           dim3(kThreads), 0, s, tv, du, sp, rec);
     });
 }
 
@@ -784,9 +871,10 @@
 void launch_tab_select_column_rmin(const TableauView& tv, const DeferredUpdate& du, SelectPartials sp, int32_t count,
                                    double* alpha, const double* b, Tolerances tol, double* rmin, PivotRecord* rec,
                                    hipStream_t s, const double* shadow, int32_t* shadow_meta) {
-    with_load_batch(du.batch, [&](auto B) {
-        hipLaunchKernelGGL((k_tab_select_column<decltype(B)::value>), dim3(cdiv(tv.m, kThreads)), dim3(kThreads), 0, s, tv, du, sp, count, alpha,
-                           (double*)nullptr, b, tol, rmin, rec, shadow, shadow_meta);
+    const int rows = col_rows(du);
+    with_geometry<true>(du.batch, rows, [&](auto B, auto P) {
+        hipLaunchKernelGGL((k_tab_select_column<decltype(B)::value, decltype(P)::value>), dim3(cdiv(tv.m, rows)), dim3(kThreads), 0, s, tv, du,
+                           sp, count, alpha, (double*)nullptr, b, tol, rmin, rec, shadow, shadow_meta);
     });
 }
 
@@ -795,13 +883,14 @@
                                  int32_t* basis_out, uint8_t* in_basis, int32_t* trace, int64_t trace_cap, Tolerances tol,
                                  const double* rmin, double* shadow, int32_t* shadow_meta, PivotRecord* rec, hipStream_t s,
                                  const double* msgs, int32_t count, int64_t msg_len, int32_t rule) {
-    const int nb_row = tv.c_hi > tv.c_lo ? tab_scan_blocks(tv.c_hi - tv.c_lo) : 0;
+    const int nb_row = tv.c_hi > tv.c_lo ? tab_scan_blocks(tv.c_hi - tv.c_lo, sp.slot_cols) : 0;
     const int nb_w = cdiv(m, kThreads);
+    const int rpb = msgs ? kThreads : col_rows(du), nrmin = cdiv(m, rpb);
     int split = tab_load_batch(du.batch) == 1 ? 1 : std::max(1, std::min({(int)du.w_split, (int)du.kmax, (kTabSplitCUs - nb_row) / nb_w}));
-    with_load_batch(du.batch, [&](auto B) {
-        hipLaunchKernelGGL((k_tab_ratio_update_all<decltype(B)::value>), dim3(nb_row + split * nb_w), dim3(kThreads), 0, s, tv, du, sp, nb_row, m,
-                           alpha, b_in, b_out, basis_in, basis_out, in_basis, trace, trace_cap, tol, rmin, nb_w, shadow,
-                           shadow_meta, rec, msgs, (int)count, msg_len, (int)rule, split);
+    with_geometry<false>(du.batch, sp.slot_cols, [&](auto B, auto P) {
+        hipLaunchKernelGGL((k_tab_ratio_update_all<decltype(B)::value, decltype(P)::value>), dim3(nb_row + split * nb_w), dim3(kThreads), 0, s,
+                           tv, du, sp, nb_row, m, alpha, b_in, b_out, basis_in, basis_out, in_basis, trace, trace_cap, tol, rmin, nb_w,
+                           nrmin, rpb, shadow, shadow_meta, rec, msgs, (int)count, msg_len, (int)rule, split);
     });
 }
 
@@ -812,14 +901,14 @@
 void launch_ratio_blocks(const double* alpha, const double* b, const int32_t* basis_indices, int32_t m, Tolerances tol,
                          const DeferredUpdate& du, const double* rmin, PivotRecord* rec, hipStream_t s) {
     hipLaunchKernelGGL(k_ratio_blocks, dim3(1), dim3(kSingleBlock), 0, s, alpha, b, basis_indices, m, tol, du, rmin,
-                       cdiv(m, kThreads), rec);
+                       cdiv(m, col_rows(du)), col_rows(du), rec);
 }
 
 void launch_tab_select_column_msg(const TableauView& tv, const DeferredUpdate& du, SelectPartials sp, int32_t count,
                                   double* msg, const double* b, Tolerances tol, PivotRecord* rec, hipStream_t s,
                                   const double* shadow, int32_t* shadow_meta) {
     with_load_batch(du.batch, [&](auto B) {
-        hipLaunchKernelGGL((k_tab_select_column<decltype(B)::value>), dim3(cdiv(tv.m, kThreads)), dim3(kThreads), 0, s, tv, du, sp, count, msg + 3,
+        hipLaunchKernelGGL((k_tab_select_column<decltype(B)::value, 1>), dim3(cdiv(tv.m, kThreads)), dim3(kThreads), 0, s, tv, du, sp, count, msg + 3,
                            msg, b, tol, msg + 3 + tv.m, rec, shadow, shadow_meta);
     });
 }
@@ -835,7 +924,7 @@
                                 int32_t nr_artificial, Tolerances tol, const PivotRecord* rec, hipStream_t s) {
     if (tv.c_hi <= tv.c_lo) return;
     with_load_batch(du.batch, [&](auto B) {
-        hipLaunchKernelGGL((k_tab_zero_level_scan<decltype(B)::value>), dim3(tab_scan_blocks(tv.c_hi - tv.c_lo)), dim3(kThreads), 0, s, tv, du, sp,
+        hipLaunchKernelGGL((k_tab_zero_level_scan<decltype(B)::value>), dim3(tab_scan_blocks(tv.c_hi - tv.c_lo, sp.slot_cols)), dim3(kThreads), 0, s, tv, du, sp,
                            row, nr_artificial, tol, rec);
     });
 }
@@ -843,11 +932,11 @@
 void launch_tab_update_all(const TableauView& tv, const DeferredUpdate& du, SelectPartials sp, int32_t m,
                            const double* alpha, double* b, int32_t* basis_indices, uint8_t* in_basis, int32_t* trace,
                            int64_t trace_cap, PivotRecord* rec, hipStream_t s) {
-    const int nb_row = tv.c_hi > tv.c_lo ? tab_scan_blocks(tv.c_hi - tv.c_lo) : 0;
+    const int nb_row = tv.c_hi > tv.c_lo ? tab_scan_blocks(tv.c_hi - tv.c_lo, sp.slot_cols) : 0;
     const int nb_w = cdiv(m, kThreads);
-    with_load_batch(du.batch, [&](auto B) {
-        hipLaunchKernelGGL((k_tab_update_all<decltype(B)::value>), dim3(nb_row + nb_w), dim3(kThreads), 0, s, tv, du, sp, nb_row, m, alpha, b,
-                           basis_indices, in_basis, trace, trace_cap, rec);
+    with_geometry<false>(du.batch, sp.slot_cols, [&](auto B, auto P) {
+        hipLaunchKernelGGL((k_tab_update_all<decltype(B)::value, decltype(P)::value>), dim3(nb_row + nb_w), dim3(kThreads), 0, s, tv, du, sp,
+                           nb_row, m, alpha, b, basis_indices, in_basis, trace, trace_cap, rec);
     });
 }
 
@@ -883,7 +972,7 @@
                     hipStream_t s) {
     if (tv.c_hi <= tv.c_lo) return;
     with_load_batch(du.batch, [&](auto B) {
-        hipLaunchKernelGGL((k_tab_row<decltype(B)::value>), dim3(tab_scan_blocks(tv.c_hi - tv.c_lo)), dim3(kThreads), 0, s, tv, du, row, out, rec);
+        hipLaunchKernelGGL((k_tab_row<decltype(B)::value>), dim3(cdiv(tv.c_hi - tv.c_lo, kThreads)), dim3(kThreads), 0, s, tv, du, row, out, rec);
     });
 }
 
diff --git a/rust-lp_amd/engine.py b/rust-lp_amd/engine.py
--- a/rust-lp_amd/engine.py
+++ b/rust-lp_amd/engine.py
@@ -74,6 +74,8 @@
     "relp_flush": (C.c_int, [C.c_void_p]),
     "relp_update_block": (C.c_int32, [C.c_void_p]),
     "relp_tab_load_batch": (C.c_int32, [C.c_void_p]),
+    "relp_tab_geometry": (C.c_int, [C.c_void_p, C.POINTER(C.c_int32)]),
+    "relp_tab_geometry_rule": (None, [C.c_int32, C.c_int32, C.c_int32, C.c_int32, C.c_int32, C.POINTER(C.c_int32)]),
     "relp_tab_flush_stats": (C.c_int, [C.c_void_p, C.POINTER(C.c_int64)]),
     "relp_lu_stats": (C.c_int, [C.c_void_p, C.POINTER(C.c_int64)]),
     "relp_lu_lookahead_stats": (C.c_int, [C.c_void_p, C.POINTER(C.c_int64)]),
@@ -341,6 +343,11 @@
     def load_batch(self) -> int:
         return self._lib.relp_tab_load_batch(self._h)
 
+    def geometry(self) -> Tuple[int, int]:
+        out = (C.c_int32 * 2)()
+        self._ck(self._lib.relp_tab_geometry(self._h, out))
+        return int(out[0]), int(out[1])
+
     def flush_stats(self) -> Tuple[int, int]:
         out = (C.c_int64 * 2)()
         self._ck(self._lib.relp_tab_flush_stats(self._h, out))
```

After: 44130 iterations/s. 2.9% lower.
